# WGLab/NanoCaller

Hardware: AMD Instinct MI355X
Metric: candidate sites/sec (pileup+CNN) (higher is better)
Workload: dtype f32 (f16x3 split MFMA, f32 accumulate)

## Files before the change

### include/nanocaller_hip.h

```cpp
#ifndef NANOCALLER_HIP_H
#define NANOCALLER_HIP_H

#include <stddef.h>
#include <stdint.h>

#ifdef __cplusplus
extern "C" {
#endif

#define NC_ABI_VERSION 11

typedef struct nc_ctx nc_ctx;

enum nc_status {
    NC_OK = 0,
    NC_ERR_ARG = -1,
    NC_ERR_CAPACITY = -2,
    NC_ERR_NOMEM = -3,
    NC_ERR_HIP = -4,
    NC_ERR_STATE = -5,
    NC_ERR_SELFTEST = -6,
    NC_ERR_UNSUPPORTED = -7
};

enum nc_model_kind { NC_MODEL_SNP = 0, NC_MODEL_SNP_HAP = 1, NC_MODEL_INDEL = 2, NC_MODEL_INDEL_HAP = 3 };

enum nc_seq_mode { NC_SEQ_ONT = 0, NC_SEQ_SHORT_ONT = 1, NC_SEQ_UL_ONT = 2, NC_SEQ_UL_ONT_EXTREME = 3, NC_SEQ_PACBIO = 4 };

#define NC_CODE_ABSENT 7
#define NC_FLANK 50000
#define NC_SNP_TENSOR 1025

int nc_abi_version(void);
int nc_device_count(int *n);
int nc_ctx_create(int device_id, nc_ctx **out);
int nc_ctx_destroy(nc_ctx *ctx);
int nc_ctx_set_stream(nc_ctx *ctx, void *hip_stream);
int nc_ctx_sync(nc_ctx *ctx);
const char *nc_last_error(const nc_ctx *ctx);
int nc_malloc(nc_ctx *ctx, size_t bytes, void **dev);
int nc_free(nc_ctx *ctx, void *dev);
int nc_memcpy_h2d(nc_ctx *ctx, void *dev, const void *host, size_t bytes);
int nc_memcpy_d2h(nc_ctx *ctx, void *host, const void *dev, size_t bytes);
int nc_d2h_async(nc_ctx *ctx, void *stream, void *host, const void *dev, size_t bytes);
int nc_last_kernel_ms(nc_ctx *ctx, int which, float *ms);
int nc_enable_timing(nc_ctx *ctx, int on);
int nc_timing_sums(nc_ctx *ctx, double *sum_ms, int64_t *count);

typedef struct {
    int32_t start;
    int32_t end;
    int64_t base_flag;
} nc_tile_entry;

typedef struct {
    int64_t codes_len;
    const uint8_t *codes;
    int32_t tile_size;
    int32_t tile_pos0;
    int32_t n_tiles;
    const int32_t *tile_off;
    const nc_tile_entry *tile_ent;
    int64_t n_entries;
} nc_readpack;

int nc_pack_plan(int32_t n_reads, const int32_t *start, const int32_t *end, const uint8_t *keep,
                 int32_t tile_size, int32_t pos_lo, int32_t pos_hi,
                 int64_t *codes_len, int32_t *tile_pos0, int32_t *n_tiles, int64_t *n_entries);
int nc_pack_fill(int32_t n_reads, const int32_t *start, const int32_t *end, const int64_t *off,
                 const uint8_t *codes_in, const uint8_t *strand, const uint8_t *keep,
                 int32_t tile_size, int32_t tile_pos0, int32_t n_tiles,
                 uint8_t *codes_out, int64_t codes_len, int32_t *tile_off, nc_tile_entry *tile_ent,
                 int64_t n_entries);

typedef struct nc_wire nc_wire;
typedef struct {
    int32_t n_reads;
    const int32_t *rd_start;
    const int32_t *rd_end;
    const int64_t *slot_off;
    int64_t codes_len;
    int64_t n_blocks;
    const uint32_t *blk_off;
    const int32_t *blk_read;
    const uint16_t *events;
    int64_t n_events;
    const uint32_t *blk_ev;
    const uint8_t *ev_bytes;
    int64_t n_ev_bytes;
} nc_wire_arrays;
int nc_wire_build(int32_t n_reads, const int32_t *start, const int32_t *end, const int64_t *off, const uint8_t *codes_in,
                  const uint8_t *keep, const uint8_t *ref_wire, int32_t ref_pos0, int64_t ref_len, nc_wire **out);
int nc_wire_view(const nc_wire *w, nc_wire_arrays *view);
int nc_wire_free(nc_wire *w);
int nc_wire_ref_unpack(nc_ctx *ctx, const uint8_t *d_ref_nib, int64_t ref_len, uint8_t *d_ref_wire);
int nc_wire_ins_unpack(nc_ctx *ctx, const uint8_t *d_packed, int64_t n_bases, const int32_t *d_other_idx, int32_t n_other, uint8_t *d_ins_bases);
int nc_wire_build_del(int32_t n_reads, const int32_t *start, const int32_t *end, const int64_t *off, const uint8_t *codes_in,
                      const uint8_t *keep, const uint8_t *ref_wire, int32_t ref_pos0, int64_t ref_len, const int32_t *ev_off,
                      const int32_t *ev_pos, const int32_t *ev_len, nc_wire **out);
int nc_wire_apply_deletions(nc_ctx *ctx, int32_t n_reads, const int32_t *d_rd_start, const int32_t *d_rd_end, const int64_t *d_slot_off,
                            const int32_t *d_ev_off, const int32_t *d_ev_pos, const int32_t *d_ev_len, uint8_t *d_codes);
int nc_wire_expand(nc_ctx *ctx, int32_t n_reads, const int32_t *d_rd_start, const int32_t *d_rd_end, const int64_t *d_slot_off,
                   const uint8_t *d_ref_wire, int32_t ref_pos0, int64_t ref_len, const uint32_t *d_blk_off,
                   const int32_t *d_blk_read, const uint16_t *d_events, int64_t n_blocks, uint8_t *d_codes, int64_t codes_len,
                   uint8_t *d_ref_code);
int nc_wire_build2(int32_t n_reads, const int32_t *start, const int32_t *end, const int64_t *off, const uint8_t *codes_in,
                   const uint8_t *keep, const uint8_t *ref_wire, int32_t ref_pos0, int64_t ref_len, const int32_t *ev_off,
                   const int32_t *ev_pos, const int32_t *ev_len, int32_t flags, nc_wire **out);
int nc_wire_expand2(nc_ctx *ctx, int32_t n_reads, const int32_t *d_rd_start, const int32_t *d_rd_end, const int64_t *d_slot_off,
                    const uint8_t *d_ref_wire, int32_t ref_pos0, int64_t ref_len, const uint32_t *d_blk_off,
                    const int32_t *d_blk_read, const uint8_t *d_ev_bytes, int64_t n_blocks, uint8_t *d_codes, int64_t codes_len,
                    uint8_t *d_ref_code, const uint32_t *d_blk_ev, const int32_t *d_ev_off, const int32_t *d_ev_pos,
                    const int32_t *d_ev_len);
int nc_wire_expand_del(nc_ctx *ctx, int32_t n_reads, const int32_t *d_rd_start, const int32_t *d_rd_end, const int64_t *d_slot_off,
                       const uint8_t *d_ref_wire, int32_t ref_pos0, int64_t ref_len, const uint32_t *d_blk_off,
                       const int32_t *d_blk_read, const uint16_t *d_events, int64_t n_blocks, uint8_t *d_codes, int64_t codes_len,
                       uint8_t *d_ref_code, const uint32_t *d_blk_ev, const int32_t *d_ev_off, const int32_t *d_ev_pos,
                       const int32_t *d_ev_len);

int nc_indel_events_pack(int32_t n_reads, const int32_t *rd_start, const int32_t *ev_off, const int32_t *ev_pos, const int32_t *ev_len,
                         uint16_t *d16, int8_t *l8, int32_t *read_ins_off, int64_t big_cap, int32_t *big_idx, int32_t *big_pos,
                         int32_t *big_len, int64_t *n_big);
int nc_indel_events_expand(nc_ctx *ctx, int32_t n_reads, const int32_t *d_rd_start, const int32_t *d_ev_off, const uint16_t *d_d16,
                           const int8_t *d_l8, int32_t n_big, const int32_t *d_big_idx, const int32_t *d_big_pos, const int32_t *d_big_len,
                           const int32_t *d_read_ins_off, int32_t *d_ev_pos, int32_t *d_ev_len, int32_t *d_ins_off);
int nc_indel_events_pack8(int32_t n_reads, const int32_t *rd_start, const int32_t *ev_off, const int32_t *ev_pos, const int32_t *ev_len,
                          uint8_t *b8, uint16_t *d16x, int64_t esc_cap, int32_t *read_esc_off, int32_t *read_ins_off, int64_t big_cap,
                          int32_t *big_idx, int32_t *big_pos, int32_t *big_len, int64_t *n_esc, int64_t *n_big);
int nc_indel_events_expand8(nc_ctx *ctx, int32_t n_reads, const int32_t *d_rd_start, const int32_t *d_ev_off, const uint8_t *d_b8,
                            const uint16_t *d_d16x, const int32_t *d_read_esc_off, int32_t n_big, const int32_t *d_big_idx,
                            const int32_t *d_big_pos, const int32_t *d_big_len, const int32_t *d_read_ins_off, int32_t *d_ev_pos,
                            int32_t *d_ev_len, int32_t *d_ins_off);

int nc_inflate_device(nc_ctx *ctx, int32_t n_blocks, const uint8_t *d_comp, const int64_t *d_coff, const int32_t *d_clen, uint8_t *d_out,
                      const int64_t *d_ooff, const int32_t *d_isize, int32_t *d_status, uint32_t *d_tok, int32_t *d_ntok);
int nc_inflate_device_phase(nc_ctx *ctx, int32_t phase, int32_t n_blocks, const uint8_t *d_comp, const int64_t *d_coff, const int32_t *d_clen,
                            uint8_t *d_out, const int64_t *d_ooff, const int32_t *d_isize, int32_t *d_status, uint32_t *d_tok, int32_t *d_ntok);
int nc_bgzf_crc_device(nc_ctx *ctx, int32_t n_blocks, const uint8_t *d_comp, const int64_t *d_coff, const int32_t *d_clen, const uint8_t *d_out,
                       const int64_t *d_ooff, const int32_t *d_isize, int32_t *d_status);

int nc_bam_retag_sizes(nc_ctx *ctx, const uint8_t *d_raw, int32_t n_rec, const int64_t *d_rec_off, const uint64_t *d_hash, const int32_t *d_ps,
                       int32_t n_tags, int32_t *d_new_size, int32_t *d_tag_idx, int64_t *d_out_off, int32_t *d_status);
int nc_bam_retag(nc_ctx *ctx, const uint8_t *d_raw, int32_t n_rec, const int64_t *d_rec_off, const uint8_t *d_hp, const int32_t *d_ps,
                 const int32_t *d_tag_idx, const int64_t *d_out_off, uint8_t *d_out);
int nc_bgzf_deflate_device(nc_ctx *ctx, int32_t n, const uint8_t *d_in, const int64_t *d_ioff, const int32_t *d_ilen, uint8_t *d_out,
                           const int64_t *d_ooff, int32_t *d_clen, uint32_t *d_crc, int32_t *d_status);
int nc_bgzf_crc32_device(nc_ctx *ctx, int32_t n, const uint8_t *d_in, const int64_t *d_ioff, const int32_t *d_ilen, uint32_t *d_crc);
int nc_bgzf_assemble_device(nc_ctx *ctx, int32_t n, const uint8_t *d_pay, const int64_t *d_poff, const int32_t *d_clen, const uint32_t *d_crc,
                            const int32_t *d_isize, int64_t *d_foff, uint8_t *d_file);

#define NC_BAM_META_COLS 12
int nc_bgzf_members(const uint8_t *data, int64_t n, int64_t cap, int64_t *coff, int32_t *clen, int32_t *isize, int64_t *n_members);
int nc_bgzf_scan(const uint8_t *data, int64_t n, int64_t start, int64_t cap, int64_t *coff, int32_t *clen, int32_t *isize, int64_t *n_members,
                 int64_t *next);
int nc_bam_walk(nc_ctx *ctx, const uint8_t *d_raw, int64_t raw_len, int32_t n_seeds, const int64_t *d_seed, const int32_t *d_seed_tid,
                const int64_t *d_first, int64_t *d_out, int32_t *d_status);
int nc_bam_meta(nc_ctx *ctx, const uint8_t *d_raw, int64_t n_rec, const int64_t *d_rec_off, int32_t *d_meta, int32_t *d_status);
int nc_bam_codes(nc_ctx *ctx, const uint8_t *d_raw, int32_t n_reads, const int64_t *d_rec, const int64_t *d_slot, const int32_t *d_cigd,
                 const int32_t *d_ncig, const int32_t *d_start, uint8_t *d_codes);
int nc_bam_name_groups(nc_ctx *ctx, const uint8_t *d_raw, int64_t raw_len, int64_t n_cand, const int64_t *d_rec_off, const uint64_t *d_hash,
                       int32_t *d_gid, int32_t *d_status);
int nc_bam_indel_reads(nc_ctx *ctx, const uint8_t *d_raw, int32_t n_reads, const int64_t *d_rec, const int32_t *d_cigd, const int32_t *d_ncig,
                       int32_t tail_cap, int32_t *d_counts, const int32_t *d_ev_off, const int32_t *d_ins_base, const int32_t *d_tail_off,
                       int32_t *d_ev_pos, int32_t *d_ev_len, int32_t *d_ins_off, uint8_t *d_ins_bases, uint8_t *d_tail_bases);

typedef struct {
    int32_t mincov;
    double min_allele_freq;
    double nbr_t0, nbr_t1;
    int32_t haploid;
} nc_scan_params;

int nc_snp_scan(nc_ctx *ctx, const nc_readpack *pack,
                const uint8_t *ref_code_dev, int32_t ref_pos0, int32_t ref_len,
                int32_t scan_lo, int32_t scan_hi, const nc_scan_params *params,
                int32_t n_chunks, const int32_t *chunk_start_host, const int32_t *chunk_end_host,
                int32_t *n_nbr, int32_t *n_cand, int32_t *n_sites);

int nc_snp_scan_begin(nc_ctx *ctx, const nc_readpack *pack,
                      const uint8_t *ref_code_dev, int32_t ref_pos0, int32_t ref_len,
                      int32_t scan_lo, int32_t scan_hi, const nc_scan_params *params,
                      int32_t n_chunks, const int32_t *chunk_start_host, const int32_t *chunk_end_host);
int nc_snp_scan_end(nc_ctx *ctx, int32_t *n_nbr, int32_t *n_cand, int32_t *n_sites);

int nc_snp_scan_fetch(nc_ctx *ctx, int32_t *nbr_pos, int32_t *site_pos, int32_t *site_chunk,
                      int32_t *site_n, int32_t *site_alt);

int nc_snp_scan_fetch_async(nc_ctx *ctx, void *copy_stream, int32_t *nbr_pos, int32_t *site_pos, int32_t *site_chunk,
                            int32_t *site_n, int32_t *site_alt);

int nc_snp_featurize(nc_ctx *ctx, const nc_readpack *pack,
                     const uint8_t *ref_code_dev, int32_t ref_pos0, int32_t ref_len,
                     int32_t seq_mode, int32_t maxcov, int32_t min_nbr_sites,
                     float *x_dev, int32_t *ref_code_out_dev, int32_t *fwd_dp_dev, int32_t *rev_dp_dev,
                     int32_t *site_depth_dev, uint8_t *valid_dev);

int nc_snp_set_mates(nc_ctx *ctx, int32_t n_mates, const int64_t *d_mate_key, const int32_t *d_mate_rec);

int nc_indel_set_mates(nc_ctx *ctx, int32_t n_mates, const int64_t *d_mate_key, const int32_t *d_mate_rec);

int nc_snp_scale(nc_ctx *ctx, const int32_t *site_depth_dev, const uint8_t *valid_dev, double train_coverage,
                 int32_t mode, double *scale_dev, double *chunk_depth_host);
int nc_snp_chunk_depth_async(nc_ctx *ctx, void *copy_stream, double *chunk_depth_host_pinned);

int nc_load_weights(nc_ctx *ctx, int32_t model_kind, const float *blob_host, size_t n_floats);
int nc_set_cnn_precision(nc_ctx *ctx, int exact_fp32);
int nc_set_tensor_format(nc_ctx *ctx, int fmt);
int nc_snp_forward(nc_ctx *ctx, int32_t model_kind, int64_t n, const float *x_dev, const int32_t *ref_code_dev,
                   const double *scale_dev, int32_t scale_mode, float *probs_dev, float *gt_dev);

int nc_snp_forward_drain(nc_ctx *ctx, int32_t model_kind, int64_t n, const float *x_dev, const int32_t *ref_code_dev,
                         const double *scale_dev, int32_t scale_mode, float *probs_dev, float *gt_dev,
                         void *copy_stream, float *probs_host, float *gt_host);
int nc_cnn_x_limit(nc_ctx *ctx, int32_t model_kind, float *x_limit);
int nc_cnn_range_watch(nc_ctx *ctx, uint8_t *site_flags_dev);
int nc_snp_trunk_info(nc_ctx *ctx, int32_t *mfma_per_site, int32_t *kernel_id);
int nc_indel_forward(nc_ctx *ctx, int32_t model_kind, int64_t n, const float *x_dev, float *probs_dev);

int nc_indel_tensor(nc_ctx *ctx, int32_t n_sets, const uint8_t *rows_dev, const int64_t *row_off_dev,
                    const int32_t *n_rows_dev, const int32_t *n_cols_dev, const uint8_t *ref_rows_dev,
                    const int64_t *ref_off_dev, int32_t max_cols, float *x_dev, uint8_t *cns_dev);

typedef struct {
    int32_t n_reads;
    const int32_t *ev_off;
    const int32_t *ev_pos;
    const int32_t *ev_len;
    const uint8_t *read_hap;
} nc_indel_events;

typedef struct {
    int32_t mincov, win_size, small_win_size;
    double ins_t, del_t;
    int32_t haploid;
    int32_t impute;
} nc_indel_scan_params;

int nc_indel_scan(nc_ctx *ctx, const nc_readpack *pack, const nc_indel_events *events, const uint8_t *excl_dev,
                  int32_t start, int32_t end, const nc_indel_scan_params *params, int8_t *col_type_host);

int nc_indel_scan_batch(nc_ctx *ctx, const nc_readpack *pack, const nc_indel_events *events, const uint8_t *excl_dev,
                        int32_t n_chunks, const int32_t *starts, const int32_t *ends, const nc_indel_scan_params *params,
                        int8_t *col_type_host, const int64_t *col_off);

typedef struct nc_bam nc_bam;
typedef struct nc_decoded nc_decoded;
typedef struct {
    int32_t n_reads;
    const int32_t *start, *end, *flag;
    const int64_t *off;
    const uint8_t *codes;
    int64_t n_codes;
    const int32_t *ev_off;
    const int32_t *ev_pos, *ev_len;
    int64_t n_events;
    const uint8_t *hap;
    const int32_t *ps;
    const int64_t *seq_off;
    const uint8_t *seq;
    int64_t n_seq;
    const int32_t *name_off;
    const char *names;
    const int32_t *qstart;
} nc_decoded_arrays;

int nc_bam_open(const char *path, nc_bam **out);
int nc_bam_close(nc_bam *bam);
int nc_bam_n_refs(nc_bam *bam, int32_t *n_refs, int32_t *has_index);
int nc_bam_ref(nc_bam *bam, int32_t i, const char **name, int32_t *length);
const char *nc_bam_error(const nc_bam *bam);
int nc_bam_set_threads(nc_bam *bam, int32_t n);
int nc_bam_decode(nc_bam *bam, int32_t tid, int32_t beg1, int32_t end1, int32_t keep_seq, nc_decoded **out);
int nc_bam_decode_regions(const char *path, int32_t tid, int32_t beg1, int32_t end1, int32_t keep_seq, int32_t n_regions,
                          nc_decoded **out);
int nc_decoded_view(const nc_decoded *d, nc_decoded_arrays *view);
int nc_decoded_free(nc_decoded *d);
#define NC_FLAG_REFSKIP 0x10000
int nc_decoded_check(const nc_decoded *d, const uint8_t *keep, int64_t *n_refskip, int64_t *n_dup_overlap);
int nc_decoded_name_groups(const nc_decoded *d, const uint8_t *keep, int32_t *gid, int64_t *n_shared);

typedef struct nc_slices nc_slices;
typedef struct {
    int32_t n_anchor;
    const int32_t *anchor_off;
    const int32_t *read_idx;
    const int64_t *seq_off;
    const uint8_t *seq;
    int64_t n_slices;
} nc_slices_arrays;
int nc_indel_slices(const nc_decoded *d, int32_t n_anchor, const int32_t *anchor_pos, int32_t window_before, int32_t window_after,
                    const uint8_t *keep, nc_slices **out);
int nc_slices_view(const nc_slices *s, nc_slices_arrays *view);
int nc_slices_free(nc_slices *s);

typedef struct nc_pass2 nc_pass2;
typedef struct {
    int32_t n_kept;
    const int32_t *anchor_idx;
    const int32_t *first0;
    int32_t sets_per_anchor;
    int32_t n_sets;
    const int32_t *set_read0;
    int32_t n_alignments;
    const int32_t *read_off;
    const char *reads;
    const int32_t *ref_off;
    const char *refs;
    int32_t max_cols;
    const int32_t *al_dup;
} nc_pass2_arrays;
int nc_indel_pass2_sets(const nc_decoded *d, const uint8_t *keep, int32_t n_anchor, const int32_t *anchors, const char *contig,
                        int64_t chrom_len, int32_t ref_lo, int32_t ref_hi, int32_t window_after, int32_t mincov, int32_t maxcov,
                        int32_t haploid, const int32_t *imp_idx, const int32_t *imp_off, const int32_t *imp_reads, nc_pass2 **out);
int nc_pass2_view(const nc_pass2 *p, nc_pass2_arrays *view);
int nc_pass2_free(nc_pass2 *p);


typedef struct nc_indel_pack_h nc_indel_pack_h;
typedef struct {
    int32_t n_reads;
    const int32_t *ev_off;
    const int32_t *ev_pos, *ev_len;
    int64_t n_events;
    const int32_t *ins_off;
    const uint8_t *ins_bases;
    int64_t n_ins_bases;
    const int32_t *tail_off;
    const uint8_t *tail_bases;
    int64_t n_tail_bases;
    const int32_t *read_ps;
    const uint8_t *read_hap;
    const uint8_t *read_flag;
} nc_indel_pack_arrays;
int nc_indel_pack_build(const nc_decoded *d, const uint8_t *keep, int32_t tail_cap, nc_indel_pack_h **out);
int nc_indel_pack_view(const nc_indel_pack_h *p, nc_indel_pack_arrays *view);
int nc_indel_pack_free(nc_indel_pack_h *p);

typedef struct {
    int32_t n_reads;
    const int64_t *slot_off;
    const int32_t *rd_start;
    const int32_t *rd_end;
    const int32_t *ev_off, *ev_pos, *ev_len;
    const int32_t *ins_off;
    const uint8_t *ins_bases;
    const int32_t *tail_off;
    const uint8_t *tail_bases;
    const int32_t *read_ps;
    const uint8_t *read_hap, *read_flag;
} nc_indel_reads;

int nc_indel_sites_plan(nc_ctx *ctx, const nc_readpack *pack, const uint8_t *ref_code_dev, int32_t ref_pos0, int32_t ref_len,
                        int64_t chrom_len, const nc_indel_reads *reads, const uint8_t *excl_dev, int32_t n_chunks,
                        const int32_t *starts, const int32_t *ends, const nc_indel_scan_params *params, int32_t window_after,
                        int32_t maxcov, int32_t *n_sites, int64_t *n_alignments);
int nc_indel_sites_scoring(nc_ctx *ctx, int32_t open, int32_t extend, int32_t match, int32_t mismatch);
int nc_indel_sites_run(nc_ctx *ctx, float *x_dev);
int nc_indel_sites_fetch(nc_ctx *ctx, int32_t *pos, int32_t *chunk, int32_t *var_type, int32_t *phase, int32_t *ref_len,
                         int32_t *alt_len, int64_t *n_alt_bytes);
int nc_indel_sites_fetch_alt(nc_ctx *ctx, uint8_t *alt_bases, int64_t cap);
int nc_indel_sites_stage_ms(nc_ctx *ctx, float *ms6, int64_t *cells2 );
int nc_indel_sites_band_stats(nc_ctx *ctx, int64_t *stats6);
int nc_indel_sites_band(nc_ctx *ctx, int32_t mode, int32_t margin);

int nc_indel_vcf_format(const char *chrom, int64_t n, const int32_t *pos, const int32_t *chunk, int32_t n_chunks, const float *probs,
                        int32_t sets, const int32_t *ref_len, const int32_t *alt_len, const uint8_t *alt_bases, const int32_t *phase,
                        const char *contig, int64_t chrom_len, int32_t haploid, char *out, int64_t cap, int64_t *n_bytes,
                        int64_t *chunk_txt_off);

int nc_nw_cigar(const char *s1, int32_t n1, const char *s2, int32_t n2, int32_t open, int32_t extend, int32_t match, int32_t mismatch,
                int32_t *ops, int32_t *counts, int32_t cap, int32_t *n_ops);

int nc_allele_prediction(const char *alt, int32_t n_alt, const char *ref_seq, int32_t n_ref, int32_t max_range, int32_t *ref_len,
                         int32_t *alt_len);
int nc_allele_prediction_batch(int32_t n, const char *alts, const int32_t *alt_off, const char *refs, const int32_t *ref_off,
                               const int32_t *max_range, int32_t *ref_len, int32_t *alt_len);
int nc_allele_prediction_device(nc_ctx *ctx, int32_t n, const char *alts, const int32_t *alt_off, const char *refs, const int32_t *ref_off,
                                const int32_t *max_range, int32_t *ref_len, int32_t *alt_len);

int nc_star_msa(int32_t n_reads, const char *reads, const int32_t *read_off, const char *ref, int32_t n_ref, int32_t open,
                int32_t extend, int32_t match, int32_t mismatch, int32_t col_cap, uint8_t *rows, uint8_t *ref_row, int32_t *n_cols);

int nc_star_msa_tensor(nc_ctx *ctx, int32_t n_sets, const char *reads, const int32_t *read_off, const int32_t *set_read0,
                       const char *refs, const int32_t *ref_off, int32_t open, int32_t extend, int32_t match, int32_t mismatch,
                       int32_t max_cols, float *x_dev, uint8_t *cns_host, int32_t *n_cols_host, uint8_t *rows_host,
                       const int64_t *rows_host_off, uint8_t *ref_rows_host, const int64_t *ref_rows_host_off);
int nc_star_msa_tensor_dup(nc_ctx *ctx, int32_t n_sets, const char *reads, const int32_t *read_off, const int32_t *set_read0,
                           const char *refs, const int32_t *ref_off, int32_t open, int32_t extend, int32_t match, int32_t mismatch,
                           int32_t max_cols, float *x_dev, uint8_t *cns_host, int32_t *n_cols_host, uint8_t *rows_host,
                           const int64_t *rows_host_off, uint8_t *ref_rows_host, const int64_t *ref_rows_host_off, const int32_t *al_dup);

int nc_consensus_strings(const uint8_t *cns, int32_t n_sets, int32_t max_cols, const int32_t *n_cols, char *out, int64_t *off);

int nc_snp_vcf_format(const char *chrom, int64_t n, const int32_t *pos, const int32_t *ref, const float *probs,
                      const int32_t *order, const int32_t *dp, const double *freq, const int32_t *fwd, const int32_t *rev,
                      int32_t haploid, char *out, int64_t cap, int64_t *n_bytes);

int nc_argsort4(const float *probs, int64_t n, int32_t *order, int64_t *n_ties, int64_t *tie_idx, int64_t tie_cap);

int nc_bgzf_compress(const uint8_t *data, int64_t n, int32_t level, uint8_t *out, int64_t cap, int64_t *n_out,
                     int64_t *block_coff, int64_t blk_cap, int64_t *n_blocks);

int nc_bgzf_read_file(const char *path, uint8_t *out, int64_t cap, int64_t *n_out);

int nc_synth_indel_truth(nc_ctx *ctx, int64_t L, uint64_t seed, double het_snp, double hom_snp, double het_indel, double hom_indel,
                         int32_t max_len, uint8_t *ref_dev, uint8_t *hap_base_dev, int8_t *hap_indel_dev);
int nc_synth_indel_reads(nc_ctx *ctx, int64_t L, uint64_t seed, double p_sub, double p_del, double p_ins, double carry, int32_t n_reads,
                         const int32_t *start_dev, const int32_t *end_dev, const int64_t *slot_off_dev, const uint8_t *hap_dev,
                         const uint8_t *hap_base_dev, const int8_t *hap_indel_dev, int32_t fill, int32_t *ev_cnt_dev, int32_t *ins_cnt_dev,
                         const int32_t *ev_off_dev, const int32_t *ins_off_read_dev, uint8_t *codes_dev, int32_t *ev_pos_dev,
                         int32_t *ev_len_dev, int32_t *ins_off_dev, uint8_t *ins_bases_dev);

typedef struct nc_phase nc_phase;
typedef struct {
    int32_t n_reads, n_sites, n_blocks, n_groups;
    int64_t n_entries;
    const int64_t *entry_off;
    const int32_t *entry_site;
    const uint8_t *entry_allele;
    const int8_t *read_side;
    const int32_t *site_block;
    const uint8_t *site_h;
    const uint8_t *site_phased;
    const int32_t *site_ps;
    const int32_t *block_first, *block_last, *block_ps;
    const int64_t *block_cost;
    const uint8_t *group_hp;
    const int32_t *group_ps;
    float ms[4];
} nc_phase_arrays;
int nc_snp_phase_gather(nc_ctx *ctx, const uint8_t *codes, int64_t codes_len, int32_t n_reads, const int32_t *rd_start, const int32_t *rd_end,
                        const int64_t *slot_off, int32_t n_sites, const int32_t *site_pos, const uint8_t *site_alleles, nc_phase **out);
int nc_snp_phase_realign(nc_ctx *ctx, const uint8_t *codes, int64_t codes_len, const nc_indel_reads *reads, int64_t n_events, int64_t n_ins_bases,
                         const uint8_t *ref_code, int32_t ref_len, int32_t n_sites, const int32_t *site_pos, const uint8_t *site_alleles, nc_phase **out);
int nc_snp_phase_load(nc_ctx *ctx, int32_t n_reads, int32_t n_sites, const int32_t *site_pos, const int64_t *entry_off, const int32_t *entry_site,
                      const uint8_t *entry_allele, nc_phase **out);
int nc_snp_phase_solve(nc_ctx *ctx, nc_phase *ph, int32_t max_cov);
int nc_haplotag_run(nc_ctx *ctx, nc_phase *ph, int32_t n_groups, const int32_t *read_group);
int nc_snp_phase_view(const nc_phase *ph, nc_phase_arrays *out);
int nc_snp_phase_free(nc_phase *ph);
int nc_snp_phase_solve_gt(nc_ctx *ctx, nc_phase *ph, int32_t max_cov, const uint8_t *site_gt, int32_t gt_cost);
int nc_snp_phase_genotypes(const nc_phase *ph, const uint8_t **site_gt);
int nc_snp_phase_set_weights(nc_ctx *ctx, nc_phase *ph, const uint8_t *entry_weight, const uint8_t *read_ok);
int nc_snp_phase_weights_from_bam(nc_ctx *ctx, nc_phase *ph, const uint8_t *d_raw, int64_t raw_len, const int64_t *d_rec_off, int32_t mapq_min,
                                  int32_t default_weight, int32_t w_max);
int nc_snp_phase_weights(const nc_phase *ph, const uint8_t **entry_weight, const uint8_t **read_mapq, const uint8_t **read_ok);

int nc_fasta_decode(nc_ctx *ctx, const uint8_t *d_raw, int64_t raw_len, int64_t first, int64_t length, int64_t linebases, int64_t linewidth,
                    uint8_t *d_letters, uint8_t *d_scan, int64_t scan_pos0, int64_t scan_len, int64_t ga, int64_t gb, uint8_t *d_blind,
                    int32_t *d_status);

#define NC_BAMIDX_BAD_BLOCK_SIZE 2
#define NC_BAMIDX_BAD_FIELDS 4
#define NC_BAMIDX_TRUNCATED 8
#define NC_BAMIDX_BAD_REFID 16
#define NC_BAMIDX_UNSORTED 32
#define NC_BAMIDX_BAD_MEMBERS 64
int nc_bamidx_candidates(nc_ctx *ctx, const uint8_t *d_raw, int64_t len, int64_t readable, int32_t n_ref, const int32_t *d_ref_len, uint64_t *d_words,
                         int32_t *d_cnt);
int nc_bamidx_chain(nc_ctx *ctx, const uint8_t *d_raw, int64_t len, int64_t first, const uint64_t *d_words, const int32_t *d_rank, int32_t n_cand,
                    int64_t *d_pos, int32_t *d_jump, int32_t *d_mark);
int nc_bamidx_collect(nc_ctx *ctx, int32_t n_cand, const int64_t *d_pos, const int32_t *d_mark, const int32_t *d_mark_rank, int64_t *d_out);
int nc_bamidx_verify(nc_ctx *ctx, const uint8_t *d_raw, int64_t len, int64_t first, int64_t n_rec, const int64_t *d_out, int32_t last, int64_t *d_res);
int nc_bamidx_serial(nc_ctx *ctx, const uint8_t *d_raw, int64_t len, int64_t first, int32_t last, int64_t *d_out, int64_t *d_res);
int nc_bamidx_fields(nc_ctx *ctx, const uint8_t *d_raw, int64_t n_rec, const int64_t *d_rec_off, int64_t stream_base, const int32_t *d_meta, int32_t n_ref,
                     int32_t n_mem, const int64_t *d_mem_ooff, const int64_t *d_mem_foff, int32_t has_prev, int32_t prev_refid, int32_t prev_pos,
                     int32_t min_shift, int32_t depth, int64_t *d_voff, int32_t *d_fields, int32_t *d_status);

#ifdef __cplusplus
}
#endif
#endif
```

### nanocaller_amd/_lib.py

```python
from __future__ import annotations

import ctypes as C
import os

import numpy as np

_HERE = os.path.dirname(os.path.abspath(__file__))
LIB_PATH = os.environ.get("NANOCALLER_HIP_LIB") or os.path.join(_HERE, "libnanocaller_hip.so")

NC_OK = 0
NC_ERR_ARG = -1
NC_ERR_CAPACITY = -2
NC_ERR_NOMEM = -3
NC_ERR_UNSUPPORTED = -7
FLAG_REFSKIP = 0x10000
ABI_VERSION = 11
MODEL_SNP, MODEL_SNP_HAP, MODEL_INDEL, MODEL_INDEL_HAP = 0, 1, 2, 3
SEQ_MODES = {"ont": 0, "short_ont": 1, "ul_ont": 2, "ul_ont_extreme": 3, "pacbio": 4}
CODE_ABSENT = 7
FLANK = 50000
SNP_TENSOR = 1025
STAR_SCORING = (25, 1, 20, -10)

EXPORTS = [
    "nc_abi_version", "nc_device_count", "nc_ctx_create", "nc_ctx_destroy", "nc_ctx_set_stream", "nc_ctx_sync",
    "nc_last_error", "nc_malloc", "nc_free", "nc_memcpy_h2d", "nc_memcpy_d2h", "nc_last_kernel_ms",
    "nc_enable_timing", "nc_pack_plan", "nc_pack_fill", "nc_snp_scan", "nc_snp_scan_begin", "nc_snp_scan_end", "nc_snp_scan_fetch", "nc_snp_featurize",
    "nc_snp_scale", "nc_load_weights", "nc_snp_forward", "nc_indel_forward", "nc_indel_tensor", "nc_indel_scan",
    "nc_bam_open", "nc_bam_close", "nc_bam_n_refs", "nc_bam_ref", "nc_bam_error", "nc_bam_decode", "nc_decoded_view",
    "nc_decoded_free", "nc_snp_vcf_format", "nc_set_cnn_precision", "nc_snp_scan_fetch_async", "nc_snp_forward_drain", "nc_argsort4", "nc_indel_slices", "nc_slices_view", "nc_slices_free",
    "nc_nw_cigar", "nc_allele_prediction", "nc_bgzf_compress", "nc_bam_set_threads", "nc_indel_scan_batch", "nc_timing_sums", "nc_snp_chunk_depth_async", "nc_bam_decode_regions", "nc_star_msa", "nc_star_msa_tensor", "nc_star_msa_tensor_dup", "nc_set_tensor_format", "nc_allele_prediction_batch", "nc_allele_prediction_device", "nc_bgzf_read_file", "nc_consensus_strings",
    "nc_wire_build", "nc_wire_build_del", "nc_wire_apply_deletions", "nc_wire_ref_unpack", "nc_wire_view", "nc_wire_free", "nc_wire_expand", "nc_wire_expand_del", "nc_snp_set_mates", "nc_indel_set_mates", "nc_decoded_name_groups", "nc_wire_ins_unpack", "nc_indel_events_pack8", "nc_indel_events_expand8", "nc_wire_build2", "nc_wire_expand2", "nc_d2h_async",
    "nc_indel_pass2_sets", "nc_pass2_view", "nc_pass2_free",
    "nc_decoded_check", "nc_indel_pack_build", "nc_indel_pack_view", "nc_indel_pack_free", "nc_indel_sites_plan", "nc_indel_sites_run",
    "nc_indel_sites_fetch", "nc_indel_sites_fetch_alt", "nc_indel_sites_stage_ms", "nc_indel_sites_band_stats", "nc_indel_sites_band", "nc_indel_events_pack", "nc_indel_events_expand", "nc_inflate_device", "nc_inflate_device_phase", "nc_bgzf_crc_device", "nc_bgzf_members", "nc_bgzf_scan", "nc_bam_walk", "nc_bam_meta", "nc_bam_codes", "nc_bam_indel_reads", "nc_bam_name_groups", "nc_indel_sites_scoring", "nc_indel_vcf_format", "nc_synth_indel_truth", "nc_synth_indel_reads", "nc_cnn_x_limit", "nc_cnn_range_watch", "nc_snp_trunk_info",
    "nc_snp_phase_gather", "nc_snp_phase_load", "nc_snp_phase_solve", "nc_haplotag_run", "nc_snp_phase_view", "nc_snp_phase_free",
    "nc_snp_phase_realign", "nc_snp_phase_solve_gt", "nc_snp_phase_genotypes",
    "nc_snp_phase_set_weights", "nc_snp_phase_weights_from_bam", "nc_snp_phase_weights",
    "nc_bam_retag_sizes", "nc_bam_retag", "nc_bgzf_deflate_device", "nc_bgzf_crc32_device", "nc_bgzf_assemble_device",
    "nc_fasta_decode",
    "nc_bamidx_candidates", "nc_bamidx_chain", "nc_bamidx_collect", "nc_bamidx_verify", "nc_bamidx_serial", "nc_bamidx_fields",
]


class TileEntry(C.Structure):
    _fields_ = [("start", C.c_int32), ("end", C.c_int32), ("base_flag", C.c_int64)]


TILE_ENTRY_DTYPE = np.dtype([("start", "<i4"), ("end", "<i4"), ("base_flag", "<i8")])
assert TILE_ENTRY_DTYPE.itemsize == C.sizeof(TileEntry) == 16


class ReadPackC(C.Structure):
    _fields_ = [("codes_len", C.c_int64), ("codes", C.c_void_p), ("tile_size", C.c_int32), ("tile_pos0", C.c_int32),
                ("n_tiles", C.c_int32), ("tile_off", C.c_void_p), ("tile_ent", C.c_void_p), ("n_entries", C.c_int64)]


class ScanParamsC(C.Structure):
    _fields_ = [("mincov", C.c_int32), ("min_allele_freq", C.c_double), ("nbr_t0", C.c_double), ("nbr_t1", C.c_double),
                ("haploid", C.c_int32)]


class IndelEventsC(C.Structure):
    _fields_ = [("n_reads", C.c_int32), ("ev_off", C.c_void_p), ("ev_pos", C.c_void_p), ("ev_len", C.c_void_p),
                ("read_hap", C.c_void_p)]


class IndelScanParamsC(C.Structure):
    _fields_ = [("mincov", C.c_int32), ("win_size", C.c_int32), ("small_win_size", C.c_int32), ("ins_t", C.c_double),
                ("del_t", C.c_double), ("haploid", C.c_int32), ("impute", C.c_int32)]


class DecodedArraysC(C.Structure):
    _fields_ = [("n_reads", C.c_int32), ("start", C.c_void_p), ("end", C.c_void_p), ("flag", C.c_void_p), ("off", C.c_void_p),
                ("codes", C.c_void_p), ("n_codes", C.c_int64), ("ev_off", C.c_void_p), ("ev_pos", C.c_void_p),
                ("ev_len", C.c_void_p), ("n_events", C.c_int64), ("hap", C.c_void_p), ("ps", C.c_void_p),
                ("seq_off", C.c_void_p), ("seq", C.c_void_p), ("n_seq", C.c_int64), ("name_off", C.c_void_p),
                ("names", C.c_void_p), ("qstart", C.c_void_p)]


class SlicesArraysC(C.Structure):
    _fields_ = [("n_anchor", C.c_int32), ("anchor_off", C.c_void_p), ("read_idx", C.c_void_p), ("seq_off", C.c_void_p),
                ("seq", C.c_void_p), ("n_slices", C.c_int64)]


class Pass2ArraysC(C.Structure):
    _fields_ = [("n_kept", C.c_int32), ("anchor_idx", C.c_void_p), ("first0", C.c_void_p), ("sets_per_anchor", C.c_int32),
                ("n_sets", C.c_int32), ("set_read0", C.c_void_p), ("n_alignments", C.c_int32), ("read_off", C.c_void_p),
                ("reads", C.c_void_p), ("ref_off", C.c_void_p), ("refs", C.c_void_p), ("max_cols", C.c_int32), ("al_dup", C.c_void_p)]


class IndelPackArraysC(C.Structure):
    _fields_ = [("n_reads", C.c_int32), ("ev_off", C.c_void_p), ("ev_pos", C.c_void_p), ("ev_len", C.c_void_p), ("n_events", C.c_int64),
                ("ins_off", C.c_void_p), ("ins_bases", C.c_void_p), ("n_ins_bases", C.c_int64), ("tail_off", C.c_void_p),
                ("tail_bases", C.c_void_p), ("n_tail_bases", C.c_int64), ("read_ps", C.c_void_p), ("read_hap", C.c_void_p),
                ("read_flag", C.c_void_p)]


class IndelReadsC(C.Structure):
    _fields_ = [("n_reads", C.c_int32), ("slot_off", C.c_void_p), ("rd_start", C.c_void_p), ("rd_end", C.c_void_p), ("ev_off", C.c_void_p),
                ("ev_pos", C.c_void_p), ("ev_len", C.c_void_p), ("ins_off", C.c_void_p), ("ins_bases", C.c_void_p), ("tail_off", C.c_void_p),
                ("tail_bases", C.c_void_p), ("read_ps", C.c_void_p), ("read_hap", C.c_void_p), ("read_flag", C.c_void_p)]


class WireArraysC(C.Structure):
    _fields_ = [("n_reads", C.c_int32), ("rd_start", C.c_void_p), ("rd_end", C.c_void_p), ("slot_off", C.c_void_p),
                ("codes_len", C.c_int64), ("n_blocks", C.c_int64), ("blk_off", C.c_void_p), ("blk_read", C.c_void_p), ("events", C.c_void_p),
                ("n_events", C.c_int64), ("blk_ev", C.c_void_p), ("ev_bytes", C.c_void_p), ("n_ev_bytes", C.c_int64)]


class PhaseArraysC(C.Structure):
    _fields_ = [("n_reads", C.c_int32), ("n_sites", C.c_int32), ("n_blocks", C.c_int32), ("n_groups", C.c_int32), ("n_entries", C.c_int64),
                ("entry_off", C.c_void_p), ("entry_site", C.c_void_p), ("entry_allele", C.c_void_p), ("read_side", C.c_void_p),
                ("site_block", C.c_void_p), ("site_h", C.c_void_p), ("site_phased", C.c_void_p), ("site_ps", C.c_void_p),
                ("block_first", C.c_void_p), ("block_last", C.c_void_p), ("block_ps", C.c_void_p), ("block_cost", C.c_void_p),
                ("group_hp", C.c_void_p), ("group_ps", C.c_void_p), ("ms", C.c_float * 4)]


_lib = None


class NanoCallerHipError(RuntimeError):
    pass


def lib():
    global _lib
    if _lib is None:
        if not os.path.exists(LIB_PATH):
            raise NanoCallerHipError(
                "%s not found: build it with `python -c 'import __graft_entry__ as g; g.build()'` "
                "(hipcc --offload-arch=gfx950). There is no CPU fallback." % LIB_PATH)
        try:
            import torch
        except ImportError:
            pass
        L = C.CDLL(LIB_PATH)
        vp, i32, i64, dbl = C.c_void_p, C.c_int32, C.c_int64, C.c_double
        L.nc_abi_version.restype = C.c_int
        if L.nc_abi_version() != ABI_VERSION:
            raise NanoCallerHipError("%s has ABI version %d, this binding needs %d: rebuild it" % (LIB_PATH, L.nc_abi_version(), ABI_VERSION))
        L.nc_device_count.argtypes = [C.POINTER(C.c_int)]
        L.nc_ctx_create.argtypes = [C.c_int, C.POINTER(vp)]
        L.nc_ctx_destroy.argtypes = [vp]
        L.nc_ctx_set_stream.argtypes = [vp, vp]
        L.nc_ctx_sync.argtypes = [vp]
        L.nc_last_error.argtypes = [vp]
        L.nc_last_error.restype = C.c_char_p
        L.nc_malloc.argtypes = [vp, C.c_size_t, C.POINTER(vp)]
        L.nc_free.argtypes = [vp, vp]
        L.nc_memcpy_h2d.argtypes = [vp, vp, vp, C.c_size_t]
        L.nc_memcpy_d2h.argtypes = [vp, vp, vp, C.c_size_t]
        L.nc_last_kernel_ms.argtypes = [vp, C.c_int, C.POINTER(C.c_float)]
        L.nc_timing_sums.argtypes = [vp, vp, vp]
        L.nc_enable_timing.argtypes = [vp, C.c_int]
        L.nc_set_cnn_precision.argtypes = [vp, C.c_int]
        L.nc_pack_plan.argtypes = [i32, vp, vp, vp, i32, i32, i32, C.POINTER(i64), C.POINTER(i32), C.POINTER(i32),
                                   C.POINTER(i64)]
        L.nc_pack_fill.argtypes = [i32, vp, vp, vp, vp, vp, vp, i32, i32, i32, vp, i64, vp, vp, i64]
        L.nc_snp_scan.argtypes = [vp, C.POINTER(ReadPackC), vp, i32, i32, i32, i32, C.POINTER(ScanParamsC), i32, vp, vp,
                                  C.POINTER(i32), C.POINTER(i32), C.POINTER(i32)]
        L.nc_snp_scan_begin.argtypes = [vp, C.POINTER(ReadPackC), vp, i32, i32, i32, i32, C.POINTER(ScanParamsC), i32, vp, vp]
        L.nc_snp_scan_end.argtypes = [vp, C.POINTER(i32), C.POINTER(i32), C.POINTER(i32)]
        L.nc_snp_scan_fetch.argtypes = [vp, vp, vp, vp, vp, vp]
        L.nc_snp_scan_fetch_async.argtypes = [vp, vp, vp, vp, vp, vp, vp]
        L.nc_snp_featurize.argtypes = [vp, C.POINTER(ReadPackC), vp, i32, i32, i32, i32, i32, vp, vp, vp, vp, vp, vp]
        L.nc_snp_scale.argtypes = [vp, vp, vp, dbl, i32, vp, vp]
        L.nc_snp_chunk_depth_async.argtypes = [vp, vp, vp]
        L.nc_load_weights.argtypes = [vp, i32, vp, C.c_size_t]
        L.nc_snp_forward.argtypes = [vp, i32, i64, vp, vp, vp, i32, vp, vp]
        L.nc_snp_forward_drain.argtypes = [vp, i32, i64, vp, vp, vp, i32, vp, vp, vp, vp, vp]
        L.nc_indel_forward.argtypes = [vp, i32, i64, vp, vp]
        L.nc_indel_tensor.argtypes = [vp, i32, vp, vp, vp, vp, vp, vp, i32, vp, vp]
        L.nc_indel_scan.argtypes = [vp, C.POINTER(ReadPackC), C.POINTER(IndelEventsC), vp, i32, i32, C.POINTER(IndelScanParamsC), vp]
        L.nc_indel_scan_batch.argtypes = [vp, C.POINTER(ReadPackC), C.POINTER(IndelEventsC), vp, i32, vp, vp, C.POINTER(IndelScanParamsC), vp, vp]
        L.nc_bam_open.argtypes = [C.c_char_p, C.POINTER(vp)]
        L.nc_bam_close.argtypes = [vp]
        L.nc_bam_set_threads.argtypes = [vp, i32]
        L.nc_bam_n_refs.argtypes = [vp, C.POINTER(i32), C.POINTER(i32)]
        L.nc_bam_ref.argtypes = [vp, i32, C.POINTER(C.c_char_p), C.POINTER(i32)]
        L.nc_bam_error.argtypes = [vp]
        L.nc_bam_error.restype = C.c_char_p
        L.nc_bam_decode.argtypes = [vp, i32, i32, i32, i32, C.POINTER(vp)]
        L.nc_star_msa_tensor.argtypes = [vp, i32, vp, vp, vp, vp, vp, i32, i32, i32, i32, i32, vp, vp, vp, vp, vp, vp, vp]
        L.nc_star_msa_tensor_dup.argtypes = L.nc_star_msa_tensor.argtypes + [vp]
        L.nc_consensus_strings.argtypes = [vp, i32, i32, vp, vp, vp]
        L.nc_allele_prediction_batch.argtypes = [i32, C.c_char_p, vp, C.c_char_p, vp, vp, vp, vp]
        L.nc_allele_prediction_device.argtypes = [vp, i32, C.c_char_p, vp, C.c_char_p, vp, vp, vp, vp]
        L.nc_set_tensor_format.argtypes = [vp, C.c_int]
        L.nc_star_msa.argtypes = [i32, C.c_char_p, vp, C.c_char_p, i32, i32, i32, i32, i32, i32, vp, vp, C.POINTER(i32)]
        L.nc_bam_decode_regions.argtypes = [C.c_char_p, i32, i32, i32, i32, i32, C.POINTER(vp)]
        L.nc_decoded_view.argtypes = [vp, C.POINTER(DecodedArraysC)]
        L.nc_decoded_free.argtypes = [vp]
        L.nc_indel_slices.argtypes = [vp, i32, vp, i32, i32, vp, C.POINTER(vp)]
        L.nc_slices_view.argtypes = [vp, C.POINTER(SlicesArraysC)]
        L.nc_slices_free.argtypes = [vp]
        L.nc_nw_cigar.argtypes = [C.c_char_p, i32, C.c_char_p, i32, i32, i32, i32, i32, vp, vp, i32, C.POINTER(i32)]
        L.nc_allele_prediction.argtypes = [C.c_char_p, i32, C.c_char_p, i32, i32, C.POINTER(i32), C.POINTER(i32)]
        L.nc_bgzf_compress.argtypes = [vp, i64, i32, vp, i64, C.POINTER(i64), vp, i64, C.POINTER(i64)]
        L.nc_indel_pass2_sets.argtypes = [vp, vp, i32, vp, C.c_char_p, i64, i32, i32, i32, i32, i32, i32, vp, vp, vp, C.POINTER(vp)]
        L.nc_pass2_view.argtypes = [vp, C.POINTER(Pass2ArraysC)]
        L.nc_pass2_free.argtypes = [vp]
        L.nc_d2h_async.argtypes = [vp, vp, vp, vp, C.c_size_t]
        L.nc_wire_build.argtypes = [i32, vp, vp, vp, vp, vp, vp, i32, i64, C.POINTER(vp)]
        L.nc_wire_build_del.argtypes = [i32, vp, vp, vp, vp, vp, vp, i32, i64, vp, vp, vp, C.POINTER(vp)]
        L.nc_wire_build2.argtypes = [i32, vp, vp, vp, vp, vp, vp, i32, i64, vp, vp, vp, i32, C.POINTER(vp)]
        L.nc_wire_apply_deletions.argtypes = [vp, i32, vp, vp, vp, vp, vp, vp, vp]
        L.nc_wire_ref_unpack.argtypes = [vp, vp, i64, vp]
        L.nc_wire_view.argtypes = [vp, C.POINTER(WireArraysC)]
        L.nc_wire_free.argtypes = [vp]
        L.nc_wire_expand.argtypes = [vp, i32, vp, vp, vp, vp, i32, i64, vp, vp, vp, i64, vp, i64, vp]
        L.nc_wire_expand_del.argtypes = L.nc_wire_expand.argtypes + [vp, vp, vp, vp]
        L.nc_wire_expand2.argtypes = L.nc_wire_expand.argtypes + [vp, vp, vp, vp]
        L.nc_snp_set_mates.argtypes = [vp, i32, vp, vp]
        L.nc_indel_set_mates.argtypes = [vp, i32, vp, vp]
        L.nc_decoded_name_groups.argtypes = [vp, vp, vp, C.POINTER(i64)]
        L.nc_wire_ins_unpack.argtypes = [vp, vp, i64, vp, i32, vp]
        L.nc_indel_events_pack8.argtypes = [i32, vp, vp, vp, vp, vp, vp, i64, vp, vp, i64, vp, vp, vp, C.POINTER(i64), C.POINTER(i64)]
        L.nc_indel_events_expand8.argtypes = [vp, i32, vp, vp, vp, vp, vp, i32, vp, vp, vp, vp, vp, vp, vp]
        L.nc_decoded_check.argtypes = [vp, vp, C.POINTER(i64), C.POINTER(i64)]
        L.nc_indel_pack_build.argtypes = [vp, vp, i32, C.POINTER(vp)]
        L.nc_indel_pack_view.argtypes = [vp, C.POINTER(IndelPackArraysC)]
        L.nc_indel_pack_free.argtypes = [vp]
        L.nc_indel_sites_plan.argtypes = [vp, C.POINTER(ReadPackC), vp, i32, i32, i64, C.POINTER(IndelReadsC), vp, i32, vp, vp,
                                          C.POINTER(IndelScanParamsC), i32, i32, C.POINTER(i32), C.POINTER(i64)]
        L.nc_indel_sites_run.argtypes = [vp, vp]
        L.nc_indel_sites_scoring.argtypes = [vp, i32, i32, i32, i32]
        L.nc_indel_sites_fetch.argtypes = [vp, vp, vp, vp, vp, vp, vp, C.POINTER(i64)]
        L.nc_indel_sites_fetch_alt.argtypes = [vp, vp, i64]
        L.nc_indel_sites_stage_ms.argtypes = [vp, vp, vp]
        L.nc_indel_sites_band_stats.argtypes = [vp, vp]
        L.nc_indel_sites_band.argtypes = [vp, i32, i32]
        L.nc_indel_events_pack.argtypes = [i32, vp, vp, vp, vp, vp, vp, vp, i64, vp, vp, vp, C.POINTER(i64)]
        L.nc_indel_events_expand.argtypes = [vp, i32, vp, vp, vp, vp, i32, vp, vp, vp, vp, vp, vp, vp]
        L.nc_inflate_device.argtypes = [vp, i32, vp, vp, vp, vp, vp, vp, vp, vp, vp]
        L.nc_inflate_device_phase.argtypes = [vp, i32, i32, vp, vp, vp, vp, vp, vp, vp, vp, vp]
        L.nc_bgzf_crc_device.argtypes = [vp, i32, vp, vp, vp, vp, vp, vp, vp]
        L.nc_bgzf_members.argtypes = [vp, i64, i64, vp, vp, vp, C.POINTER(i64)]
        L.nc_bgzf_scan.argtypes = [vp, i64, i64, i64, vp, vp, vp, C.POINTER(i64), C.POINTER(i64)]
        L.nc_bam_walk.argtypes = [vp, vp, i64, i32, vp, vp, vp, vp, vp]
        L.nc_bam_meta.argtypes = [vp, vp, i64, vp, vp, vp]
        L.nc_bam_codes.argtypes = [vp, vp, i32, vp, vp, vp, vp, vp, vp]
        L.nc_bam_indel_reads.argtypes = [vp, vp, i32, vp, vp, vp, i32, vp, vp, vp, vp, vp, vp, vp, vp, vp]
        L.nc_bam_name_groups.argtypes = [vp, vp, i64, i64, vp, vp, vp, vp]
        L.nc_indel_vcf_format.argtypes = [C.c_char_p, i64, vp, vp, i32, vp, i32, vp, vp, vp, vp, C.c_char_p, i64, i32, vp, i64, C.POINTER(i64), vp]
        L.nc_synth_indel_truth.argtypes = [vp, i64, C.c_uint64, dbl, dbl, dbl, dbl, i32, vp, vp, vp]
        L.nc_synth_indel_reads.argtypes = [vp, i64, C.c_uint64, dbl, dbl, dbl, dbl, i32, vp, vp, vp, vp, vp, vp, i32, vp, vp, vp, vp, vp, vp, vp, vp, vp]
        L.nc_cnn_x_limit.argtypes = [vp, i32, C.POINTER(C.c_float)]
        L.nc_snp_trunk_info.argtypes = [vp, C.POINTER(C.c_int32), C.POINTER(C.c_int32)]
        L.nc_cnn_range_watch.argtypes = [vp, vp]
        L.nc_argsort4.argtypes = [vp, i64, vp, C.POINTER(i64), vp, i64]
        L.nc_snp_phase_gather.argtypes = [vp, vp, i64, i32, vp, vp, vp, i32, vp, vp, C.POINTER(vp)]
        L.nc_snp_phase_load.argtypes = [vp, i32, i32, vp, vp, vp, vp, C.POINTER(vp)]
        L.nc_snp_phase_solve.argtypes = [vp, vp, i32]
        L.nc_snp_phase_solve_gt.argtypes = [vp, vp, i32, vp, i32]
        L.nc_snp_phase_genotypes.argtypes = [vp, C.POINTER(vp)]
        L.nc_snp_phase_set_weights.argtypes = [vp, vp, vp, vp]
        L.nc_snp_phase_weights_from_bam.argtypes = [vp, vp, vp, i64, vp, i32, i32, i32]
        L.nc_snp_phase_weights.argtypes = [vp, C.POINTER(vp), C.POINTER(vp), C.POINTER(vp)]
        L.nc_snp_phase_realign.argtypes = [vp, vp, i64, C.POINTER(IndelReadsC), i64, i64, vp, i32, i32, vp, vp, C.POINTER(vp)]
        L.nc_haplotag_run.argtypes = [vp, vp, i32, vp]
        L.nc_snp_phase_view.argtypes = [vp, C.POINTER(PhaseArraysC)]
        L.nc_snp_phase_free.argtypes = [vp]
        L.nc_bam_retag_sizes.argtypes = [vp, vp, i32, vp, vp, vp, i32, vp, vp, vp, vp]
        L.nc_bam_retag.argtypes = [vp, vp, i32, vp, vp, vp, vp, vp, vp]
        L.nc_bgzf_deflate_device.argtypes = [vp, i32, vp, vp, vp, vp, vp, vp, vp, vp]
        L.nc_bgzf_crc32_device.argtypes = [vp, i32, vp, vp, vp, vp]
        L.nc_bgzf_assemble_device.argtypes = [vp, i32, vp, vp, vp, vp, vp, vp, vp]
        L.nc_fasta_decode.argtypes = [vp, vp, i64, i64, i64, i64, i64, vp, vp, i64, i64, i64, i64, vp, vp]
        L.nc_bamidx_candidates.argtypes = [vp, vp, i64, i64, i32, vp, vp, vp]
        L.nc_bamidx_chain.argtypes = [vp, vp, i64, i64, vp, vp, i32, vp, vp, vp]
        L.nc_bamidx_collect.argtypes = [vp, i32, vp, vp, vp, vp]
        L.nc_bamidx_verify.argtypes = [vp, vp, i64, i64, i64, vp, i32, vp]
        L.nc_bamidx_serial.argtypes = [vp, vp, i64, i64, i32, vp, vp]
        L.nc_bamidx_fields.argtypes = [vp, vp, i64, vp, i64, vp, i32, i32, vp, vp, i32, i32, i32, i32, i32, vp, vp, vp]
        L.nc_snp_vcf_format.argtypes = [C.c_char_p, i64, vp, vp, vp, vp, vp, vp, vp, vp, i32, vp, i64, C.POINTER(i64)]
        for name in EXPORTS:
            fn = getattr(L, name)
            if name not in ("nc_last_error", "nc_bam_error"):
                fn.restype = C.c_int
        _lib = L
    return _lib


def npp(a):
    if a is None:
        return None
    assert a.flags["C_CONTIGUOUS"]
    return a.ctypes.data_as(C.c_void_p)
```

### nanocaller_amd/csrc/nc_cnn.h

```cpp
#pragma once
#include <cmath>
#include <vector>

#include "nc_common.h"

constexpr float SELU_L = 1.0507009873554805f;
constexpr float SELU_LA = 1.0507009873554805f * 1.6732632423543772f;

__device__ __forceinline__ float selu(float x) { return x > 0.0f ? SELU_L * x : SELU_LA * (__expf(x) - 1.0f); }
__device__ __forceinline__ float selu_acc(float x) { return x > 0.0f ? SELU_L * x : SELU_LA * (expf(x) - 1.0f); }

typedef float f32x4v __attribute__((ext_vector_type(4)));
typedef _Float16 h8 __attribute__((ext_vector_type(8)));
typedef _Float16 h2 __attribute__((ext_vector_type(2)));
typedef float f32x2v __attribute__((ext_vector_type(2)));
__device__ __forceinline__ h8 as_h8(uint4 v) { union { uint4 u; h8 h; } c; c.u = v; return c.h; }
__device__ __forceinline__ h8 lds_h8(const _Float16 *p) { return *reinterpret_cast<const h8 *>(p); }
struct h_epi { float c1, c2, c3; };
__device__ __forceinline__ float exp2_clamp01(float x) { float r; asm("v_exp_f32_e64 %0, %1 clamp" : "=v"(r) : "v"(x)); return r; }
__device__ __forceinline__ float sub_h_lo(float v, uint32_t hpk) { float r; asm("v_fma_mix_f32 %0, %1, -1.0, %2 op_sel_hi:[1,0,0]" : "=v"(r) : "v"(hpk), "v"(v)); return r; }
__device__ __forceinline__ float sub_h_hi(float v, uint32_t hpk) { float r; asm("v_fma_mix_f32 %0, %1, -1.0, %2 op_sel:[1,0,0] op_sel_hi:[1,0,0]" : "=v"(r) : "v"(hpk), "v"(v)); return r; }
__device__ __forceinline__ f32x4v selu4_scaled(const f32x4v &acc, const h_epi &k)
{
    f32x4v s;
#pragma unroll
    for (int r = 0; r < 4; r++) {
        const float a = acc[r];
        const float e = exp2_clamp01(a * k.c1);
        const float pos = __builtin_amdgcn_fmed3f(a, 0.0f, k.c3);
        const float neg = fmaf(e, SELU_LA, -SELU_LA);
        s[r] = fmaf(pos, k.c2, neg);
    }
    return s;
}
__device__ __forceinline__ void split4_store(const f32x4v &v, _Float16 *hp, _Float16 *lp)
{
    const h2 h01 = __builtin_convertvector((f32x2v){v[0], v[1]}, h2), h23 = __builtin_convertvector((f32x2v){v[2], v[3]}, h2);
    const uint32_t u01 = __builtin_bit_cast(uint32_t, h01), u23 = __builtin_bit_cast(uint32_t, h23);
    const f32x2v d01 = {sub_h_lo(v[0], u01), sub_h_hi(v[1], u01)}, d23 = {sub_h_lo(v[2], u23), sub_h_hi(v[3], u23)};
    const h2 l01 = __builtin_convertvector(d01, h2), l23 = __builtin_convertvector(d23, h2);
    *reinterpret_cast<uint2 *>(hp) = make_uint2(u01, u23);
    *reinterpret_cast<uint2 *>(lp) = make_uint2(__builtin_bit_cast(uint32_t, l01), __builtin_bit_cast(uint32_t, l23));
}

struct H3Scale {
    float S;
    H3Scale(const float *w0, const float *w1, float s0) : S(s0)
    {
        float wmax = 0.0f;
        for (const float *q = w0; q < w1; q++) wmax = std::fmax(wmax, std::fabs(*q));
        while (S > 1.0f && wmax * S > 16384.0f) S *= 0.5f;
    }
    void split(float v, _Float16 &h, _Float16 &l) const
    {
        const float sv = v * S;
        h = (_Float16)sv;
        l = (_Float16)(sv - (float)h);
    }
};

inline unsigned blocks_for(int64_t n, int per = 256) { return (unsigned)((n + per - 1) / per); }

enum { NC_TRUNK_FP32 = 0, NC_TRUNK_P3 = 2, NC_TRUNK_LIN = 3 };
struct SnpTrunk { int kernel_id, mfma_per_site; };
SnpTrunk nc_cnn_snp_trunk_select(const nc_ctx *ctx);
struct SnpTrunkArgs {
    hipStream_t stream;
    hipEvent_t ev0, ev1;
    const float *x_f32;
    const int16_t *x_i16;
    float *a3;
    int64_t nb, site0;
    const double *scale;
    int scale_mode;
    float x_limit;
    uint8_t *range_sites;
};
void nc_cnn_launch_k4_conv12(const SnpTrunkArgs &a, const float *packed);
void nc_cnn_launch_k5_trunk(int kernel_id, const SnpTrunkArgs &a, const uint8_t *packed_h);
void nc_cnn_launch_fc1_h3(hipStream_t st, const float *a3, const uint8_t *packed_h, float *f1, int64_t nb);
std::vector<float> nc_cnn_pack_k4(const float *blob);
std::vector<uint8_t> nc_cnn_pack_snp_h3(const float *blob);

void nc_cnn_launch_fc1_fp32(hipStream_t st, int F, const float *a3, int K, const float *kf, const float *bf, float *f1, int64_t nb);

void nc_cnn_launch_indel_convs_fp32(hipStream_t st, int H, const float *x, const float *w, float *a1, float *a2, float *a3, int64_t nb);
int nc_cnn_launch_k10(nc_ctx *ctx, int H, const float *x, const uint8_t *packed_h, float *a3, int64_t nb);
std::vector<uint8_t> nc_cnn_pack_indel_h3(const float *blob);
```

### nanocaller_amd/csrc/nc_cnn.hip

```cpp
#include <algorithm>

#include "nc_cnn.h"

namespace {

__device__ __forceinline__ void dense_small(const float *in, int n_in, const float *k, const float *b, int n_out, float *out, bool act)
{
    for (int o = 0; o < n_out; o++) {
        float acc = b[o];
        for (int i = 0; i < n_in; i++) acc = fmaf(in[i], k[i * n_out + o], acc);
        out[o] = act ? selu_acc(acc) : acc;
    }
}

__device__ __forceinline__ void softmax_small(float *x, int n)
{
    float m = x[0];
    for (int i = 1; i < n; i++) m = fmaxf(m, x[i]);
    float sum = 0.0f;
    for (int i = 0; i < n; i++) { x[i] = expf(x[i] - m); sum += x[i]; }
    for (int i = 0; i < n; i++) x[i] = x[i] / sum;
}

__global__ __launch_bounds__(256) void k_snp_heads(const float *__restrict__ fc1, const float *__restrict__ w,
                                                   const int32_t *__restrict__ ref_code, int64_t n, float *__restrict__ probs,
                                                   float *__restrict__ gt)
{
    const int64_t s = (int64_t)blockIdx.x * 256 + threadIdx.x;
    if (s >= n) return;
    float f1[48], fa[16], in17[17], heads[4][2], fc2[16], in24[24], fc3[8], g[2];
    for (int i = 0; i < 48; i++) f1[i] = fc1[s * 48 + i];
    const float *p = w;
    dense_small(f1, 48, p, p + 768, 16, fa, true);
    p += 768 + 16;
    for (int i = 0; i < 16; i++) in17[i] = fa[i];
    const int rc = ref_code[s];
    for (int h = 0; h < 4; h++) {
        in17[16] = rc == h ? 1.0f : 0.0f;
        dense_small(in17, 17, p, p + 34, 2, heads[h], false);
        p += 34 + 2;
        softmax_small(heads[h], 2);
        probs[s * 4 + h] = heads[h][1];
    }
    dense_small(f1, 48, p, p + 768, 16, fc2, true);
    p += 768 + 16;
    for (int i = 0; i < 16; i++) in24[i] = fc2[i];
    for (int h = 0; h < 4; h++) { in24[16 + 2 * h] = heads[h][0]; in24[17 + 2 * h] = heads[h][1]; }
    dense_small(in24, 24, p, p + 192, 8, fc3, true);
    p += 192 + 8;
    dense_small(fc3, 8, p, p + 16, 2, g, false);
    softmax_small(g, 2);
    if (gt) { gt[s * 2] = g[0]; gt[s * 2 + 1] = g[1]; }
}

__global__ __launch_bounds__(256) void k_snp_hap_heads(const float *__restrict__ fc1, const float *__restrict__ w,
                                                       const int32_t *__restrict__ ref_code, int64_t n, float *__restrict__ probs)
{
    const int64_t s = (int64_t)blockIdx.x * 256 + threadIdx.x;
    if (s >= n) return;
    float f1[48], in20[20], out[4];
    for (int i = 0; i < 48; i++) f1[i] = fc1[s * 48 + i];
    const float *p = w;
    dense_small(f1, 48, p, p + 768, 16, in20, true);
    p += 768 + 16;
    const int rc = ref_code[s];
    for (int b = 0; b < 4; b++) in20[16 + b] = rc == b ? 1.0f : 0.0f;
    dense_small(in20, 20, p, p + 80, 4, out, true);
    softmax_small(out, 4);
    for (int b = 0; b < 4; b++) probs[s * 4 + b] = out[b];
}

__global__ __launch_bounds__(256) void k_indel_heads(const float *__restrict__ fc1, const float *__restrict__ w, int nout, int64_t n,
                                                     float *__restrict__ probs)
{
    const int64_t s = (int64_t)blockIdx.x * 256 + threadIdx.x;
    if (s >= n) return;
    float f1[32], f2[24], out[4];
    for (int i = 0; i < 32; i++) f1[i] = fc1[s * 32 + i];
    const float *p = w;
    dense_small(f1, 32, p, p + 768, 24, f2, true);
    p += 768 + 24;
    dense_small(f2, 24, p, p + 24 * nout, nout, out, false);
    if (nout == 4) {
        softmax_small(out, 4);
        for (int b = 0; b < 4; b++) probs[s * 4 + b] = out[b];
    } else {
        probs[s] = 1.0f / (1.0f + expf(-out[0]));
    }
}

const size_t NPARAM[4] = {109370, 108308, 634420, 158185};

int run_snp_trunk(nc_ctx *ctx, const nc_weights &w, int64_t s0, int64_t nb, const void *x_dev, const double *scale, int scale_mode, const float **f1_out, const float **tail)
{
    constexpr int64_t n3 = 3 * 9 * 64, F = 48;
    NC_TRY(nc_ensure(ctx, ctx->cnn_c, (size_t)(nb * (n3 + F)) * 4 + 64));
    float *a3 = (float *)ctx->cnn_c.p, *f1 = a3 + ((nb * n3 + 3) & ~int64_t(3));
    const float *kf = w.dev + (400 + 16) * 2 + 2000 + 16 + 6 * 48 * 32 + 32 + 6 * 32 * 64 + 64, *bf = kf + n3 * F;
    *tail = bf + F;
    *f1_out = f1;
    SnpTrunkArgs a = {ctx->stream, nullptr, nullptr, nullptr, nullptr, a3, nb, s0, scale, scale_mode, w.x_limit, ctx->range_sites};
    if (ctx->x_i16) a.x_i16 = (const int16_t *)x_dev + s0 * NC_SNP_TENSOR;
    else a.x_f32 = (const float *)x_dev + s0 * NC_SNP_TENSOR;
    if (ctx->timing && ctx->n_kev + 2 <= 128) {
        for (int e = 0; e < 2; e++)
            if (!ctx->kev[ctx->n_kev + e]) NC_HIP(ctx, hipEventCreate(&ctx->kev[ctx->n_kev + e]));
        a.ev0 = ctx->kev[ctx->n_kev];
        a.ev1 = ctx->kev[ctx->n_kev + 1];
        ctx->n_kev += 2;
    }
    const SnpTrunk t = nc_cnn_snp_trunk_select(ctx);
    if (t.kernel_id == NC_TRUNK_FP32) {
        nc_cnn_launch_k4_conv12(a, w.packed);
        nc_cnn_launch_fc1_fp32(ctx->stream, F, a3, (int)n3, kf, bf, f1, nb);
    } else {
        nc_cnn_launch_k5_trunk(t.kernel_id, a, (const uint8_t *)w.packed_h);
        nc_cnn_launch_fc1_h3(ctx->stream, a3, (const uint8_t *)w.packed_h, f1, nb);
    }
    NC_HIP(ctx, hipGetLastError());
    return NC_OK;
}

int run_indel_trunk(nc_ctx *ctx, const nc_weights &w, int H, int64_t nb, const float *x_batch, const float **f1_out, const float **tail)
{
    constexpr int W = 128, CI = 2, C1 = 8, C2 = 32, C3 = 48, F = 32, W2 = (W - 3) / 2 + 1, W3 = (W2 - 3) / 2 + 1;
    const int64_t n1 = (int64_t)H * W * 3 * C1, n2 = (int64_t)(H - 1) * W2 * C2, n3 = (int64_t)(H - 2) * W3 * C3;
    const bool h3 = !ctx->cnn_exact_fp32 && w.x_limit >= 1.0f;
    if (!h3) {
        NC_TRY(nc_ensure(ctx, ctx->cnn_a, (size_t)(nb * n1) * 4));
        NC_TRY(nc_ensure(ctx, ctx->cnn_b, (size_t)(nb * n2) * 4));
    }
    NC_TRY(nc_ensure(ctx, ctx->cnn_c, (size_t)(nb * (n3 + F)) * 4 + 64));
    float *a3 = (float *)ctx->cnn_c.p, *f1 = a3 + ((nb * n3 + 3) & ~int64_t(3));
    const float *kf = w.dev + (5 + 5 + 25) * CI * C1 + 3 * C1 + 6 * 3 * C1 * C2 + C2 + 6 * C2 * C3 + C3, *bf = kf + n3 * F;
    *tail = bf + F;
    *f1_out = f1;
    if (h3) NC_TRY(nc_cnn_launch_k10(ctx, H, x_batch, (const uint8_t *)w.packed_h, a3, nb));
    else nc_cnn_launch_indel_convs_fp32(ctx->stream, H, x_batch, w.dev, (float *)ctx->cnn_a.p, (float *)ctx->cnn_b.p, a3, nb);
    nc_cnn_launch_fc1_fp32(ctx->stream, F, a3, (int)n3, kf, bf, f1, nb);
    NC_HIP(ctx, hipGetLastError());
    return NC_OK;
}

float cnn_x_limit(int kind, const float *blob)
{
    const bool snp = kind == NC_MODEL_SNP || kind == NC_MODEL_SNP_HAP;
    const int CI = snp ? 5 : 2, C1 = snp ? 16 : 8, C2 = 32, C3 = snp ? 64 : 48;
    auto l1 = [](const float *k, int n_in, int cout) {
        double best = 0;
        for (int c = 0; c < cout; c++) {
            double acc = 0;
            for (int i = 0; i < n_in; i++) acc += std::fabs((double)k[(size_t)i * cout + c]);
            best = std::max(best, acc);
        }
        return best;
    };
    auto amax = [](const float *b, int n) { double m = 0; for (int i = 0; i < n; i++) m = std::max(m, std::fabs((double)b[i])); return m; };
    const float *k11 = blob, *b11 = k11 + 5 * CI * C1, *k12 = b11 + C1, *b12 = k12 + 5 * CI * C1, *k13 = b12 + C1, *b13 = k13 + 25 * CI * C1;
    const float *k2 = b13 + C1, *b2 = k2 + 6 * 3 * C1 * C2, *k3 = b2 + C2, *b3 = k3 + 6 * C2 * C3;
    const double L1 = std::max(l1(k11, 5 * CI, C1), std::max(l1(k12, 5 * CI, C1), l1(k13, 25 * CI, C1)));
    const double B1 = std::max(amax(b11, C1), std::max(amax(b12, C1), amax(b13, C1)));
    const double L2 = l1(k2, 6 * 3 * C1, C2), B2 = amax(b2, C2), L3 = l1(k3, 6 * C2, C3), B3 = amax(b3, C3);
    const double LAM = 1.0507009873554805, LA = LAM * 1.6732632423543772, CAP = 60000.0 * 0.999;
    auto worst = [&](double X) {
        const double a1 = std::max(LAM * (L1 * X + B1), LA), a2 = std::max(LAM * (L2 * a1 + B2), LA), a3 = std::max(LAM * (L3 * a2 + B3), LA);
        return snp ? std::max(a1, std::max(a2, a3)) : std::max(a1, a2);
    };
    double lo = 0.0, hi = 1e6;
    if (worst(0.0) >= CAP) hi = 0.0;
    for (int it = 0; it < 60 && hi > 0.0; it++) {
        const double mid = 0.5 * (lo + hi);
        if (worst(mid) < CAP) lo = mid; else hi = mid;
    }
    return (float)lo;
}

int upload_blob(nc_ctx *ctx, void **dev, const void *host, size_t bytes, const char *what)
{
    if (!*dev) {
        hipError_t e = hipMalloc(dev, bytes);
        if (e != hipSuccess) return nc_fail(ctx, NC_ERR_NOMEM, "hipMalloc %s: %s", what, hipGetErrorString(e));
    }
    NC_HIP(ctx, hipMemcpyAsync(*dev, host, bytes, hipMemcpyHostToDevice, ctx->stream));
    NC_HIP(ctx, hipStreamSynchronize(ctx->stream));
    return NC_OK;
}

}

extern "C" {

int nc_load_weights(nc_ctx *ctx, int32_t kind, const float *blob_host, size_t n_floats)
{
    if (!ctx) return NC_ERR_ARG;
    if (kind < 0 || kind > 3 || !blob_host) return nc_fail(ctx, NC_ERR_ARG, "nc_load_weights: bad argument");
    if (n_floats != NPARAM[kind])
        return nc_fail(ctx, NC_ERR_ARG, "nc_load_weights: kind %d expects %zu floats, got %zu", kind, NPARAM[kind], n_floats);
    NC_HIP(ctx, hipSetDevice(ctx->device));
    nc_weights &w = ctx->w[kind];
    NC_TRY(upload_blob(ctx, (void **)&w.dev, blob_host, n_floats * 4, "weights"));
    w.n = n_floats;
    w.x_limit = cnn_x_limit(kind, blob_host);
    if (kind == NC_MODEL_SNP || kind == NC_MODEL_SNP_HAP) {
        const std::vector<float> pk = nc_cnn_pack_k4(blob_host);
        NC_TRY(upload_blob(ctx, (void **)&w.packed, pk.data(), pk.size() * 4, "packed weights"));
        const std::vector<uint8_t> hp = nc_cnn_pack_snp_h3(blob_host);
        NC_TRY(upload_blob(ctx, &w.packed_h, hp.data(), hp.size(), "packed fp16 weights"));
    } else {
        const std::vector<uint8_t> hp = nc_cnn_pack_indel_h3(blob_host);
        NC_TRY(upload_blob(ctx, &w.packed_h, hp.data(), hp.size(), "packed fp16 weights"));
    }
    return NC_OK;
}


int nc_snp_forward(nc_ctx *ctx, int32_t kind, int64_t n, const float *x_dev, const int32_t *ref_code_dev, const double *scale_dev,
                   int32_t scale_mode, float *probs_dev, float *gt_dev)
{
    return nc_snp_forward_drain(ctx, kind, n, x_dev, ref_code_dev, scale_dev, scale_mode, probs_dev, gt_dev, nullptr, nullptr, nullptr);
}

int nc_snp_forward_drain(nc_ctx *ctx, int32_t kind, int64_t n, const float *x_dev, const int32_t *ref_code_dev, const double *scale_dev,
                         int32_t scale_mode, float *probs_dev, float *gt_dev, void *copy_stream, float *probs_host, float *gt_host)
{
    if (!ctx) return NC_ERR_ARG;
    if (probs_host && !copy_stream) return nc_fail(ctx, NC_ERR_ARG, "nc_snp_forward_drain: host drain needs a copy stream");
    if (kind != NC_MODEL_SNP && kind != NC_MODEL_SNP_HAP) return nc_fail(ctx, NC_ERR_ARG, "nc_snp_forward: not an SNP model kind");
    if (!ctx->w[kind].dev) return nc_fail(ctx, NC_ERR_STATE, "nc_snp_forward: weights of kind %d not loaded", kind);
    if (n < 0 || (n && (!x_dev || !ref_code_dev || !probs_dev))) return nc_fail(ctx, NC_ERR_ARG, "nc_snp_forward: null argument");
    if (scale_mode != 0 && scale_mode != 1) return nc_fail(ctx, NC_ERR_ARG, "nc_snp_forward: scale_mode");
    if (ctx->x_i16 && ctx->cnn_exact_fp32) return nc_fail(ctx, NC_ERR_STATE, "nc_snp_forward: int16 tensors are read by the split-precision trunk only");
    NC_HIP(ctx, hipSetDevice(ctx->device));
    NcTimer tm(ctx, 2);
    if (ctx->timing) nc_timing_resolve(ctx, 4);
    ctx->n_kev = 0;
    const int64_t BATCH = 262144;
    for (int64_t s0 = 0; s0 < n; s0 += BATCH) {
        const int64_t nb = n - s0 < BATCH ? n - s0 : BATCH;
        const float *tail = nullptr, *f1 = nullptr;
        NC_TRY(run_snp_trunk(ctx, ctx->w[kind], s0, nb, x_dev, scale_dev, scale_mode, &f1, &tail));
        if (kind == NC_MODEL_SNP)
            hipLaunchKernelGGL(k_snp_heads, dim3(blocks_for(nb)), dim3(256), 0, ctx->stream, f1, tail, ref_code_dev + s0, nb,
                               probs_dev + s0 * 4, gt_dev ? gt_dev + s0 * 2 : nullptr);
        else
            hipLaunchKernelGGL(k_snp_hap_heads, dim3(blocks_for(nb)), dim3(256), 0, ctx->stream, f1, tail, ref_code_dev + s0, nb,
                               probs_dev + s0 * 4);
        NC_HIP(ctx, hipGetLastError());
        if (probs_host) {
            const int slot = (int)((s0 / BATCH) & 3);
            if (!ctx->drain_ev[slot]) NC_HIP(ctx, hipEventCreateWithFlags(&ctx->drain_ev[slot], hipEventDisableTiming));
            NC_HIP(ctx, hipEventRecord(ctx->drain_ev[slot], ctx->stream));
            NC_HIP(ctx, hipStreamWaitEvent((hipStream_t)copy_stream, ctx->drain_ev[slot], 0));
            NC_TRY(nc_d2h(ctx, probs_host + s0 * 4, probs_dev + s0 * 4, (size_t)nb * 16, (hipStream_t)copy_stream));
            if (gt_host && gt_dev)
                NC_TRY(nc_d2h(ctx, gt_host + s0 * 2, gt_dev + s0 * 2, (size_t)nb * 8, (hipStream_t)copy_stream));
        }
    }
    tm.stop();
    if (ctx->timing) ctx->kev_pending = true;
    return NC_OK;
}

int nc_cnn_x_limit(nc_ctx *ctx, int32_t kind, float *x_limit)
{
    if (!ctx || kind < 0 || kind > 3 || !x_limit) return NC_ERR_ARG;
    if (!ctx->w[kind].dev) return nc_fail(ctx, NC_ERR_STATE, "nc_cnn_x_limit: weights of kind %d not loaded", kind);
    *x_limit = ctx->w[kind].x_limit;
    return NC_OK;
}

int nc_snp_trunk_info(nc_ctx *ctx, int32_t *mfma_per_site, int32_t *kernel_id)
{
    if (!ctx) return NC_ERR_ARG;
    const SnpTrunk t = nc_cnn_snp_trunk_select(ctx);
    if (mfma_per_site) *mfma_per_site = t.mfma_per_site;
    if (kernel_id) *kernel_id = t.kernel_id;
    return NC_OK;
}

int nc_cnn_range_watch(nc_ctx *ctx, uint8_t *site_flags_dev)
{
    if (!ctx) return NC_ERR_ARG;
    ctx->range_sites = site_flags_dev;
    return NC_OK;
}

int nc_indel_forward(nc_ctx *ctx, int32_t kind, int64_t n, const float *x_dev, float *probs_dev)
{
    if (!ctx) return NC_ERR_ARG;
    if (kind != NC_MODEL_INDEL && kind != NC_MODEL_INDEL_HAP) return nc_fail(ctx, NC_ERR_ARG, "nc_indel_forward: not an indel model kind");
    if (!ctx->w[kind].dev) return nc_fail(ctx, NC_ERR_STATE, "nc_indel_forward: weights of kind %d not loaded", kind);
    if (n < 0 || (n && (!x_dev || !probs_dev))) return nc_fail(ctx, NC_ERR_ARG, "nc_indel_forward: null argument");
    NC_HIP(ctx, hipSetDevice(ctx->device));
    const int nout = kind == NC_MODEL_INDEL ? 4 : 1;
    const int H = kind == NC_MODEL_INDEL ? 15 : 5;
    const int64_t xs = H * 128 * 2;
    NcTimer tm(ctx, 2);
    const int64_t BATCH = kind == NC_MODEL_INDEL ? 65536 : 262144;
    for (int64_t s0 = 0; s0 < n; s0 += BATCH) {
        const int64_t nb = n - s0 < BATCH ? n - s0 : BATCH;
        const float *tail = nullptr, *f1 = nullptr;
        NC_TRY(run_indel_trunk(ctx, ctx->w[kind], H, nb, x_dev + s0 * xs, &f1, &tail));
        hipLaunchKernelGGL(k_indel_heads, dim3(blocks_for(nb)), dim3(256), 0, ctx->stream, f1, tail, nout, nb, probs_dev + s0 * nout);
        NC_HIP(ctx, hipGetLastError());
    }
    tm.stop();
    return NC_OK;
}

}
```

### nanocaller_amd/csrc/nc_common.h

```cpp
#pragma once
#include <hip/hip_runtime.h>

#include <cstdarg>
#include <cstdint>
#include <cstdio>
#include <cstring>
#include <vector>

#include "../../include/nanocaller_hip.h"

__device__ __forceinline__ int32_t nc_wave_incl_scan(int32_t v)
{
    v += __builtin_amdgcn_update_dpp(0, v, 0x111, 0xf, 0xf, true);
    v += __builtin_amdgcn_update_dpp(0, v, 0x112, 0xf, 0xf, true);
    v += __builtin_amdgcn_update_dpp(0, v, 0x114, 0xf, 0xf, true);
    v += __builtin_amdgcn_update_dpp(0, v, 0x118, 0xf, 0xf, true);
    v += __builtin_amdgcn_update_dpp(0, v, 0x142, 0xa, 0xf, true);
    v += __builtin_amdgcn_update_dpp(0, v, 0x143, 0xc, 0xf, true);
    return v;
}

struct DevBuf {
    void *p = nullptr;
    size_t cap = 0;
    DevBuf() = default;
    DevBuf(const DevBuf &) = delete;
    DevBuf &operator=(const DevBuf &) = delete;
    ~DevBuf() { release(); }
    void release()
    {
        if (p) (void)hipFree(p);
        p = nullptr;
        cap = 0;
    }
};

struct nc_weights {
    float *dev = nullptr;
    size_t n = 0;
    float *packed = nullptr;
    void *packed_h = nullptr;
    float x_limit = 0.0f;
};

struct nc_ctx {
    int device = 0;
    hipStream_t own_stream = nullptr;
    hipStream_t stream = nullptr;
    char err[512] = {0};
    int timing = 0;
    bool x_i16 = false;
    bool cnn_exact_fp32 = false;
    bool k10_lds_set[2] = {false, false};
    bool huff_lds_set = false;
    bool deflate_lds_set = false;
    DevBuf deflate_tok;
    int32_t n_mates = 0;
    const int64_t *mate_key = nullptr;
    const int32_t *mate_rec = nullptr;
    int32_t n_imates = 0;
    const int64_t *imate_key = nullptr;
    const int32_t *imate_rec = nullptr;
    hipEvent_t ev0 = nullptr, ev1 = nullptr;
    float last_ms[6] = {0, 0, 0, 0, 0, 0};
    hipEvent_t kev[128] = {nullptr};
    int n_kev = 0;
    hipEvent_t tev[4][2] = {{nullptr, nullptr}, {nullptr, nullptr}, {nullptr, nullptr}, {nullptr, nullptr}};
    bool tev_pending[4] = {false, false, false, false};
    bool kev_pending = false;
    double sum_ms[6] = {0, 0, 0, 0, 0, 0};
    int64_t sum_n[6] = {0, 0, 0, 0, 0, 0};
    hipEvent_t drain_ev[4] = {nullptr};
    hipEvent_t scale_ev = nullptr;
    hipEvent_t scan_ev = nullptr;

    DevBuf stage_nbr, stage_cpos, stage_cn, stage_calt;
    DevBuf tile_cnt, tile_pre;
    DevBuf nbr_pos, cand_pos, cand_n, cand_alt;
    DevBuf chunk_start, chunk_end, chunk_lo, chunk_cnt, chunk_off;
    DevBuf site_pos, site_chunk, site_n, site_alt;
    DevBuf totals;
    DevBuf cnn_a, cnn_b, cnn_c;
    DevBuf chunk_depth;
    DevBuf nbr_idx;
    struct {
        size_t budget = 0;
        bool budget_shrunk = false;
        DevBuf ws;
        DevBuf ent_read;
        const void *ent_of = nullptr;
        int ent_spt = 0;
    } k7;
    DevBuf msa_reads, msa_read_off, msa_read_set, msa_refs, msa_ref_off;
    DevBuf msa_dup;
    DevBuf msa_rows_hf, msa_hcol, msa_tb, msa_trace, msa_cols, msa_out;
    int32_t n_nbr = 0, n_cand = 0, n_sites = 0, n_chunks = 0;
    bool have_scan = false;

    nc_weights w[4];
    struct nc_pipe_state *pipe = nullptr;
    uint8_t *range_sites = nullptr;

    int32_t *mbox = nullptr;
    bool scan_begun = false;
    int scan_tile = 0, scan_n_tiles = 0, scan_n_chunks = 0, scan_cap_nbr = 0, scan_cap_cand = 0;
    hipEvent_t scan_tot_ev = nullptr;
    uint8_t *stage_h = nullptr;
    int stage_turn = 0;
};

int nc_d2h(nc_ctx *ctx, void *host, const void *dev, size_t bytes, hipStream_t st);
int nc_h2d_small(nc_ctx *ctx, void *dev, const void *host, size_t bytes, hipStream_t st);
#define NC_D2H_KERNEL_MAX 65536
#define NC_STAGE_SLOT 16384
#define NC_STAGE_SLOTS 16

inline int nc_h2d_pieces(nc_ctx *ctx, void *dev, const void *host, size_t bytes, hipStream_t st)
{
    int in_flight = 0;
    for (size_t o = 0; o < bytes; o += NC_STAGE_SLOT) {
        if (++in_flight >= NC_STAGE_SLOTS - 2) {
            if (hipStreamSynchronize(st) != hipSuccess) return NC_ERR_HIP;
            in_flight = 1;
        }
        const size_t n = bytes - o < (size_t)NC_STAGE_SLOT ? bytes - o : (size_t)NC_STAGE_SLOT;
        const int rc = nc_h2d_small(ctx, (char *)dev + o, (const char *)host + o, n, st);
        if (rc != NC_OK) return rc;
    }
    return NC_OK;
}
inline int nc_d2h_pieces(nc_ctx *ctx, void *host_pinned, const void *dev, size_t bytes, hipStream_t st)
{
    for (size_t o = 0; o < bytes; o += NC_D2H_KERNEL_MAX) {
        const size_t n = bytes - o < (size_t)NC_D2H_KERNEL_MAX ? bytes - o : (size_t)NC_D2H_KERNEL_MAX;
        const int rc = nc_d2h(ctx, (char *)host_pinned + o, (const char *)dev + o, n, st);
        if (rc != NC_OK) return rc;
    }
    return NC_OK;
}

inline int nc_fail(nc_ctx *ctx, int code, const char *fmt, ...)
{
    if (ctx) {
        va_list ap;
        va_start(ap, fmt);
        vsnprintf(ctx->err, sizeof ctx->err, fmt, ap);
        va_end(ap);
    }
    return code;
}

#define NC_HIP(ctx, call)                                                                           \
    do {                                                                                            \
        hipError_t e_ = (call);                                                                     \
        if (e_ != hipSuccess)                                                                       \
            return nc_fail(ctx, NC_ERR_HIP, "%s failed: %s (%s:%d)", #call, hipGetErrorString(e_),  \
                           __FILE__, __LINE__);                                                     \
    } while (0)

inline int nc_ensure(nc_ctx *ctx, DevBuf &b, size_t bytes)
{
    if (bytes <= b.cap) return NC_OK;
    if (b.p) {
        NC_HIP(ctx, hipStreamSynchronize(ctx->stream));
        NC_HIP(ctx, hipFree(b.p));
        b.p = nullptr;
        b.cap = 0;
    }
    size_t want = bytes + bytes / 4 + 256;
    hipError_t e = hipMalloc(&b.p, want);
    if (e != hipSuccess) return nc_fail(ctx, NC_ERR_NOMEM, "hipMalloc(%zu) failed: %s", want, hipGetErrorString(e));
    b.cap = want;
    return NC_OK;
}

#define NC_TRY(x)                \
    do {                         \
        int rc_ = (x);           \
        if (rc_ != NC_OK) return rc_; \
    } while (0)

extern "C" __attribute__((visibility("hidden"))) void nc_timing_resolve(nc_ctx *ctx, int which);

struct NcTimer {
    nc_ctx *ctx;
    int which;
    NcTimer(nc_ctx *c, int w) : ctx(c), which(w)
    {
        if (ctx->timing == 1) {
            nc_timing_resolve(ctx, which);
            for (int e = 0; e < 2; e++)
                if (!ctx->tev[which][e]) (void)hipEventCreate(&ctx->tev[which][e]);
            (void)hipEventRecord(ctx->tev[which][0], ctx->stream);
        }
    }
    void stop()
    {
        if (ctx->timing == 1) {
            (void)hipEventRecord(ctx->tev[which][1], ctx->stream);
            ctx->tev_pending[which] = true;
        }
    }
};

int nc_selftest_device(nc_ctx *ctx);
void nc_pipe_destroy(nc_ctx *ctx);
```

### nanocaller_amd/csrc/nc_ctx.hip

```cpp
#include <algorithm>
#include <new>
#include <thread>
#include <vector>

#include "nc_common.h"
#include "nc_host.h"

extern "C" {

int nc_abi_version(void) { return NC_ABI_VERSION; }

int nc_device_count(int *n)
{
    if (!n) return NC_ERR_ARG;
    int c = 0;
    hipError_t e = hipGetDeviceCount(&c);
    if (e != hipSuccess) { *n = 0; return NC_ERR_HIP; }
    *n = c;
    return NC_OK;
}

}

namespace {
__global__ void k_copy16(uint4 *__restrict__ dst, const uint4 *__restrict__ src, size_t n16)
{
    for (size_t i = (size_t)blockIdx.x * blockDim.x + threadIdx.x; i < n16; i += (size_t)gridDim.x * blockDim.x) dst[i] = src[i];
    __threadfence_system();
}
__global__ void k_copy4(uint32_t *__restrict__ dst, const uint32_t *__restrict__ src, size_t n4)
{
    for (size_t i = (size_t)blockIdx.x * blockDim.x + threadIdx.x; i < n4; i += (size_t)gridDim.x * blockDim.x) dst[i] = src[i];
    __threadfence_system();
}
__global__ void k_copy1(uint8_t *__restrict__ dst, const uint8_t *__restrict__ src, size_t n)
{
    for (size_t i = (size_t)blockIdx.x * blockDim.x + threadIdx.x; i < n; i += (size_t)gridDim.x * blockDim.x) dst[i] = src[i];
    __threadfence_system();
}

void launch_copy(void *dst, const void *src, size_t bytes, hipStream_t st)
{
    const uintptr_t a = (uintptr_t)dst | (uintptr_t)src | (uintptr_t)bytes;
    if ((a & 15) == 0) {
        const size_t n = bytes / 16;
        hipLaunchKernelGGL(k_copy16, dim3((unsigned)std::min<size_t>((n + 255) / 256, 128)), dim3(256), 0, st, (uint4 *)dst, (const uint4 *)src, n);
    } else if ((a & 3) == 0) {
        const size_t n = bytes / 4;
        hipLaunchKernelGGL(k_copy4, dim3((unsigned)std::min<size_t>((n + 255) / 256, 128)), dim3(256), 0, st, (uint32_t *)dst, (const uint32_t *)src, n);
    } else {
        hipLaunchKernelGGL(k_copy1, dim3((unsigned)std::min<size_t>((bytes + 255) / 256, 128)), dim3(256), 0, st, (uint8_t *)dst, (const uint8_t *)src, bytes);
    }
}
}

int nc_d2h(nc_ctx *ctx, void *host, const void *dev, size_t bytes, hipStream_t st)
{
    if (!bytes) return NC_OK;
    hipPointerAttribute_t at;
    void *alias = nullptr;
    if (hipPointerGetAttributes(&at, host) == hipSuccess && at.type == hipMemoryTypeHost && at.devicePointer) alias = at.devicePointer;
    else (void)hipGetLastError();
    static const size_t kernel_max = [] { const char *e = getenv("NC_D2H_KERNEL_BYTES"); return e ? (size_t)atoll(e) : (size_t)NC_D2H_KERNEL_MAX; }();
    if (!alias || bytes > kernel_max) {
        NC_HIP(ctx, hipMemcpyAsync(host, dev, bytes, hipMemcpyDeviceToHost, st));
        return NC_OK;
    }
    launch_copy(alias, dev, bytes, st);
    NC_HIP(ctx, hipGetLastError());
    return NC_OK;
}

int nc_h2d_small(nc_ctx *ctx, void *dev, const void *host, size_t bytes, hipStream_t st)
{
    if (!bytes) return NC_OK;
    if (bytes > NC_STAGE_SLOT || !ctx->stage_h) {
        NC_HIP(ctx, hipMemcpyAsync(dev, host, bytes, hipMemcpyHostToDevice, st));
        return NC_OK;
    }
    uint8_t *slot = ctx->stage_h + (size_t)(ctx->stage_turn++ % NC_STAGE_SLOTS) * NC_STAGE_SLOT;
    memcpy(slot, host, bytes);
    const size_t padded = (bytes + 15) & ~(size_t)15;
    launch_copy(dev, slot, ((uintptr_t)dev & 15) ? bytes : padded, st);
    NC_HIP(ctx, hipGetLastError());
    return NC_OK;
}

extern "C" {

int nc_d2h_async(nc_ctx *ctx, void *stream, void *host, const void *dev, size_t bytes)
{
    if (!ctx || (bytes && (!host || !dev))) return NC_ERR_ARG;
    return nc_d2h(ctx, host, dev, bytes, stream ? (hipStream_t)stream : ctx->stream);
}

int nc_ctx_create(int device_id, nc_ctx **out)
{
    if (!out) return NC_ERR_ARG;
    *out = nullptr;
    int n = 0;
    if (hipGetDeviceCount(&n) != hipSuccess || n <= 0) return NC_ERR_HIP;
    if (device_id < 0 || device_id >= n) return NC_ERR_ARG;
    nc_ctx *ctx = new (std::nothrow) nc_ctx();
    if (!ctx) return NC_ERR_NOMEM;
    ctx->device = device_id;
    if (hipSetDevice(device_id) != hipSuccess || hipStreamCreate(&ctx->own_stream) != hipSuccess ||
        hipEventCreate(&ctx->ev0) != hipSuccess || hipEventCreate(&ctx->ev1) != hipSuccess) {
        delete ctx;
        return NC_ERR_HIP;
    }
    ctx->stream = ctx->own_stream;
    if (hipHostMalloc((void **)&ctx->mbox, 256, hipHostMallocDefault) != hipSuccess ||
        hipHostMalloc((void **)&ctx->stage_h, (size_t)NC_STAGE_SLOT * NC_STAGE_SLOTS, hipHostMallocDefault) != hipSuccess) {
        nc_ctx_destroy(ctx);
        return NC_ERR_NOMEM;
    }
    int rc = nc_selftest_device(ctx);
    if (rc != NC_OK) {
        fprintf(stderr, "nanocaller_hip: device self-test failed: %s\n", ctx->err);
        nc_ctx_destroy(ctx);
        return rc;
    }
    *out = ctx;
    return NC_OK;
}

int nc_ctx_destroy(nc_ctx *ctx)
{
    if (!ctx) return NC_OK;
    (void)hipSetDevice(ctx->device);
    (void)hipStreamSynchronize(ctx->stream);
    nc_pipe_destroy(ctx);
    for (auto &w : ctx->w) {
        if (w.dev) (void)hipFree(w.dev);
        if (w.packed) (void)hipFree(w.packed);
        if (w.packed_h) (void)hipFree(w.packed_h);
    }
    for (auto &e : ctx->kev) if (e) (void)hipEventDestroy(e);
    for (auto &e : ctx->drain_ev) if (e) (void)hipEventDestroy(e);
    if (ctx->scan_ev) (void)hipEventDestroy(ctx->scan_ev);
    if (ctx->scale_ev) (void)hipEventDestroy(ctx->scale_ev);
    for (auto &p : ctx->tev) for (auto &e : p) if (e) (void)hipEventDestroy(e);
    if (ctx->ev0) (void)hipEventDestroy(ctx->ev0);
    if (ctx->ev1) (void)hipEventDestroy(ctx->ev1);
    if (ctx->own_stream) (void)hipStreamDestroy(ctx->own_stream);
    if (ctx->mbox) (void)hipHostFree(ctx->mbox);
    if (ctx->stage_h) (void)hipHostFree(ctx->stage_h);
    delete ctx;
    return NC_OK;
}

int nc_ctx_set_stream(nc_ctx *ctx, void *hip_stream)
{
    if (!ctx) return NC_ERR_ARG;
    ctx->stream = hip_stream ? (hipStream_t)hip_stream : ctx->own_stream;
    return NC_OK;
}

int nc_ctx_sync(nc_ctx *ctx)
{
    if (!ctx) return NC_ERR_ARG;
    NC_HIP(ctx, hipStreamSynchronize(ctx->stream));
    return NC_OK;
}

const char *nc_last_error(const nc_ctx *ctx) { return ctx ? ctx->err : "null context"; }

int nc_malloc(nc_ctx *ctx, size_t bytes, void **dev)
{
    if (!ctx || !dev) return NC_ERR_ARG;
    NC_HIP(ctx, hipSetDevice(ctx->device));
    hipError_t e = hipMalloc(dev, bytes ? bytes : 16);
    if (e != hipSuccess) return nc_fail(ctx, NC_ERR_NOMEM, "hipMalloc(%zu): %s", bytes, hipGetErrorString(e));
    return NC_OK;
}

int nc_free(nc_ctx *ctx, void *dev)
{
    if (!ctx) return NC_ERR_ARG;
    if (dev) NC_HIP(ctx, hipFree(dev));
    return NC_OK;
}

int nc_memcpy_h2d(nc_ctx *ctx, void *dev, const void *host, size_t bytes)
{
    if (!ctx || (bytes && (!dev || !host))) return NC_ERR_ARG;
    if (bytes) NC_HIP(ctx, hipMemcpyAsync(dev, host, bytes, hipMemcpyHostToDevice, ctx->stream));
    NC_HIP(ctx, hipStreamSynchronize(ctx->stream));
    return NC_OK;
}

int nc_memcpy_d2h(nc_ctx *ctx, void *host, const void *dev, size_t bytes)
{
    if (!ctx || (bytes && (!dev || !host))) return NC_ERR_ARG;
    if (bytes) NC_HIP(ctx, hipMemcpyAsync(host, dev, bytes, hipMemcpyDeviceToHost, ctx->stream));
    NC_HIP(ctx, hipStreamSynchronize(ctx->stream));
    return NC_OK;
}

int nc_set_cnn_precision(nc_ctx *ctx, int exact_fp32)
{
    if (!ctx) return NC_ERR_ARG;
    ctx->cnn_exact_fp32 = exact_fp32 != 0;
    return NC_OK;
}

int nc_set_tensor_format(nc_ctx *ctx, int fmt)
{
    if (!ctx || (fmt != 0 && fmt != 1)) return NC_ERR_ARG;
    ctx->x_i16 = fmt == 1;
    return NC_OK;
}

int nc_enable_timing(nc_ctx *ctx, int on)
{
    if (!ctx) return NC_ERR_ARG;
    if (on && !ctx->timing)
        for (int w = 0; w < 6; w++) { ctx->sum_ms[w] = 0.0; ctx->sum_n[w] = 0; }
    ctx->timing = on == 2 ? 2 : on != 0;
    return NC_OK;
}

void nc_timing_resolve(nc_ctx *ctx, int which)
{
    if (which < 4) {
        if (!ctx->tev_pending[which]) return;
        if (hipEventSynchronize(ctx->tev[which][1]) == hipSuccess &&
            hipEventElapsedTime(&ctx->last_ms[which], ctx->tev[which][0], ctx->tev[which][1]) == hipSuccess) {
            ctx->sum_ms[which] += ctx->last_ms[which];
            ctx->sum_n[which]++;
        }
        ctx->tev_pending[which] = false;
        return;
    }
    if (!ctx->kev_pending) return;
    float tot = 0.0f;
    for (int e = 0; e + 1 < ctx->n_kev; e += 2) {
        float one = 0.0f;
        if (hipEventSynchronize(ctx->kev[e + 1]) == hipSuccess && hipEventElapsedTime(&one, ctx->kev[e], ctx->kev[e + 1]) == hipSuccess) tot += one;
    }
    ctx->last_ms[4] = tot;
    ctx->last_ms[5] = (float)(ctx->n_kev / 2);
    ctx->sum_ms[4] += tot;
    ctx->sum_ms[5] += ctx->n_kev / 2;
    ctx->sum_n[4]++;
    ctx->sum_n[5]++;
    ctx->kev_pending = false;
}

int nc_last_kernel_ms(nc_ctx *ctx, int which, float *ms)
{
    if (!ctx || !ms || which < 0 || which > 5) return NC_ERR_ARG;
    nc_timing_resolve(ctx, which < 4 ? which : 4);
    *ms = ctx->last_ms[which];
    return NC_OK;
}

int nc_timing_sums(nc_ctx *ctx, double *sum_ms, int64_t *count)
{
    if (!ctx || !sum_ms) return NC_ERR_ARG;
    for (int w = 0; w < 5; w++) nc_timing_resolve(ctx, w);
    for (int w = 0; w < 6; w++) {
        sum_ms[w] = ctx->sum_ms[w];
        if (count) count[w] = ctx->sum_n[w];
    }
    return NC_OK;
}

static inline int64_t floor16(int64_t x) { return x & ~int64_t(15); }
static inline int64_t ceil16(int64_t x) { return (x + 15) & ~int64_t(15); }

static bool tile_size_ok(int32_t t) { return t == 1024 || t == 2048 || t == 4096; }

int nc_pack_plan(int32_t n_reads, const int32_t *start, const int32_t *end, const uint8_t *keep,
                 int32_t tile_size, int32_t pos_lo, int32_t pos_hi,
                 int64_t *codes_len, int32_t *tile_pos0, int32_t *n_tiles, int64_t *n_entries)
{
    if (n_reads < 0 || (n_reads && (!start || !end)) || !tile_size_ok(tile_size) || pos_hi < pos_lo ||
        !codes_len || !tile_pos0 || !n_tiles || !n_entries)
        return NC_ERR_ARG;
    int64_t t0 = (int64_t)pos_lo - (((int64_t)pos_lo % tile_size) + tile_size) % tile_size;
    int64_t nt = ((int64_t)pos_hi - t0) / tile_size + 1;
    if (nt > INT32_MAX) return NC_ERR_ARG;
    int64_t bytes = 0, ents = 0;
    int32_t prev = INT32_MIN;
    for (int32_t r = 0; r < n_reads; r++) {
        if (keep && !keep[r]) continue;
        if (end[r] <= start[r]) return NC_ERR_ARG;
        if (start[r] < prev) return NC_ERR_ARG;
        prev = start[r];
        bytes += ceil16(end[r]) - floor16(start[r]);
        int64_t a = std::max<int64_t>(start[r], t0), b = std::min<int64_t>((int64_t)end[r] - 1, t0 + nt * tile_size - 1);
        if (a <= b) ents += (b - t0) / tile_size - (a - t0) / tile_size + 1;
    }
    *codes_len = bytes + 16;
    *tile_pos0 = (int32_t)t0;
    *n_tiles = (int32_t)nt;
    *n_entries = ents;
    return NC_OK;
}

int nc_pack_fill(int32_t n_reads, const int32_t *start, const int32_t *end, const int64_t *off,
                 const uint8_t *codes_in, const uint8_t *strand, const uint8_t *keep,
                 int32_t tile_size, int32_t tile_pos0, int32_t n_tiles,
                 uint8_t *codes_out, int64_t codes_len, int32_t *tile_off, nc_tile_entry *tile_ent,
                 int64_t n_entries)
{
    const bool index_only = !codes_in && !codes_out;
    if (n_reads < 0 || !tile_size_ok(tile_size) || n_tiles <= 0 || !tile_off || (n_entries && !tile_ent) ||
        (n_reads && (!start || !end)) || (!index_only && (!codes_out || (n_reads && (!off || !codes_in)))))
        return NC_ERR_ARG;
    const int64_t t0 = tile_pos0;
    std::vector<int64_t> cnt((size_t)n_tiles + 1, 0);
    for (int32_t r = 0; r < n_reads; r++) {
        if (keep && !keep[r]) continue;
        int64_t a = std::max<int64_t>(start[r], t0), b = std::min<int64_t>((int64_t)end[r] - 1, t0 + (int64_t)n_tiles * tile_size - 1);
        if (a > b) continue;
        for (int64_t t = (a - t0) / tile_size; t <= (b - t0) / tile_size; t++) cnt[(size_t)t + 1]++;
    }
    for (int32_t t = 0; t < n_tiles; t++) cnt[(size_t)t + 1] += cnt[(size_t)t];
    if (cnt[(size_t)n_tiles] != n_entries || n_entries > INT32_MAX) return NC_ERR_CAPACITY;
    for (int32_t t = 0; t <= n_tiles; t++) tile_off[t] = (int32_t)cnt[(size_t)t];
    std::vector<int64_t> cur(cnt.begin(), cnt.end() - 1);
    std::vector<int64_t> base((size_t)(n_reads > 0 ? n_reads : 1), 0);
    int64_t w = 0;
    for (int32_t r = 0; r < n_reads; r++) {
        if (keep && !keep[r]) { base[(size_t)r] = -1; continue; }
        const int64_t lo = floor16(start[r]), hi = ceil16(end[r]);
        if (w + (hi - lo) > codes_len) return NC_ERR_CAPACITY;
        base[(size_t)r] = w - lo;
        w += hi - lo;
        nc_tile_entry e;
        e.start = start[r];
        e.end = end[r];
        e.base_flag = base[(size_t)r] | (strand ? (strand[r] & 15) : 0);
        int64_t a = std::max<int64_t>(start[r], t0), b = std::min<int64_t>((int64_t)end[r] - 1, t0 + (int64_t)n_tiles * tile_size - 1);
        if (a > b) continue;
        for (int64_t t = (a - t0) / tile_size; t <= (b - t0) / tile_size; t++) tile_ent[cur[(size_t)t]++] = e;
    }
    if (!index_only) {
        const int hw = nc_host_cpus();
        int T = hw > 32 ? 32 : hw;
        if (n_reads < 4096) T = 1;
        auto fill = [&](int32_t r0, int32_t r1, int64_t out0, int64_t out1) {
            memset(codes_out + out0, NC_CODE_ABSENT, (size_t)(out1 - out0));
            for (int32_t r = r0; r < r1; r++)
                if (!(keep && !keep[r]))
                    memcpy(codes_out + base[(size_t)r] + start[r], codes_in + off[r], (size_t)(end[r] - start[r]));
        };
        auto slot0 = [&](int32_t r) { return base[(size_t)r] + floor16(start[r]); };
        std::vector<int32_t> cut((size_t)T + 1, n_reads);
        cut[0] = 0;
        for (int t = 1; t < T; t++) {
            int32_t r = (int32_t)((int64_t)n_reads * t / T);
            while (r < n_reads && keep && !keep[r]) r++;
            cut[(size_t)t] = r;
        }
        std::vector<std::thread> th;
        for (int t = 0; t < T; t++) {
            const int32_t r0 = cut[(size_t)t], r1 = cut[(size_t)t + 1];
            const int64_t out0 = t == 0 ? 0 : (r0 < n_reads ? slot0(r0) : w);
            const int64_t out1 = t + 1 == T ? codes_len : (r1 < n_reads ? slot0(r1) : w);
            if (out1 <= out0 && r1 <= r0) continue;
            if (T == 1) fill(r0, r1, out0, out1);
            else th.emplace_back(fill, r0, r1, out0, out1);
        }
        for (auto &x : th) x.join();
    }
    return NC_OK;
}

}
```

### nanocaller_amd/engine.py

```python
from __future__ import annotations

import ctypes as C
import os
import weakref
from dataclasses import dataclass

import numpy as np
import torch

from . import _lib
from .pack import HostPack
from .weights import Weights


def _ptr(t):
    return C.c_void_p(t.data_ptr()) if t is not None else None


@dataclass
class DevicePack:
    codes: torch.Tensor
    tile_off: torch.Tensor
    tile_ent: torch.Tensor
    ref_code: torch.Tensor
    tile_size: int
    tile_pos0: int
    n_tiles: int
    n_entries: int
    pos_lo: int
    pos_hi: int
    events: dict | None = None
    reads: dict | None = None
    indel: dict | None = None
    mates: tuple | None = None
    records: tuple | None = None

    def c_struct(self) -> _lib.ReadPackC:
        return _lib.ReadPackC(codes_len=self.codes.numel(), codes=self.codes.data_ptr(), tile_size=self.tile_size,
                              tile_pos0=self.tile_pos0, n_tiles=self.n_tiles, tile_off=self.tile_off.data_ptr(),
                              tile_ent=self.tile_ent.data_ptr(), n_entries=self.n_entries)

    @property
    def nbytes(self):
        return self.codes.numel() + self.tile_off.numel() * 4 + self.tile_ent.numel() + self.ref_code.numel()


@dataclass
class SnpSites:
    n_sites: int
    n_nbr: int
    pos: np.ndarray
    chunk: np.ndarray
    dp: np.ndarray
    alt: np.ndarray
    x: torch.Tensor | None = None
    ref_code: torch.Tensor | None = None
    fwd_dp: torch.Tensor | None = None
    rev_dp: torch.Tensor | None = None
    depth: torch.Tensor | None = None
    valid: torch.Tensor | None = None


class _PinnedPool:

    def __init__(self):
        self.blocks = []

    def get(self, shape, dtype):
        shape = tuple(int(v) for v in (shape if isinstance(shape, (tuple, list, torch.Size)) else (shape,)))
        nbytes = int(np.prod(shape, dtype=np.int64)) * torch.empty(0, dtype=dtype).element_size()
        best = None
        for b in self.blocks:
            if (b[1] is None or b[1]() is None) and b[0].numel() >= nbytes and (best is None or b[0].numel() < best[0].numel()):
                best = b
        if best is None:
            cap = max(4096, nbytes + nbytes // 4)
            best = [torch.empty(cap, dtype=torch.uint8, pin_memory=True), None]
            self.blocks.append(best)
        t = best[0][:nbytes].view(dtype).view(shape)
        arr = t.numpy()
        best[1] = weakref.ref(arr)
        return t, arr


class Engine:

    def __init__(self, device: int = 0):
        if not torch.cuda.is_available():
            raise _lib.NanoCallerHipError("no ROCm device visible: the NanoCaller HIP path has no CPU fallback")
        self.L = _lib.lib()
        self.device = torch.device("cuda", device)
        torch.cuda.set_device(self.device)
        ctx = C.c_void_p()
        rc = self.L.nc_ctx_create(device, C.byref(ctx))
        if rc != _lib.NC_OK:
            raise _lib.NanoCallerHipError("nc_ctx_create(device=%d) failed with status %d" % (device, rc))
        self.ctx = ctx
        self._loaded = {}
        self._pinned = _PinnedPool()
        self.use_torch_stream()

    def close(self):
        if getattr(self, "ctx", None):
            self.L.nc_ctx_destroy(self.ctx)
            self.ctx = None

    def __del__(self):
        try:
            self.close()
        except Exception:
            pass

    def _check(self, rc, what):
        if rc != _lib.NC_OK:
            msg = self.L.nc_last_error(self.ctx)
            raise _lib.NanoCallerHipError("%s failed (%d): %s" % (what, rc, msg.decode() if msg else ""))

    def use_torch_stream(self):
        import os
        s = torch.cuda.current_stream(self.device)
        if s.cuda_stream == 0 and os.environ.get("NC_ONE_QUEUE", "1") != "0":
            if getattr(self, "_tstream", None) is None:
                self._tstream = torch.cuda.Stream(device=self.device)
            self._tstream.wait_stream(s)
            torch.cuda.set_stream(self._tstream)
            s = self._tstream
        self._check(self.L.nc_ctx_set_stream(self.ctx, C.c_void_p(s.cuda_stream)), "nc_ctx_set_stream")

    def _adopt_thread(self):
        import os
        s = torch.cuda.current_stream(self.device)
        if s.cuda_stream == 0 and os.environ.get("NC_ONE_QUEUE", "1") != "0" and getattr(self, "_tstream", None) is not None:
            self._tstream.wait_stream(s)
            torch.cuda.set_stream(self._tstream)

    def set_cnn_precision(self, exact_fp32: bool):
        self._check(self.L.nc_set_cnn_precision(self.ctx, 1 if exact_fp32 else 0), "nc_set_cnn_precision")
        self.exact_fp32 = bool(exact_fp32)

    def set_tensor_format(self, int16: bool):
        self._check(self.L.nc_set_tensor_format(self.ctx, 1 if int16 else 0), "nc_set_tensor_format")
        self.x_int16 = bool(int16)

    TRUNK_KERNELS = {0: "k4_conv12", 2: "k5_trunk_p3", 3: "k5_trunk_lin"}

    def trunk_info(self):
        n, k = C.c_int32(), C.c_int32()
        self._check(self.L.nc_snp_trunk_info(self.ctx, C.byref(n), C.byref(k)), "nc_snp_trunk_info")
        return int(n.value), self.TRUNK_KERNELS[int(k.value)]

    def trunk_mfma_per_site(self) -> int:
        return self.trunk_info()[0]

    def enable_timing(self, on=True, trunk_only=False):
        self._check(self.L.nc_enable_timing(self.ctx, (2 if trunk_only else 1) if on else 0), "nc_enable_timing")

    def last_ms(self, which):
        ms = C.c_float()
        self._check(self.L.nc_last_kernel_ms(self.ctx, which, C.byref(ms)), "nc_last_kernel_ms")
        return float(ms.value)

    def timing_sums(self):
        sums, cnt = np.zeros(6, np.float64), np.zeros(6, np.int64)
        self._check(self.L.nc_timing_sums(self.ctx, _lib.npp(sums), _lib.npp(cnt)), "nc_timing_sums")
        return sums, cnt

    def upload(self, hp: HostPack) -> DevicePack:
        dev = self.device
        ent_bytes = np.frombuffer(hp.tile_ent.tobytes(), np.uint8) if hp.tile_ent.size else np.zeros(16, np.uint8)
        dp = DevicePack(codes=torch.from_numpy(hp.codes).to(dev), tile_off=torch.from_numpy(hp.tile_off).to(dev),
                        tile_ent=torch.from_numpy(ent_bytes.copy()).to(dev), ref_code=torch.from_numpy(hp.ref_code).to(dev),
                        tile_size=hp.tile_size, tile_pos0=hp.tile_pos0, n_tiles=hp.n_tiles,
                        n_entries=int(hp.tile_ent.shape[0]), pos_lo=hp.pos_lo, pos_hi=hp.pos_hi)
        if hp.mates is not None:
            dp.mates = (torch.from_numpy(hp.mates[0]).to(dev), torch.from_numpy(hp.mates[1]).to(dev))
        if hp.ev_off is not None:
            z = lambda a, dt: torch.from_numpy(np.ascontiguousarray(a, dt) if a.size else np.zeros(1, dt)).to(dev)
            dp.events = dict(n_reads=int(hp.read_hap.shape[0]), ev_off=z(hp.ev_off, np.int32), ev_pos=z(hp.ev_pos, np.int32),
                             ev_len=z(hp.ev_len, np.int32), read_hap=z(hp.read_hap, np.uint8))
        return dp

    def load_weights(self, kind: int, w: Weights):
        if self._loaded.get(kind) == w.path:
            return
        if w.kind != kind:
            raise ValueError("weights %s are of kind %d, expected %d" % (w.path, w.kind, kind))
        flat = np.ascontiguousarray(w.flat, np.float32)
        self._check(self.L.nc_load_weights(self.ctx, kind, _lib.npp(flat), flat.size), "nc_load_weights")
        self._loaded[kind] = w.path

    def snp_scan(self, dp: DevicePack, chunks, *, mincov, min_allele_freq, threshold, haploid=False, async_fetch=False, between=None) -> SnpSites:
        cs = np.ascontiguousarray([c[0] for c in chunks], np.int32)
        ce = np.ascontiguousarray([c[1] for c in chunks], np.int32)
        scan_lo = max(1, int(cs.min()) - _lib.FLANK)
        scan_hi = int(ce.max()) + _lib.FLANK
        if scan_lo < dp.pos_lo or min(scan_hi, dp.pos_hi) < scan_lo:
            pass
        params = _lib.ScanParamsC(mincov=int(mincov), min_allele_freq=float(min_allele_freq), nbr_t0=float(threshold[0]),
                                  nbr_t1=float(threshold[1]), haploid=1 if haploid else 0)
        pc = dp.c_struct()
        self._check(self.L.nc_snp_scan_begin(self.ctx, C.byref(pc), _ptr(dp.ref_code), dp.tile_pos0, dp.ref_code.numel(), scan_lo,
                                             scan_hi, C.byref(params), len(chunks), _lib.npp(cs), _lib.npp(ce)), "nc_snp_scan_begin")
        if between is not None:
            between()
        n_nbr, n_cand, n_sites = C.c_int32(), C.c_int32(), C.c_int32()
        self._check(self.L.nc_snp_scan_end(self.ctx, C.byref(n_nbr), C.byref(n_cand), C.byref(n_sites)), "nc_snp_scan_end")
        N = n_sites.value
        hb, h = self._pinned.get((4, max(N, 1)), torch.int32)
        ptr = [C.c_void_p(hb[i].data_ptr()) for i in range(4)]
        if async_fetch:
            self._check(self.L.nc_snp_scan_fetch_async(self.ctx, self._copy_stream_ptr(), None, ptr[0], ptr[1], ptr[2], ptr[3]),
                        "nc_snp_scan_fetch_async")
        else:
            self._check(self.L.nc_snp_scan_fetch(self.ctx, None, ptr[0], ptr[1], ptr[2], ptr[3]), "nc_snp_scan_fetch")
        return SnpSites(n_sites=N, n_nbr=n_nbr.value, pos=h[0, :N], chunk=h[1, :N], dp=h[2, :N], alt=h[3, :N])

    def fetch_nbr_sites(self, n_nbr) -> np.ndarray:
        out = np.empty(n_nbr, np.int32)
        self._check(self.L.nc_snp_scan_fetch(self.ctx, _lib.npp(out), None, None, None, None), "nc_snp_scan_fetch")
        return out

    def snp_featurize(self, dp: DevicePack, sites: SnpSites, *, seq, maxcov, min_nbr_sites=1) -> SnpSites:
        N = sites.n_sites
        dev = self.device
        if dp.mates is not None and not getattr(self, "x_int16", False):
            self.set_tensor_format(int16=True)
            try:
                self.snp_featurize(dp, sites, seq=seq, maxcov=maxcov, min_nbr_sites=min_nbr_sites)
            finally:
                self.set_tensor_format(int16=False)
            sites.x = sites.x.to(torch.float32)
            return sites
        i16 = getattr(self, "x_int16", False)
        xb = N * 1025 * (2 if i16 else 4)
        a16 = lambda v: (v + 15) & ~15
        o_ref = a16(xb); o_fwd = a16(o_ref + 4 * N); o_rev = a16(o_fwd + 16 * N); o_dep = a16(o_rev + 16 * N); o_val = a16(o_dep + 4 * N)
        buf = torch.empty(o_val + N + 16, dtype=torch.uint8, device=dev)
        sites.x = buf[:xb].view(torch.int16 if i16 else torch.float32).view(N, 5, 41, 5)
        sites.ref_code = buf[o_ref:o_ref + 4 * N].view(torch.int32)
        sites.fwd_dp = buf[o_fwd:o_fwd + 16 * N].view(torch.int32).view(N, 4)
        sites.rev_dp = buf[o_rev:o_rev + 16 * N].view(torch.int32).view(N, 4)
        sites.depth = buf[o_dep:o_dep + 4 * N].view(torch.int32)
        sites.valid = buf[o_val:o_val + N]
        pc = dp.c_struct()
        if dp.mates is not None:
            self._check(self.L.nc_snp_set_mates(self.ctx, int(dp.mates[0].numel()), _ptr(dp.mates[0]), _ptr(dp.mates[1])), "nc_snp_set_mates")
        try:
            self._check(self.L.nc_snp_featurize(self.ctx, C.byref(pc), _ptr(dp.ref_code), dp.tile_pos0, dp.ref_code.numel(),
                                                _lib.SEQ_MODES[seq], int(maxcov), int(min_nbr_sites), _ptr(sites.x),
                                                _ptr(sites.ref_code), _ptr(sites.fwd_dp), _ptr(sites.rev_dp), _ptr(sites.depth),
                                                _ptr(sites.valid)), "nc_snp_featurize")
        finally:
            if dp.mates is not None:
                self.L.nc_snp_set_mates(self.ctx, 0, None, None)
        return sites

    def snp_scale(self, sites: SnpSites, n_chunks, train_coverage, per_site=False, async_fetch=False):
        scale = torch.empty(sites.n_sites, dtype=torch.float64, device=self.device)
        if not async_fetch:
            cd = np.zeros(n_chunks, np.float64)
            self._check(self.L.nc_snp_scale(self.ctx, _ptr(sites.depth), _ptr(sites.valid), float(train_coverage),
                                            1 if per_site else 0, _ptr(scale), _lib.npp(cd)), "nc_snp_scale")
            return scale, cd
        hb, cd = self._pinned.get((max(int(n_chunks), 1),), torch.float64)
        self._check(self.L.nc_snp_scale(self.ctx, _ptr(sites.depth), _ptr(sites.valid), float(train_coverage),
                                        1 if per_site else 0, _ptr(scale), None), "nc_snp_scale")
        self._check(self.L.nc_snp_chunk_depth_async(self.ctx, self._copy_stream_ptr(), C.c_void_p(hb.data_ptr())), "nc_snp_chunk_depth_async")
        return scale, cd[:int(n_chunks)]

    def x_limit(self, kind) -> float:
        v = C.c_float()
        self._check(self.L.nc_cnn_x_limit(self.ctx, kind, C.byref(v)), "nc_cnn_x_limit")
        return float(v.value)

    def snp_forward_guarded(self, kind, x, ref_code, scale, scale_mode=0):
        n = int(x.shape[0])
        flags = torch.zeros(max(n, 1), dtype=torch.uint8, device=self.device)
        probs, gt = self.snp_forward(kind, x, ref_code, scale, scale_mode, range_flags=flags)
        idx = torch.nonzero(flags[:n]).squeeze(1)
        if idx.numel():
            self.range_rerun(kind, x, ref_code, scale, scale_mode, idx, probs, gt)
        return probs, gt, int(idx.numel())

    def range_rerun(self, kind, x, ref_code, scale, scale_mode, idx, probs, gt):
        was_exact, was_i16 = getattr(self, "exact_fp32", False), getattr(self, "x_int16", False)
        xs = x[idx].to(torch.float32).contiguous()
        self.set_tensor_format(int16=False)
        self.set_cnn_precision(exact_fp32=True)
        try:
            p2, g2 = self.snp_forward(kind, xs, ref_code[idx].contiguous(), scale[idx].contiguous() if scale is not None else None, scale_mode,
                                      want_gt=gt is not None)
        finally:
            self.set_cnn_precision(exact_fp32=was_exact)
            self.set_tensor_format(int16=was_i16)
        probs[idx] = p2
        if gt is not None and g2 is not None:
            gt[idx] = g2

    def snp_forward(self, kind, x, ref_code, scale, scale_mode=0, want_gt=True, drain=False, range_flags=None):
        n = int(x.shape[0])
        if range_flags is not None:
            self._check(self.L.nc_cnn_range_watch(self.ctx, C.c_void_p(range_flags.data_ptr())), "nc_cnn_range_watch")
        try:
            return self._snp_forward(kind, x, ref_code, scale, scale_mode, want_gt, drain, n)
        finally:
            if range_flags is not None:
                self.L.nc_cnn_range_watch(self.ctx, None)

    def _snp_forward(self, kind, x, ref_code, scale, scale_mode, want_gt, drain, n):
        probs = torch.empty((n, 4), dtype=torch.float32, device=self.device)
        gt = torch.empty((n, 2), dtype=torch.float32, device=self.device) if (want_gt and kind == _lib.MODEL_SNP) else None
        if not drain:
            self._check(self.L.nc_snp_forward(self.ctx, kind, n, _ptr(x), _ptr(ref_code), _ptr(scale), int(scale_mode),
                                              _ptr(probs), _ptr(gt)), "nc_snp_forward")
            return probs, gt
        hp, hp_np = self._pinned.get((n, 4), torch.float32)
        hg, hg_np = self._pinned.get((n, 2), torch.float32) if gt is not None else (None, None)
        self._check(self.L.nc_snp_forward_drain(self.ctx, kind, n, _ptr(x), _ptr(ref_code), _ptr(scale), int(scale_mode),
                                                _ptr(probs), _ptr(gt), self._copy_stream_ptr(), C.c_void_p(hp.data_ptr()),
                                                C.c_void_p(hg.data_ptr()) if hg is not None else None), "nc_snp_forward_drain")
        return probs, gt, hp_np, hg_np

    def indel_forward(self, kind, x):
        n = int(x.shape[0])
        nout = 4 if kind == _lib.MODEL_INDEL else 1
        probs = torch.empty((n, nout), dtype=torch.float32, device=self.device)
        self._check(self.L.nc_indel_forward(self.ctx, kind, n, _ptr(x), _ptr(probs)), "nc_indel_forward")
        return probs

    def snp_phase(self, site_pos, site_alleles, read_group, n_groups, *, max_cov=15, reads=None, csr=None, realign=None, site_gt=None,
                  distrust_cost=1, weights=None, bam_quals=None) -> dict:
        L = self.L
        pos = np.ascontiguousarray(site_pos, np.int32)
        h = C.c_void_p()
        if realign is not None:
            codes, reads_c, n_events, n_ins, ref_code = realign
            al = np.ascontiguousarray(site_alleles, np.uint8).reshape(-1, 2)
            torch.cuda.current_stream(self.device).synchronize()
            rc = L.nc_snp_phase_realign(self.ctx, _ptr(codes), codes.numel(), C.byref(reads_c), int(n_events), int(n_ins), _ptr(ref_code),
                                        int(ref_code.numel()), pos.size, _lib.npp(pos), _lib.npp(al), C.byref(h))
            self._check(rc, "nc_snp_phase_realign")
        elif reads is not None:
            codes, rs, re_, so = reads
            al = np.ascontiguousarray(site_alleles, np.uint8).reshape(-1, 2)
            torch.cuda.current_stream(self.device).synchronize()
            rc = L.nc_snp_phase_gather(self.ctx, _ptr(codes), codes.numel(), int(rs.numel()), _ptr(rs), _ptr(re_), _ptr(so), pos.size, _lib.npp(pos),
                                       _lib.npp(al), C.byref(h))
            self._check(rc, "nc_snp_phase_gather")
        else:
            off, site, allele = (np.ascontiguousarray(a, t) for a, t in zip(csr, (np.int64, np.int32, np.uint8)))
            self._check(L.nc_snp_phase_load(self.ctx, off.size - 1, pos.size, _lib.npp(pos), _lib.npp(off), _lib.npp(site), _lib.npp(allele),
                                            C.byref(h)), "nc_snp_phase_load")
        try:
            if weights is not None and bam_quals is not None:
                raise ValueError("snp_phase: weights= and bam_quals= are two sources of the same weights")
            if weights is not None:
                ew, ok = (None if a is None else np.ascontiguousarray(a, np.uint8) for a in weights)
                v = _lib.PhaseArraysC()
                L.nc_snp_phase_view(h, C.byref(v))
                if (ew is not None and ew.size != v.n_entries) or (ok is not None and ok.size != v.n_reads):
                    raise ValueError("snp_phase: weights= holds %s weights / %s flags for %d entries / %d reads"
                                     % (None if ew is None else ew.size, None if ok is None else ok.size, v.n_entries, v.n_reads))
                self._check(L.nc_snp_phase_set_weights(self.ctx, h, None if ew is None else _lib.npp(ew), None if ok is None else _lib.npp(ok)),
                            "nc_snp_phase_set_weights")
            if bam_quals is not None:
                raw, rec_off, mapq_min, default_weight, w_max = bam_quals
                v = _lib.PhaseArraysC()
                L.nc_snp_phase_view(h, C.byref(v))
                if rec_off.dtype != torch.int64 or rec_off.numel() != v.n_reads or raw.dtype != torch.uint8:
                    raise ValueError("snp_phase: bam_quals= needs a uint8 record stream and %d int64 record offsets, one per read" % v.n_reads)
                torch.cuda.current_stream(self.device).synchronize()
                self._check(L.nc_snp_phase_weights_from_bam(self.ctx, h, _ptr(raw), int(raw.numel()), _ptr(rec_off), int(mapq_min), int(default_weight),
                                                            int(w_max)), "nc_snp_phase_weights_from_bam")
            if site_gt is None:
                self._check(L.nc_snp_phase_solve(self.ctx, h, int(max_cov)), "nc_snp_phase_solve")
            else:
                gt = np.ascontiguousarray(site_gt, np.uint8)
                if gt.shape != pos.shape:
                    raise ValueError("snp_phase: site_gt holds %d classes for %d sites" % (gt.size, pos.size))
                self._check(L.nc_snp_phase_solve_gt(self.ctx, h, int(max_cov), _lib.npp(gt), int(distrust_cost)), "nc_snp_phase_solve_gt")
            grp = np.ascontiguousarray(read_group, np.int32)
            self._check(L.nc_haplotag_run(self.ctx, h, int(n_groups), _lib.npp(grp)), "nc_haplotag_run")
            v = _lib.PhaseArraysC()
            L.nc_snp_phase_view(h, C.byref(v))

            def a(ptr, n, dt):
                return np.ctypeslib.as_array(C.cast(ptr, C.POINTER(np.ctypeslib.as_ctypes_type(dt))), (n,)).copy() if n and ptr else np.zeros(0, dt)
            R, S, nb, ng = v.n_reads, v.n_sites, v.n_blocks, v.n_groups
            extra = {}
            if site_gt is not None:
                g = C.c_void_p()
                L.nc_snp_phase_genotypes(h, C.byref(g))
                extra = dict(site_gt=a(g, S, np.uint8))
            if weights is not None or bam_quals is not None:
                pw, pm, po = C.c_void_p(), C.c_void_p(), C.c_void_p()
                L.nc_snp_phase_weights(h, C.byref(pw), C.byref(pm), C.byref(po))
                extra.update(entry_weight=a(pw, v.n_entries, np.uint8), read_mapq=a(pm, R, np.uint8), read_ok=a(po, R, np.uint8))
            return dict(entry_off=a(v.entry_off, R + 1, np.int64), entry_site=a(v.entry_site, v.n_entries, np.int32),
                        entry_allele=a(v.entry_allele, v.n_entries, np.uint8), side=a(v.read_side, R, np.int8),
                        site_block=a(v.site_block, S, np.int32), site_h=a(v.site_h, S, np.uint8), site_phased=a(v.site_phased, S, np.uint8).astype(bool),
                        site_ps=a(v.site_ps, S, np.int32), block_first=a(v.block_first, nb, np.int32), block_last=a(v.block_last, nb, np.int32),
                        block_ps=a(v.block_ps, nb, np.int32), block_cost=a(v.block_cost, nb, np.int64), group_hp=a(v.group_hp, ng, np.uint8),
                        group_ps=a(v.group_ps, ng, np.int32), ms=dict(zip(("gather", "select", "dp", "haplotag"), list(v.ms))), **extra)
        finally:
            L.nc_snp_phase_free(h)

    def bam_retag_sizes(self, raw, rec_off, thash, tps, new_size, tag_idx, out_off, status, raw_byte_off=0):
        self._check(self.L.nc_bam_retag_sizes(self.ctx, C.c_void_p(raw.data_ptr() + raw_byte_off), int(rec_off.numel()), _ptr(rec_off),
                                              _ptr(thash) if thash.numel() else None, _ptr(tps) if tps.numel() else None, int(thash.numel()),
                                              _ptr(new_size), _ptr(tag_idx), _ptr(out_off), _ptr(status)), "nc_bam_retag_sizes")

    def bam_retag(self, raw, rec_off, thp, tps, tag_idx, out_off, out, out_byte_off=0, raw_byte_off=0):
        self._check(self.L.nc_bam_retag(self.ctx, C.c_void_p(raw.data_ptr() + raw_byte_off), int(rec_off.numel()), _ptr(rec_off),
                                        _ptr(thp) if thp.numel() else None, _ptr(tps) if tps.numel() else None, _ptr(tag_idx), _ptr(out_off),
                                        C.c_void_p(out.data_ptr() + out_byte_off)), "nc_bam_retag")

    def bgzf_deflate(self, data, ioff, ilen, out, ooff, clen, status, crc=None):
        self._check(self.L.nc_bgzf_deflate_device(self.ctx, int(ioff.numel()), _ptr(data), _ptr(ioff), _ptr(ilen), _ptr(out), _ptr(ooff), _ptr(clen),
                                                  _ptr(crc), _ptr(status)), "nc_bgzf_deflate_device")

    def bgzf_crc32(self, data, ioff, ilen, crc):
        self._check(self.L.nc_bgzf_crc32_device(self.ctx, int(ioff.numel()), _ptr(data), _ptr(ioff), _ptr(ilen), _ptr(crc)), "nc_bgzf_crc32_device")

    def bgzf_assemble(self, pay, poff, clen, crc, isize, foff, file=None):
        self._check(self.L.nc_bgzf_assemble_device(self.ctx, int(clen.numel()), _ptr(pay), _ptr(poff), _ptr(clen), _ptr(crc), _ptr(isize), _ptr(foff),
                                                   _ptr(file)), "nc_bgzf_assemble_device")

    def fasta_decode(self, raw, first, length, linebases, linewidth, *, letters=None, scan=None, scan_pos0=1, ga=1, gb=None, blind=None, status=None,
                     raw_len=None):
        if status is None:
            status = torch.empty(1, dtype=torch.int32, device=self.device)
        rc = self.L.nc_fasta_decode(self.ctx, _ptr(raw), int(raw.numel() if raw_len is None else raw_len), int(first), int(length), int(linebases),
                                    int(linewidth), _ptr(letters), _ptr(scan), int(scan_pos0), 0 if scan is None else int(scan.numel()), int(ga),
                                    int(length if gb is None else gb), _ptr(blind), _ptr(status))
        self._check(rc, "nc_fasta_decode")

    def indel_scan(self, dp: DevicePack, start, end, *, mincov, win_size, small_win_size, ins_t, del_t, excl=None, haploid=False, impute=False):
        if dp.events is None:
            raise ValueError("this read pack carries no indel events / haplotype tags")
        ev = dp.events
        evc = _lib.IndelEventsC(n_reads=ev["n_reads"], ev_off=ev["ev_off"].data_ptr(), ev_pos=ev["ev_pos"].data_ptr(),
                                ev_len=ev["ev_len"].data_ptr(), read_hap=ev["read_hap"].data_ptr())
        prm = _lib.IndelScanParamsC(mincov=int(mincov), win_size=int(win_size), small_win_size=int(small_win_size),
                                    ins_t=float(ins_t), del_t=float(del_t), haploid=1 if haploid else 0, impute=1 if impute else 0)
        lo = max(1, int(start))
        out = np.empty(int(end) - lo + 1, np.int8)
        pc = dp.c_struct()
        self._check(self.L.nc_indel_scan(self.ctx, C.byref(pc), C.byref(evc), _ptr(excl), lo, int(end), C.byref(prm),
                                         _lib.npp(out)), "nc_indel_scan")
        return out

    def indel_scan_batch(self, dp: DevicePack, chunks, *, mincov, win_size, small_win_size, ins_t, del_t, excl=None, haploid=False, impute=False):
        if dp.events is None:
            raise ValueError("this read pack carries no indel events / haplotype tags")
        ev = dp.events
        evc = _lib.IndelEventsC(n_reads=ev["n_reads"], ev_off=ev["ev_off"].data_ptr(), ev_pos=ev["ev_pos"].data_ptr(),
                                ev_len=ev["ev_len"].data_ptr(), read_hap=ev["read_hap"].data_ptr())
        prm = _lib.IndelScanParamsC(mincov=int(mincov), win_size=int(win_size), small_win_size=int(small_win_size),
                                    ins_t=float(ins_t), del_t=float(del_t), haploid=1 if haploid else 0, impute=1 if impute else 0)
        starts = np.ascontiguousarray([c[0] for c in chunks], np.int32)
        ends = np.ascontiguousarray([c[1] for c in chunks], np.int32)
        ncol = ends.astype(np.int64) - np.maximum(starts, 1) + 1
        off = np.zeros(len(chunks) + 1, np.int64)
        np.cumsum(ncol, out=off[1:])
        out = np.empty(int(off[-1]), np.int8)
        pc = dp.c_struct()
        self._check(self.L.nc_indel_scan_batch(self.ctx, C.byref(pc), C.byref(evc), _ptr(excl), len(chunks), _lib.npp(starts),
                                               _lib.npp(ends), C.byref(prm), _lib.npp(out), _lib.npp(off)), "nc_indel_scan_batch")
        return [out[off[k]:off[k + 1]] for k in range(len(chunks))]

    def star_msa_tensor(self, read_sets, refs, *, open_=None, extend=None, match=None, mismatch=None, max_cols=None, want_rows=False, cns_as_str=False):
        S = len(read_sets)
        if S == 0:
            x = torch.empty((0, 5, 128, 2), dtype=torch.float32, device=self.device)
            return (x, [], np.zeros(0, np.int32)) + (([], []) if want_rows else ())
        n_reads = np.fromiter(map(len, read_sets), np.int64, S)
        set0 = np.zeros(S + 1, np.int32)
        np.cumsum(n_reads, out=set0[1:])
        flat = [q for rs in read_sets for q in rs]
        rlen = np.fromiter(map(len, flat), np.int64, len(flat))
        read_off = np.zeros(len(flat) + 1, np.int32)
        np.cumsum(rlen, out=read_off[1:])
        reflen = np.fromiter(map(len, refs), np.int64, S)
        ref_off = np.zeros(S + 1, np.int32)
        np.cumsum(reflen, out=ref_off[1:])
        raw_reads, raw_refs = "".join(flat).encode(), "".join(refs).encode()
        per_set = np.zeros(S, np.int64)
        nz = n_reads > 0
        if len(flat):
            per_set[nz] = np.add.reduceat(rlen, set0[:-1][nz])
        cap = reflen + per_set
        mc = int(max_cols) if max_cols else int(cap.max())
        return self.star_msa_tensor_flat(S, raw_reads, read_off, set0, raw_refs, ref_off, mc, open_=open_, extend=extend, match=match,
                                         mismatch=mismatch, want_rows=want_rows, cns_as_str=cns_as_str, _n_reads=n_reads, _cap=cap)

    def star_msa_tensor_flat(self, S, reads, read_off, set_read0, refs, ref_off, max_cols, *, open_=None, extend=None, match=None, mismatch=None,
                             want_rows=False, cns_as_str=False, _n_reads=None, _cap=None, al_dup=None):
        open_, extend, match, mismatch = [d if v is None else v for v, d in zip((open_, extend, match, mismatch), _lib.STAR_SCORING)]
        x = torch.empty((S, 5, 128, 2), dtype=torch.float32, device=self.device)
        mc = int(max_cols)
        cns = np.empty((S, mc), np.uint8)
        ncols = np.empty(S, np.int32)
        ptr = lambda a: _lib.npp(a) if isinstance(a, np.ndarray) else a
        rows = rr = roff = rroff = None
        if want_rows:
            roff = np.zeros(S + 1, np.int64)
            np.cumsum(_n_reads * _cap, out=roff[1:])
            rroff = np.zeros(S + 1, np.int64)
            np.cumsum(_cap, out=rroff[1:])
            rows, rr = np.empty(max(int(roff[-1]), 1), np.uint8), np.empty(max(int(rroff[-1]), 1), np.uint8)
        self._check(self.L.nc_star_msa_tensor_dup(self.ctx, S, reads, ptr(read_off), ptr(set_read0), refs, ptr(ref_off),
                                                  int(open_), int(extend), int(match), int(mismatch), mc, _ptr(x), _lib.npp(cns), _lib.npp(ncols),
                                                  _lib.npp(rows), _lib.npp(roff), _lib.npp(rr), _lib.npp(rroff), ptr(al_dup)), "nc_star_msa_tensor")
        if int(ncols.max()) > mc and not want_rows:
            return self.star_msa_tensor_flat(S, reads, read_off, set_read0, refs, ref_off, int(ncols.max()), open_=open_, extend=extend,
                                             match=match, mismatch=mismatch, cns_as_str=cns_as_str, al_dup=al_dup)
        if cns_as_str:
            cut = np.empty(S + 1, np.int64)
            flat = np.empty(max(S * mc, 1), np.uint8)
            self._check(self.L.nc_consensus_strings(_lib.npp(cns), S, mc, _lib.npp(ncols), _lib.npp(flat), _lib.npp(cut)), "nc_consensus_strings")
            cl = cut.tolist()
            big = flat[:cl[-1]].tobytes().decode("ascii")
            out_cns = [big[a:b] for a, b in zip(cl, cl[1:])]
        else:
            keep = (np.arange(mc, dtype=np.int32)[None, :] < np.minimum(ncols, mc)[:, None]) & (cns != 4)
            cnt = keep.sum(1)
            cut = np.zeros(S + 1, np.int64)
            np.cumsum(cnt, out=cut[1:])
            flat_cns = cns[keep]
            out_cns = [flat_cns[cut[k]:cut[k + 1]] for k in range(S)]
        if not want_rows:
            return x, out_cns, ncols
        out_rows = [rows[roff[s]:roff[s] + int(_n_reads[s]) * int(ncols[s])].reshape(int(_n_reads[s]), int(ncols[s])) for s in range(S)]
        out_rr = [rr[rroff[s]:rroff[s] + int(ncols[s])] for s in range(S)]
        return x, out_cns, ncols, out_rows, out_rr

    def indel_tensor(self, rows_list, ref_rows_list):
        S = len(rows_list)
        dev = self.device
        n_rows = np.array([r.shape[0] for r in rows_list], np.int32)
        n_cols = np.array([r.shape[1] for r in rows_list], np.int32)
        row_off = np.zeros(S, np.int64)
        ref_off = np.zeros(S, np.int64)
        if S:
            np.cumsum((n_rows.astype(np.int64) * n_cols)[:-1], out=row_off[1:])
            np.cumsum(n_cols.astype(np.int64)[:-1], out=ref_off[1:])
        max_cols = max(128, int(n_cols.max()) if S else 128)
        rows = np.concatenate([np.ascontiguousarray(r, np.uint8).ravel() for r in rows_list]) if S else np.zeros(1, np.uint8)
        refs = np.concatenate([np.ascontiguousarray(r, np.uint8).ravel() for r in ref_rows_list]) if S else np.zeros(1, np.uint8)
        t = lambda a: torch.from_numpy(a).to(dev)
        d_rows, d_refs, d_ro, d_fo, d_nr, d_nc = t(rows), t(refs), t(row_off), t(ref_off), t(n_rows), t(n_cols)
        x = torch.empty((S, 5, 128, 2), dtype=torch.float32, device=dev)
        cns = torch.empty((S, max_cols), dtype=torch.uint8, device=dev)
        self._check(self.L.nc_indel_tensor(self.ctx, S, _ptr(d_rows), _ptr(d_ro), _ptr(d_nr), _ptr(d_nc), _ptr(d_refs),
                                           _ptr(d_fo), max_cols, _ptr(x), _ptr(cns)), "nc_indel_tensor")
        cns_h = cns.cpu().numpy()
        out = []
        for s in range(S):
            row = cns_h[s, :n_cols[s]]
            out.append(row[row != 4])
        return x, out

    def to_host(self, tensors):
        outs = []
        for t in tensors:
            if t is None:
                outs.append(None)
                continue
            h, h_np = self._pinned.get(t.shape, t.dtype)
            h.copy_(t, non_blocking=True)
            outs.append(h_np)
        torch.cuda.current_stream(self.device).synchronize()
        return outs

    def _copy_stream(self):
        if getattr(self, "_cstream", None) is None:
            self._cstream = torch.cuda.Stream(device=self.device)
        return self._cstream

    def _copy_stream_ptr(self):
        return C.c_void_p(self._copy_stream().cuda_stream)

    def to_host_async(self, tensors):
        cs = self._copy_stream()
        ev = torch.cuda.Event()
        ev.record(torch.cuda.current_stream(self.device))
        cs.wait_event(ev)
        outs = []
        with torch.cuda.stream(cs):
            for t in tensors:
                if t is None:
                    outs.append(None)
                    continue
                h, h_np = self._pinned.get(t.shape, t.dtype)
                t = t.contiguous()
                self._check(self.L.nc_d2h_async(self.ctx, C.c_void_p(cs.cuda_stream), C.c_void_p(h.data_ptr()), C.c_void_p(t.data_ptr()),
                                                t.numel() * t.element_size()), "nc_d2h_async")
                t.record_stream(cs)
                outs.append(h_np)
        return outs

    def copy_event(self):
        ev = torch.cuda.Event()
        ev.record(self._copy_stream())
        return ev

    def wait_copies(self):
        self._copy_stream().synchronize()

    def sync(self):
        torch.cuda.synchronize(self.device)


_engines = {}


def get_engine(device: int = 0) -> Engine:
    if device not in _engines:
        _engines[device] = Engine(device)
    else:
        _engines[device]._adopt_thread()
    return _engines[device]


def local_device(devices=None, rank=0) -> int:
    import os
    local = int(os.environ.get("LOCAL_RANK", rank))
    if devices:
        return int(devices[local % len(devices)])
    n = torch.cuda.device_count() if torch.cuda.is_available() else 0
    return local % n if n > 0 else 0
```

### nanocaller_amd/snpCaller.py

```python
from __future__ import annotations

import datetime
import os
import queue
import shutil
import struct
import sys
import zlib

import numpy as np
import torch

from . import _lib
from .engine import get_engine
from .generate_SNP_pileups import device_pack_for, release_contig
from .weights import Weights, get_SNP_model

num_to_base_map = {0: 'A', 1: 'G', 2: 'T', 3: 'C'}
_B = "AGTC"


def _qual(p, cap=99.0, mult=-10.0):
    return min(cap, mult * np.log10(1e-10 + 1 - float(p)))


def snp_vcf_lines(chrom, pos, ref_idx, probs, dp, freq, fwd_dp, rev_dp):
    probs = np.asarray(probs, np.float32)
    order = np.argsort(probs, axis=1)
    k = np.sum(probs >= 0.5, axis=1)
    out = []
    for j in range(len(pos)):
        pr = probs[j]
        info = 'PR=' + ','.join("{:.4f}".format(x) for x in pr[[0, 3, 1, 2]]) + ";FQ={:.4f}".format(freq[j])
        r = int(ref_idx[j])
        d = int(dp[j])
        ref_dp = (fwd_dp[j][r], rev_dp[j][r])
        p1, p2 = int(order[j, -1]), int(order[j, -2])
        head = '%s\t%d\t.\t%s\t' % (chrom, pos[j], _B[r])
        fmt = 'GT:DP:VF:AD:ADF:ADR'
        if k[j] >= 2:
            if p1 == r:
                a = (fwd_dp[j][p2], rev_dp[j][p2])
                out.append(head + '%s\t%.3f\t%s\t%s\t%s\t%s:%d:%.4f:%d,%d:%d,%d:%d,%d\n' % (
                    _B[p2], _qual(pr[p2]), 'PASS', info, fmt, '0/1', d, sum(a) / d, sum(ref_dp), sum(a), ref_dp[0], a[0],
                    ref_dp[1], a[1]))
            elif p2 == r and pr[p2] >= 0.5:
                a = (fwd_dp[j][p1], rev_dp[j][p1])
                out.append(head + '%s\t%.3f\t%s\t%s\t%s\t%s:%d:%.4f:%d,%d:%d,%d:%d,%d\n' % (
                    _B[p1], _qual(pr[p2]), 'PASS', info, fmt, '0/1', d, sum(a) / d, sum(ref_dp), sum(a), ref_dp[0], a[0],
                    ref_dp[1], a[1]))
            elif p2 != r and p1 != r and pr[p2] >= 0.5:
                a1 = (fwd_dp[j][p1], rev_dp[j][p1])
                a2 = (fwd_dp[j][p2], rev_dp[j][p2])
                out.append(head + '%s,%s\t%.3f\t%s\t%s\t%s\t%s:%d:%.4f,%.4f:%d,%d,%d:%d,%d,%d:%d,%d,%d\n' % (
                    _B[p1], _B[p2], _qual(pr[p2]), 'PASS', info, fmt, '1/2', d, sum(a1) / d, sum(a2) / d, sum(ref_dp),
                    sum(a1), sum(a2), ref_dp[0], a1[0], a2[0], ref_dp[1], a1[1], a2[1]))
        elif k[j] == 1 and r != p1 and pr[p1] >= 0.5:
            a = (fwd_dp[j][p1], rev_dp[j][p1])
            out.append(head + '%s\t%.3f\t%s\t%s\t%s\t%s:%d:%.4f:%d,%d:%d,%d:%d,%d\n' % (
                _B[p1], _qual(pr[p1]), 'PASS', info, fmt, '1/1', d, sum(a) / d, sum(ref_dp), sum(a), ref_dp[0], a[0],
                ref_dp[1], a[1]))
        elif k[j] == 1 and r == p1:
            out.append(head + '%s\t%.3f\t%s\t%s\t%s\t%s:%d:.:.:.:.\n' % ('.', _qual(pr[p1]), 'REF', info, fmt, './.', d))
        else:
            out.append(head + '%s\t%.3f\t%s\t%s\t%s\t%s:%d:.:.:.:.\n' % ('.', 0, 'LOW', info, fmt, './.', d))
    return out


def snp_vcf_lines_haploid(chrom, pos, ref_idx, probs, dp, freq):
    probs = np.asarray(probs, np.float32)
    pred = np.argmax(probs, 1)
    out = []
    for j in range(len(pos)):
        pr = probs[j]
        p = int(pred[j])
        r = int(ref_idx[j])
        info = 'PR=' + ','.join("{:.4f}".format(x) for x in pr[[0, 3, 1, 2]]) + ";FQ={:.4f}".format(freq[j])
        out.append('%s\t%d\t.\t%s\t%s\t%.3f\t%s\t%s\tGT:DP:VF:AD:ADF:ADR\t%s:%d:%.4f:.:.:.\n' % (
            chrom, pos[j], _B[r], _B[p], _qual(pr[p], 999.0, -100.0), 'PASS' if p != r else 'REF', info, '1/1', int(dp[j]),
            freq[j]))
    return out


def argsort4(probs):
    import ctypes as C
    L = _lib.lib()
    probs = np.ascontiguousarray(probs, np.float32)
    n = probs.shape[0]
    order = np.empty((n, 4), np.int32)
    ties = np.empty(max(n, 1), np.int64)
    nt = C.c_int64()
    rc = L.nc_argsort4(_lib.npp(probs), n, _lib.npp(order), C.byref(nt), _lib.npp(ties), ties.size)
    if rc != _lib.NC_OK:
        raise _lib.NanoCallerHipError("nc_argsort4 failed (%d)" % rc)
    if nt.value:
        t = ties[:nt.value]
        order[t] = np.argsort(probs[t], axis=1)
    return order


def snp_vcf_text(chrom, pos, ref_idx, probs, dp, freq, fwd_dp=None, rev_dp=None, haploid=False, as_array=False, out=None):
    import ctypes as C
    L = _lib.lib()
    n = len(pos)
    i32 = lambda a: np.ascontiguousarray(a, np.int32)
    probs = np.ascontiguousarray(probs, np.float32)
    order = None if haploid else argsort4(probs)
    pos_, ref_, dp_ = i32(pos), i32(ref_idx), i32(dp)
    freq_ = np.ascontiguousarray(freq, np.float64)
    fwd_ = None if haploid else i32(fwd_dp)
    rev_ = None if haploid else i32(rev_dp)
    cap = (400 + len(chrom)) * max(n, 1) + 1024
    if out is None or out.size < cap:
        out = np.empty(cap, np.uint8)
    cap = out.size
    nb = C.c_int64()
    rc = L.nc_snp_vcf_format(chrom.encode(), n, _lib.npp(pos_), _lib.npp(ref_), _lib.npp(probs), _lib.npp(order),
                             _lib.npp(dp_), _lib.npp(freq_), _lib.npp(fwd_), _lib.npp(rev_), 1 if haploid else 0,
                             _lib.npp(out), cap, C.byref(nb))
    if rc != _lib.NC_OK:
        raise _lib.NanoCallerHipError("nc_snp_vcf_format failed (%d)" % rc)
    return out[:nb.value] if as_array else out[:nb.value].tobytes()


VCF_HEADER = (
    '##fileformat=VCFv4.2\n'
    '##FILTER=<ID=PASS,Description="All filters passed">\n'
    '##FILTER=<ID=LOW,Description="All alleles have probability less than 50%.">\n'
    '##FILTER=<ID=REF,Description="Homozygous Reference. Only reference allele has greater than 50% probability. '
    'All alternative alleles having probability less than 50%.">\n'
    '{contigs}'
    '##FORMAT=<ID=GT,Number=1,Type=String,Description="Genotype">\n'
    '##FORMAT=<ID=DP,Number=1,Type=Integer,Description="Depth">\n'
    '##FORMAT=<ID=AD,Number=R,Type=Integer,Description="Allelic depths for the ref and alt alleles in the order listed">\n'
    '##FORMAT=<ID=ADF,Number=R,Type=Integer,Description="Allelic depths on forward strand for the ref and alt alleles in the order listed">\n'
    '##FORMAT=<ID=ADR,Number=R,Type=Integer,Description="Allelic depths on reverse strand for the ref and alt alleles in the order listed">\n'
    '##FORMAT=<ID=VF,Number=A,Type=Float,Description="Alternative allele frequency in the order listed">\n'
    '##INFO=<ID=PR,Number=4,Type=Float,Description="Probability of presence of alleles A, C, G and T, in the given order. '
    'Probability of each base is out of 1, independent of each other.">\n'
    '##INFO=<ID=FQ,Number=1,Type=Float,Description="Maximum frequency of non-reference base.">\n'
    '#CHROM\tPOS\tID\tREF\tALT\tQUAL\tFILTER\tINFO\tFORMAT\t{sample}\n')


PARAM_KEYS = frozenset(['chunks_list', 'regions_list', 'sam_path', 'fasta_path', 'mincov', 'maxcov', 'min_allele_freq', 'min_nbr_sites',
                        'threshold', 'snp_model', 'vcf_path', 'prefix', 'sample', 'seq', 'supplementary', 'exclude_bed',
                        'suppress_progress', 'disable_coverage_normalization'])

_WEIGHTS = {}


def _weights(path):
    if path not in _WEIGHTS:
        _WEIGHTS[path] = Weights(path)
    return _WEIGHTS[path]


class PendingCall:

    def __init__(self, finish):
        self._finish, self._res = finish, None

    def result(self):
        if self._finish is not None:
            self._res, self._finish = self._finish(), None
        return self._res


_PENDING_CNN = {}


def flush_pending_cnn(device=0):
    f = _PENDING_CNN.pop(device, None)
    if f is not None:
        f()


def call_chunks(params, chunks, device=0, dpk=None, defer=False, pipeline=None):
    if pipeline is None:
        pipeline = bool(defer) and os.environ.get('NC_PIPE_CNN', '0') == '1'
    if not pipeline:
        flush_pending_cnn(device)
    chrom = chunks[0]['chrom']
    ploidy = chunks[0]['ploidy']
    assert all(c['chrom'] == chrom and c['ploidy'] == ploidy for c in chunks)
    eng = get_engine(device)
    eng.use_torch_stream()
    if ploidy == 'diploid':
        path, train_cov = get_SNP_model(params['snp_model'])
        if path is None:
            print('Invalid SNP model name or path', flush=True)
            sys.exit(1)
        kind = _lib.MODEL_SNP
    else:
        path, _ = get_SNP_model('haploid')
        train_cov = 30
        kind = _lib.MODEL_SNP_HAP
    eng.load_weights(kind, _weights(path))
    if dpk is None:
        from .generate_SNP_pileups import contig_span
        dpk = device_pack_for(params, chrom, device, span=contig_span(params['sam_path'], chrom, chunks))
    sites = eng.snp_scan(dpk, [(c['start'], c['end']) for c in chunks], mincov=params['mincov'],
                         min_allele_freq=params['min_allele_freq'], threshold=params['threshold'],
                         haploid=(ploidy == 'haploid'), async_fetch=True, between=(lambda: flush_pending_cnn(device)) if pipeline else None)
    res = dict(chrom=chrom, ploidy=ploidy, n=0)
    if sites.n_sites == 0:
        eng.wait_copies()
        return PendingCall(lambda: res) if defer else res
    eng.set_tensor_format(int16=not getattr(eng, "exact_fp32", False))
    eng.snp_featurize(dpk, sites, seq=params['seq'], maxcov=params['maxcov'], min_nbr_sites=params['min_nbr_sites'])
    all_valid = bool(sites.valid.all().item()) if params['min_nbr_sites'] > 1 else True
    per_site = bool(params.get('disable_coverage_normalization'))
    scale, chunk_depth = eng.snp_scale(sites, len(chunks), train_cov, per_site=per_site, async_fetch=True)
    scan_copied = eng.copy_event()
    h_ref, h_fwd, h_rev, h_valid = eng.to_host_async([sites.ref_code, sites.fwd_dp, sites.rev_dp, None if all_valid else sites.valid])
    guard = not getattr(eng, "exact_fp32", False)
    i16 = not getattr(eng, "exact_fp32", False)
    eng.set_tensor_format(int16=False)
    cnn = {}

    def enqueue_cnn():
        eng.use_torch_stream()
        eng.set_tensor_format(int16=i16)
        try:
            flags_ = torch.zeros(sites.n_sites, dtype=torch.uint8, device=eng.device) if guard else None
            cnn['d_probs'], cnn['d_gt'], cnn['h_probs'], cnn['h_gt'] = eng.snp_forward(kind, sites.x, sites.ref_code, scale, scale_mode=1 if per_site else 0,
                                                                                   drain=True, range_flags=flags_)
            cnn['flags'] = flags_
            cnn['h_nflag'] = eng.to_host_async([flags_.sum(dtype=torch.int32).reshape(1)])[0] if guard else None
        finally:
            eng.set_tensor_format(int16=False)
        cnn['drained'] = eng.copy_event()
    if pipeline:
        _PENDING_CNN[device] = enqueue_cnn
    else:
        enqueue_cnn()
    scan_copied.synchronize()
    freq = sites.alt.astype(np.float64) / sites.dp.astype(np.float64)
    keep_alive = (sites, scale, cnn)

    def finish():
        nonlocal keep_alive
        if 'drained' not in cnn:
            if _PENDING_CNN.get(device) is enqueue_cnn:
                flush_pending_cnn(device)
            else:
                enqueue_cnn()
        drained, h_nflag, flags, d_probs, d_gt, h_probs, h_gt = (cnn[k] for k in ('drained', 'h_nflag', 'flags', 'd_probs', 'd_gt', 'h_probs', 'h_gt'))
        drained.synchronize()
        n_rerun = int(h_nflag[0]) if h_nflag is not None else 0
        if n_rerun:
            idx = torch.nonzero(flags).squeeze(1)
            eng.use_torch_stream()
            eng.range_rerun(kind, sites.x, sites.ref_code, scale, 1 if per_site else 0, idx, d_probs, d_gt)
            ih = idx.cpu().numpy()
            h_probs[ih] = d_probs[idx].cpu().numpy()
            if h_gt is not None and d_gt is not None:
                h_gt[ih] = d_gt[idx].cpu().numpy()
        res['range_reruns'] = n_rerun
        keep_alive = None
        out = dict(pos=sites.pos, chunk=sites.chunk, ref=h_ref, probs=h_probs, gt=h_gt, dp=sites.dp, alt=sites.alt,
                   fwd_dp=h_fwd, rev_dp=h_rev, freq=freq)
        if not all_valid:
            m = h_valid.astype(bool)
            out = {k: (v[m] if v is not None else None) for k, v in out.items()}
        res.update(out, n=int(out['pos'].shape[0]), chunk_depth=chunk_depth)
        return res
    return PendingCall(finish) if defer else finish()


def _prepare_wire(params, chrom, grp):
    from .generate_SNP_pileups import _check_supported, _exclude_rows, _resolve, contig_span
    from .wire import build_wire_from_world
    span = contig_span(params['sam_path'], chrom, grp)
    world = _resolve(params['sam_path'], chrom, params.get('fasta_path'), span)
    _check_supported(world, params['sam_path'], chrom, bool(params.get('supplementary')), by_name=True)
    kw = dict(pos_lo=span[0], pos_hi=span[1]) if span else {}
    return build_wire_from_world(world, supplementary=bool(params.get('supplementary')), exclude=_exclude_rows(params, chrom), **kw)


def _prepare_device(dbam, params, chrom, grp, ref=None):
    from .device_fasta import reference_for
    from .generate_SNP_pileups import _exclude_rows
    length = dbam.ref_lengths[dbam.ref_names.index(chrom)] if chrom in dbam.ref_names else 0
    lo = max(1, min(c['start'] for c in grp) - _lib.FLANK)
    hi = min(length, max(c['end'] for c in grp) + _lib.FLANK)
    span = None if (hi - lo + 1) >= 0.9 * length else (lo, hi)
    ref = ref.result() if ref is not None else reference_for(params['fasta_path'], chrom, dbam.device, params)
    return dbam.prepare(chrom, ref, supplementary=bool(params.get('supplementary')), exclude=_exclude_rows(params, chrom), span=span, by_name=True)


def caller(params, chunks_Q, counter_Q, snp_files, device=0, worker_id=1):
    curr_vcf_path = os.path.join(params['intermediate_snp_files_dir'], '%s.%d.snps.vcf' % (params['prefix'], worker_id))
    snp_files.append(curr_vcf_path)
    chunks = []
    while True:
        try:
            chunks.append(chunks_Q.get(block=False))
        except queue.Empty:
            break
        except Exception:
            if chunks_Q.empty():
                break
            raise
    groups = {}
    for c in chunks:
        groups.setdefault((c['chrom'], c['ploidy']), []).append(c)
    from concurrent.futures import ThreadPoolExecutor

    scratch = [None]

    def emit(f, chrom, ploidy, r, grp):
        if r['n']:
            need = (400 + len(chrom)) * r['n'] + 1024
            if scratch[0] is None or scratch[0].size < need:
                scratch[0] = np.empty(need + need // 4, np.uint8)
            f.write(snp_vcf_text(chrom, r['pos'], r['ref'], r['probs'], r['dp'], r['freq'], r['fwd_dp'], r['rev_dp'],
                                 haploid=(ploidy != 'diploid'), as_array=True, out=scratch[0]))
        f.flush()
        os.fsync(f.fileno())
        for _ in grp:
            counter_Q.put(1)

    with open(curr_vcf_path, 'wb') as f, ThreadPoolExecutor(max_workers=1) as pool:
        pending, in_flight = None, []

        def collect():
            nonlocal pending
            chrom, ploidy, call, grp, gi = in_flight.pop(0)
            r = call.result()
            if pending is not None:
                pending.result()
            pending = pool.submit(emit, f, chrom, ploidy, r, grp)
            if last_use[chrom] == gi:
                if piped:
                    prep_pool.submit(release_contig, chrom)
                else:
                    release_contig(chrom)
        keys = list(groups)
        last_use = {chrom: i for i, (chrom, _) in enumerate(keys)}
        for k in keys:
            groups[k].sort(key=lambda c: c['start'])
        piped = isinstance(params['sam_path'], str) and os.path.exists(params['sam_path']) and not os.environ.get('NC_SERIAL_INGEST')
        uploader = None
        preps = []
        dev_codes, refs = [None], {}
        run_end, run_dev = [len(keys)] * len(keys), [None] * len(keys)
        if piped and keys and params.get('device_ingest', os.environ.get('NC_DEVICE_INGEST', '1') != '0') and params.get('fasta_path'):
            from .device_bam import DeviceIngestUnavailable, ensure_index, open_device_bam, plan_shares
            from .device_fasta import reference_for
            ensure_index(params['sam_path'], params, device)
            try:
                lim = os.environ.get('NC_DEVICE_INGEST_SHARE_GB')
                order = list(dict.fromkeys(k[0] for k in keys))
                share_of = {}
                for n_sh, (cs, fits) in enumerate(plan_shares(params['sam_path'], order, None if lim is None else int(float(lim) * (1 << 30)), device=device)):
                    for c in cs:
                        share_of[c] = (n_sh, tuple(cs) if fits else None)
                a0 = 0
                for j in range(1, len(keys) + 1):
                    if j == len(keys) or share_of[keys[j][0]][0] != share_of[keys[a0][0]][0]:
                        for q in range(a0, j):
                            run_end[q], run_dev[q] = j, share_of[keys[a0][0]][1]
                        a0 = j
            except DeviceIngestUnavailable:
                pass
        dbam, prepare, nxt = None, None, 0
        depth = max(1, int(os.environ.get('NC_CALLER_DEPTH', 2 if piped else 1)))
        if piped and keys:
            ahead = int(os.environ.get('NC_INGEST_AHEAD', 2))
            prep_pool = ThreadPoolExecutor(max_workers=max(1, ahead))

        def enter_run(i):
            nonlocal dbam, prepare, uploader, nxt
            dbam = None
            prepare = None
            if i > 0 and run_dev[i - 1] is not None:
                from .device_bam import release as _release_device_bam
                get_engine(device).sync()
                _release_device_bam(params['sam_path'])
            if run_dev[i] is not None:
                ref_pool = ThreadPoolExecutor(max_workers=2)
                for k in keys[i:min(run_end[i], i + 3)]:
                    refs.setdefault(k[0], ref_pool.submit(reference_for, params['fasta_path'], k[0], device, params))
                try:
                    dbam = open_device_bam(params['sam_path'], device, contigs=list(run_dev[i]))
                except DeviceIngestUnavailable:
                    dbam = None
                ref_pool.shutdown(wait=False)
            if dbam is not None:
                db = dbam
                prepare = lambda chrom, grp: _prepare_device(db, params, chrom, grp, refs.pop(chrom, None))
            else:
                prepare = lambda chrom, grp: _prepare_wire(params, chrom, grp)
                if uploader is None:
                    from .wire import WireUploader
                    uploader = WireUploader(get_engine(device))
            nxt = i
            while nxt < run_end[i] and len(preps) < max(1, ahead):
                preps.append(prep_pool.submit(prepare, keys[nxt][0], groups[keys[nxt]]))
                nxt += 1
        for i, (chrom, ploidy) in enumerate(keys):
            grp = groups[(chrom, ploidy)]
            if piped:
                if i == 0 or run_end[i - 1] == i:
                    enter_run(i)
                wp = preps.pop(0).result()
                if nxt < run_end[i]:
                    preps.append(prep_pool.submit(prepare, keys[nxt][0], groups[keys[nxt]]))
                    nxt += 1
                if dbam is not None:
                    if dev_codes[0] is None or dev_codes[0].numel() < wp['codes_len']:
                        dev_codes[0] = torch.empty(wp['codes_len'] + wp['codes_len'] // 8, dtype=torch.uint8, device=get_engine(device).device)
                    call = call_chunks(params, grp, device, dpk=dbam.pack(wp, codes=dev_codes[0]), defer=True)
                else:
                    tk = uploader.submit(wp)
                    call = call_chunks(params, grp, device, dpk=uploader.expand(tk), defer=True)
                    uploader.release(tk)
            else:
                call = call_chunks(params, grp, device, defer=True)
            in_flight.append((chrom, ploidy, call, grp, i))
            while len(in_flight) > depth:
                collect()
        while in_flight:
            collect()
        if pending is not None:
            pending.result()
        if piped and keys:
            prep_pool.shutdown(wait=True)
        if dbam is not None:
            from .device_bam import release as release_device_bam
            dbam = None
            release_device_bam(params['sam_path'])
            from .device_fasta import release as release_device_fasta
            release_device_fasta(params['fasta_path'])


def bgzf_write(path, data: bytes):
    from . import vcfio
    vcfio.bgzf_write(path, data)


def _sort_key(line, order):
    f = line.split('\t', 2)
    return (order.get(f[0], 1 << 30), int(f[1]))


def call_manager(params, devices=None):
    from . import shard
    from .engine import local_device
    import torch.distributed as dist
    rank, world = (dist.get_rank(), dist.get_world_size()) if (dist.is_available() and dist.is_initialized()) else (0, 1)
    if world > 1:
        from .numa import bind_rank
        bind_rank(local_device(devices, rank))
    chunks_Q = queue.Queue()
    counter_Q = queue.Queue()
    snp_files = []
    from .device_bam import ensure_index
    ensure_index(params.get('sam_path'), params, local_device(devices, rank), collective=True)
    wts = shard.depth_weights(params.get('sam_path'), params['chunks_list']) if world > 1 else None
    for chunk in shard.shard_chunks(params['chunks_list'], rank, world, wts):
        chunks_Q.put(chunk)
    params['intermediate_snp_files_dir'] = os.path.join(params['vcf_path'], 'intermediate_snp_files')
    if rank == 0:
        if os.path.exists(params['intermediate_snp_files_dir']):
            shutil.rmtree(params['intermediate_snp_files_dir'])
        os.makedirs(params['intermediate_snp_files_dir'])
    shard.barrier()
    caller(params, chunks_Q, counter_Q, snp_files, device=local_device(devices, rank), worker_id=rank + 1)
    shard.barrier()
    all_path_ = os.path.join(params['vcf_path'], '%s.snps.vcf.gz' % params['prefix'])
    if rank != 0:
        shard.barrier()
        return all_path_
    snp_files = [os.path.join(params['intermediate_snp_files_dir'], '%s.%d.snps.vcf' % (params['prefix'], r + 1))
                 for r in range(world)]
    all_path = os.path.join(params['vcf_path'], '%s.unfiltered.snps.vcf.gz' % params['prefix'])
    pass_path = os.path.join(params['vcf_path'], '%s.snps.vcf.gz' % params['prefix'])
    if not params.get('suppress_progress'):
        print('\n%s: Combining SNP calls.' % str(datetime.datetime.now()))
    contigs = []
    for x in params['regions_list']:
        if x[0] not in contigs:
            contigs.append(x[0])
    header = VCF_HEADER.format(contigs=''.join('##contig=<ID=%s>\n' % c for c in contigs), sample=params['sample'])
    lines = []
    for fn in snp_files:
        with open(fn) as fd:
            lines.extend(fd.readlines())
    order = {c: i for i, c in enumerate(contigs)}
    keyed = []
    for ln in lines:
        f = ln.split('\t', 7)
        keyed.append((order.get(f[0], 1 << 30), int(f[1]), len(f[3]), f[6] == 'PASS', ln))
    keyed.sort(key=lambda k: (k[0], k[1]))
    from . import vcfio
    for path, recs in ((all_path, keyed), (pass_path, [k for k in keyed if k[3]])):
        body = ''.join(k[4] for k in recs).encode()
        vcfio.write_vcf_gz_with_csi(path, header, body, contigs, np.array([k[0] for k in recs], np.int64),
                                    np.array([k[1] for k in recs], np.int64), np.array([k[2] for k in recs], np.int64),
                                    np.array([len(k[4].encode()) for k in recs], np.int64))
    shard.barrier()
    return pass_path
```

Measured before the change: 61.21 million.

## Split SNP CNN into trunk and deferred tail overlapped on a side stream

```diff
diff --git a/include/nanocaller_hip.h b/include/nanocaller_hip.h
--- a/include/nanocaller_hip.h
+++ b/include/nanocaller_hip.h
@@ -212,6 +212,11 @@
 int nc_snp_forward_drain(nc_ctx *ctx, int32_t model_kind, int64_t n, const float *x_dev, const int32_t *ref_code_dev,
                          const double *scale_dev, int32_t scale_mode, float *probs_dev, float *gt_dev,
                          void *copy_stream, float *probs_host, float *gt_host);
+typedef struct nc_snp_tail nc_snp_tail;
+int nc_snp_trunk_phase(nc_ctx *ctx, int32_t model_kind, int64_t n, const float *x_dev, const int32_t *ref_code_dev,
+                       const double *scale_dev, int32_t scale_mode, float *probs_dev, float *gt_dev,
+                       void *side_stream, float *probs_host, float *gt_host, nc_snp_tail **tail);
+int nc_snp_tail_enqueue(nc_ctx *ctx, nc_snp_tail *tail, void *side_stream, void *start_event);
 int nc_cnn_x_limit(nc_ctx *ctx, int32_t model_kind, float *x_limit);
 int nc_cnn_range_watch(nc_ctx *ctx, uint8_t *site_flags_dev);
 int nc_snp_trunk_info(nc_ctx *ctx, int32_t *mfma_per_site, int32_t *kernel_id);
diff --git a/nanocaller_amd/_lib.py b/nanocaller_amd/_lib.py
--- a/nanocaller_amd/_lib.py
+++ b/nanocaller_amd/_lib.py
@@ -28,7 +28,7 @@
     "nc_enable_timing", "nc_pack_plan", "nc_pack_fill", "nc_snp_scan", "nc_snp_scan_begin", "nc_snp_scan_end", "nc_snp_scan_fetch", "nc_snp_featurize",
     "nc_snp_scale", "nc_load_weights", "nc_snp_forward", "nc_indel_forward", "nc_indel_tensor", "nc_indel_scan",
     "nc_bam_open", "nc_bam_close", "nc_bam_n_refs", "nc_bam_ref", "nc_bam_error", "nc_bam_decode", "nc_decoded_view",
-    "nc_decoded_free", "nc_snp_vcf_format", "nc_set_cnn_precision", "nc_snp_scan_fetch_async", "nc_snp_forward_drain", "nc_argsort4", "nc_indel_slices", "nc_slices_view", "nc_slices_free",
+    "nc_decoded_free", "nc_snp_vcf_format", "nc_set_cnn_precision", "nc_snp_scan_fetch_async", "nc_snp_forward_drain", "nc_snp_trunk_phase", "nc_snp_tail_enqueue", "nc_argsort4", "nc_indel_slices", "nc_slices_view", "nc_slices_free",
     "nc_nw_cigar", "nc_allele_prediction", "nc_bgzf_compress", "nc_bam_set_threads", "nc_indel_scan_batch", "nc_timing_sums", "nc_snp_chunk_depth_async", "nc_bam_decode_regions", "nc_star_msa", "nc_star_msa_tensor", "nc_star_msa_tensor_dup", "nc_set_tensor_format", "nc_allele_prediction_batch", "nc_allele_prediction_device", "nc_bgzf_read_file", "nc_consensus_strings",
     "nc_wire_build", "nc_wire_build_del", "nc_wire_apply_deletions", "nc_wire_ref_unpack", "nc_wire_view", "nc_wire_free", "nc_wire_expand", "nc_wire_expand_del", "nc_snp_set_mates", "nc_indel_set_mates", "nc_decoded_name_groups", "nc_wire_ins_unpack", "nc_indel_events_pack8", "nc_indel_events_expand8", "nc_wire_build2", "nc_wire_expand2", "nc_d2h_async",
     "nc_indel_pass2_sets", "nc_pass2_view", "nc_pass2_free",
@@ -170,6 +170,8 @@
         L.nc_load_weights.argtypes = [vp, i32, vp, C.c_size_t]
         L.nc_snp_forward.argtypes = [vp, i32, i64, vp, vp, vp, i32, vp, vp]
         L.nc_snp_forward_drain.argtypes = [vp, i32, i64, vp, vp, vp, i32, vp, vp, vp, vp, vp]
+        L.nc_snp_trunk_phase.argtypes = [vp, i32, i64, vp, vp, vp, i32, vp, vp, vp, vp, vp, C.POINTER(vp)]
+        L.nc_snp_tail_enqueue.argtypes = [vp, vp, vp, vp]
         L.nc_indel_forward.argtypes = [vp, i32, i64, vp, vp]
         L.nc_indel_tensor.argtypes = [vp, i32, vp, vp, vp, vp, vp, vp, i32, vp, vp]
         L.nc_indel_scan.argtypes = [vp, C.POINTER(ReadPackC), C.POINTER(IndelEventsC), vp, i32, i32, C.POINTER(IndelScanParamsC), vp]
diff --git a/nanocaller_amd/csrc/nc_cnn.h b/nanocaller_amd/csrc/nc_cnn.h
--- a/nanocaller_amd/csrc/nc_cnn.h
+++ b/nanocaller_amd/csrc/nc_cnn.h
@@ -82,6 +82,19 @@
 std::vector<float> nc_cnn_pack_k4(const float *blob);
 std::vector<uint8_t> nc_cnn_pack_snp_h3(const float *blob);
 
+struct SnpBatch {
+    const float *a3 = nullptr;
+    float *f1 = nullptr;
+    bool fp32 = false;
+};
+struct nc_snp_tail {
+    int32_t kind = 0;
+    int64_t n = 0;
+    const int32_t *ref_code = nullptr;
+    float *probs = nullptr, *gt = nullptr, *probs_host = nullptr, *gt_host = nullptr;
+    SnpBatch batch[NC_SNP_SLOTS];
+};
+
 void nc_cnn_launch_fc1_fp32(hipStream_t st, int F, const float *a3, int K, const float *kf, const float *bf, float *f1, int64_t nb);
 
 void nc_cnn_launch_indel_convs_fp32(hipStream_t st, int H, const float *x, const float *w, float *a1, float *a2, float *a3, int64_t nb);
diff --git a/nanocaller_amd/csrc/nc_cnn.hip b/nanocaller_amd/csrc/nc_cnn.hip
--- a/nanocaller_amd/csrc/nc_cnn.hip
+++ b/nanocaller_amd/csrc/nc_cnn.hip
@@ -1,4 +1,5 @@
 #include <algorithm>
+#include <new>
 
 #include "nc_cnn.h"
 
@@ -91,14 +92,15 @@
 
 const size_t NPARAM[4] = {109370, 108308, 634420, 158185};
 
-int run_snp_trunk(nc_ctx *ctx, const nc_weights &w, int64_t s0, int64_t nb, const void *x_dev, const double *scale, int scale_mode, const float **f1_out, const float **tail)
-{
-    constexpr int64_t n3 = 3 * 9 * 64, F = 48;
-    NC_TRY(nc_ensure(ctx, ctx->cnn_c, (size_t)(nb * (n3 + F)) * 4 + 64));
-    float *a3 = (float *)ctx->cnn_c.p, *f1 = a3 + ((nb * n3 + 3) & ~int64_t(3));
-    const float *kf = w.dev + (400 + 16) * 2 + 2000 + 16 + 6 * 48 * 32 + 32 + 6 * 32 * 64 + 64, *bf = kf + n3 * F;
-    *tail = bf + F;
-    *f1_out = f1;
+constexpr int64_t SNP_BATCH = 262144, SNP_N3 = 3 * 9 * 64, SNP_F = 48;
+inline const float *snp_fc1_weights(const nc_weights &w) { return w.dev + (400 + 16) * 2 + 2000 + 16 + 6 * 48 * 32 + 32 + 6 * 32 * 64 + 64; }
+
+int launch_snp_trunk(nc_ctx *ctx, const nc_weights &w, DevBuf &buf, int64_t s0, int64_t nb, const void *x_dev, const double *scale, int scale_mode, SnpBatch *out)
+{
+    NC_TRY(nc_ensure(ctx, buf, (size_t)(nb * (SNP_N3 + SNP_F)) * 4 + 64));
+    float *a3 = (float *)buf.p;
+    out->a3 = a3;
+    out->f1 = a3 + ((nb * SNP_N3 + 3) & ~int64_t(3));
     SnpTrunkArgs a = {ctx->stream, nullptr, nullptr, nullptr, nullptr, a3, nb, s0, scale, scale_mode, w.x_limit, ctx->range_sites};
     if (ctx->x_i16) a.x_i16 = (const int16_t *)x_dev + s0 * NC_SNP_TENSOR;
     else a.x_f32 = (const float *)x_dev + s0 * NC_SNP_TENSOR;
@@ -110,14 +112,52 @@
         ctx->n_kev += 2;
     }
     const SnpTrunk t = nc_cnn_snp_trunk_select(ctx);
-    if (t.kernel_id == NC_TRUNK_FP32) {
-        nc_cnn_launch_k4_conv12(a, w.packed);
-        nc_cnn_launch_fc1_fp32(ctx->stream, F, a3, (int)n3, kf, bf, f1, nb);
-    } else {
-        nc_cnn_launch_k5_trunk(t.kernel_id, a, (const uint8_t *)w.packed_h);
-        nc_cnn_launch_fc1_h3(ctx->stream, a3, (const uint8_t *)w.packed_h, f1, nb);
-    }
+    out->fp32 = t.kernel_id == NC_TRUNK_FP32;
+    if (out->fp32) nc_cnn_launch_k4_conv12(a, w.packed);
+    else nc_cnn_launch_k5_trunk(t.kernel_id, a, (const uint8_t *)w.packed_h);
     NC_HIP(ctx, hipGetLastError());
+    return NC_OK;
+}
+
+int launch_snp_tail(nc_ctx *ctx, hipStream_t st, int kind, const nc_weights &w, const SnpBatch &b, int64_t s0, int64_t nb, const int32_t *ref_code_dev,
+                    float *probs_dev, float *gt_dev)
+{
+    const float *kf = snp_fc1_weights(w), *bf = kf + SNP_N3 * SNP_F, *heads = bf + SNP_F;
+    if (b.fp32) nc_cnn_launch_fc1_fp32(st, (int)SNP_F, b.a3, (int)SNP_N3, kf, bf, b.f1, nb);
+    else nc_cnn_launch_fc1_h3(st, b.a3, (const uint8_t *)w.packed_h, b.f1, nb);
+    if (kind == NC_MODEL_SNP)
+        hipLaunchKernelGGL(k_snp_heads, dim3(blocks_for(nb)), dim3(256), 0, st, b.f1, heads, ref_code_dev + s0, nb, probs_dev + s0 * 4,
+                           gt_dev ? gt_dev + s0 * 2 : nullptr);
+    else
+        hipLaunchKernelGGL(k_snp_hap_heads, dim3(blocks_for(nb)), dim3(256), 0, st, b.f1, heads, ref_code_dev + s0, nb, probs_dev + s0 * 4);
+    NC_HIP(ctx, hipGetLastError());
+    return NC_OK;
+}
+
+int drain_snp_batch(nc_ctx *ctx, hipStream_t st, int64_t s0, int64_t nb, const float *probs_dev, const float *gt_dev, float *probs_host, float *gt_host)
+{
+    NC_TRY(nc_d2h(ctx, probs_host + s0 * 4, probs_dev + s0 * 4, (size_t)nb * 16, st));
+    if (gt_host && gt_dev) NC_TRY(nc_d2h(ctx, gt_host + s0 * 2, gt_dev + s0 * 2, (size_t)nb * 8, st));
+    return NC_OK;
+}
+
+int check_snp_forward(nc_ctx *ctx, int32_t kind, int64_t n, const void *x_dev, const int32_t *ref_code_dev, int32_t scale_mode, const float *probs_dev)
+{
+    if (kind != NC_MODEL_SNP && kind != NC_MODEL_SNP_HAP) return nc_fail(ctx, NC_ERR_ARG, "nc_snp_forward: not an SNP model kind");
+    if (!ctx->w[kind].dev) return nc_fail(ctx, NC_ERR_STATE, "nc_snp_forward: weights of kind %d not loaded", kind);
+    if (n < 0 || (n && (!x_dev || !ref_code_dev || !probs_dev))) return nc_fail(ctx, NC_ERR_ARG, "nc_snp_forward: null argument");
+    if (scale_mode != 0 && scale_mode != 1) return nc_fail(ctx, NC_ERR_ARG, "nc_snp_forward: scale_mode");
+    if (ctx->x_i16 && ctx->cnn_exact_fp32) return nc_fail(ctx, NC_ERR_STATE, "nc_snp_forward: int16 tensors are read by the split-precision trunk only");
+    return NC_OK;
+}
+
+int wait_snp_tails(nc_ctx *ctx)
+{
+    for (int b = 0; b < NC_SNP_SLOTS; b++)
+        if (ctx->snp_act_busy[b]) {
+            NC_HIP(ctx, hipEventSynchronize(ctx->snp_act_ev[b]));
+            ctx->snp_act_busy[b] = false;
+        }
     return NC_OK;
 }
 
@@ -188,6 +228,8 @@
 
 }
 
+void nc_snp_tail_free(nc_snp_tail *t) { delete t; }
+
 extern "C" {
 
 int nc_load_weights(nc_ctx *ctx, int32_t kind, const float *blob_host, size_t n_floats)
@@ -197,6 +239,8 @@
     if (n_floats != NPARAM[kind])
         return nc_fail(ctx, NC_ERR_ARG, "nc_load_weights: kind %d expects %zu floats, got %zu", kind, NPARAM[kind], n_floats);
     NC_HIP(ctx, hipSetDevice(ctx->device));
+    if (ctx->snp_tail) return nc_fail(ctx, NC_ERR_STATE, "nc_load_weights: a deferred SNP tail is pending (nc_snp_tail_enqueue)");
+    NC_TRY(wait_snp_tails(ctx));
     nc_weights &w = ctx->w[kind];
     NC_TRY(upload_blob(ctx, (void **)&w.dev, blob_host, n_floats * 4, "weights"));
     w.n = n_floats;
@@ -225,40 +269,101 @@
 {
     if (!ctx) return NC_ERR_ARG;
     if (probs_host && !copy_stream) return nc_fail(ctx, NC_ERR_ARG, "nc_snp_forward_drain: host drain needs a copy stream");
-    if (kind != NC_MODEL_SNP && kind != NC_MODEL_SNP_HAP) return nc_fail(ctx, NC_ERR_ARG, "nc_snp_forward: not an SNP model kind");
-    if (!ctx->w[kind].dev) return nc_fail(ctx, NC_ERR_STATE, "nc_snp_forward: weights of kind %d not loaded", kind);
-    if (n < 0 || (n && (!x_dev || !ref_code_dev || !probs_dev))) return nc_fail(ctx, NC_ERR_ARG, "nc_snp_forward: null argument");
-    if (scale_mode != 0 && scale_mode != 1) return nc_fail(ctx, NC_ERR_ARG, "nc_snp_forward: scale_mode");
-    if (ctx->x_i16 && ctx->cnn_exact_fp32) return nc_fail(ctx, NC_ERR_STATE, "nc_snp_forward: int16 tensors are read by the split-precision trunk only");
+    NC_TRY(check_snp_forward(ctx, kind, n, x_dev, ref_code_dev, scale_mode, probs_dev));
     NC_HIP(ctx, hipSetDevice(ctx->device));
     NcTimer tm(ctx, 2);
     if (ctx->timing) nc_timing_resolve(ctx, 4);
     ctx->n_kev = 0;
-    const int64_t BATCH = 262144;
-    for (int64_t s0 = 0; s0 < n; s0 += BATCH) {
-        const int64_t nb = n - s0 < BATCH ? n - s0 : BATCH;
-        const float *tail = nullptr, *f1 = nullptr;
-        NC_TRY(run_snp_trunk(ctx, ctx->w[kind], s0, nb, x_dev, scale_dev, scale_mode, &f1, &tail));
-        if (kind == NC_MODEL_SNP)
-            hipLaunchKernelGGL(k_snp_heads, dim3(blocks_for(nb)), dim3(256), 0, ctx->stream, f1, tail, ref_code_dev + s0, nb,
-                               probs_dev + s0 * 4, gt_dev ? gt_dev + s0 * 2 : nullptr);
-        else
-            hipLaunchKernelGGL(k_snp_hap_heads, dim3(blocks_for(nb)), dim3(256), 0, ctx->stream, f1, tail, ref_code_dev + s0, nb,
-                               probs_dev + s0 * 4);
-        NC_HIP(ctx, hipGetLastError());
+    for (int64_t s0 = 0; s0 < n; s0 += SNP_BATCH) {
+        const int64_t nb = n - s0 < SNP_BATCH ? n - s0 : SNP_BATCH;
+        SnpBatch b;
+        NC_TRY(launch_snp_trunk(ctx, ctx->w[kind], ctx->cnn_c, s0, nb, x_dev, scale_dev, scale_mode, &b));
+        NC_TRY(launch_snp_tail(ctx, ctx->stream, kind, ctx->w[kind], b, s0, nb, ref_code_dev, probs_dev, gt_dev));
         if (probs_host) {
-            const int slot = (int)((s0 / BATCH) & 3);
+            const int slot = (int)((s0 / SNP_BATCH) & 3);
             if (!ctx->drain_ev[slot]) NC_HIP(ctx, hipEventCreateWithFlags(&ctx->drain_ev[slot], hipEventDisableTiming));
             NC_HIP(ctx, hipEventRecord(ctx->drain_ev[slot], ctx->stream));
             NC_HIP(ctx, hipStreamWaitEvent((hipStream_t)copy_stream, ctx->drain_ev[slot], 0));
-            NC_TRY(nc_d2h(ctx, probs_host + s0 * 4, probs_dev + s0 * 4, (size_t)nb * 16, (hipStream_t)copy_stream));
-            if (gt_host && gt_dev)
-                NC_TRY(nc_d2h(ctx, gt_host + s0 * 2, gt_dev + s0 * 2, (size_t)nb * 8, (hipStream_t)copy_stream));
+            NC_TRY(drain_snp_batch(ctx, (hipStream_t)copy_stream, s0, nb, probs_dev, gt_dev, probs_host, gt_host));
         }
     }
     tm.stop();
     if (ctx->timing) ctx->kev_pending = true;
     return NC_OK;
+}
+
+int nc_snp_trunk_phase(nc_ctx *ctx, int32_t kind, int64_t n, const float *x_dev, const int32_t *ref_code_dev, const double *scale_dev,
+                       int32_t scale_mode, float *probs_dev, float *gt_dev, void *side_stream, float *probs_host, float *gt_host, nc_snp_tail **tail_out)
+{
+    if (!ctx) return NC_ERR_ARG;
+    if (!tail_out || !side_stream) return nc_fail(ctx, NC_ERR_ARG, "nc_snp_trunk_phase: null argument");
+    *tail_out = nullptr;
+    const int64_t nbatch = n > 0 ? (n + SNP_BATCH - 1) / SNP_BATCH : 0;
+    if (ctx->timing == 1 || nbatch > NC_SNP_SLOTS)
+        return nc_snp_forward_drain(ctx, kind, n, x_dev, ref_code_dev, scale_dev, scale_mode, probs_dev, gt_dev, side_stream, probs_host, gt_host);
+    NC_TRY(check_snp_forward(ctx, kind, n, x_dev, ref_code_dev, scale_mode, probs_dev));
+    if (ctx->snp_tail) return nc_fail(ctx, NC_ERR_STATE, "nc_snp_trunk_phase: the previous call's tail has not been enqueued (nc_snp_tail_enqueue)");
+    NC_HIP(ctx, hipSetDevice(ctx->device));
+    if (ctx->timing) nc_timing_resolve(ctx, 4);
+    ctx->n_kev = 0;
+    nc_snp_tail *t = new (std::nothrow) nc_snp_tail();
+    if (!t) return nc_fail(ctx, NC_ERR_NOMEM, "nc_snp_trunk_phase: out of host memory");
+    t->kind = kind;
+    t->n = n;
+    t->ref_code = ref_code_dev;
+    t->probs = probs_dev;
+    t->gt = gt_dev;
+    t->probs_host = probs_host;
+    t->gt_host = gt_host;
+    auto trunks = [&]() -> int {
+        for (int b = 0; b < (int)nbatch; b++) {
+            const int64_t s0 = b * SNP_BATCH, nb = n - s0 < SNP_BATCH ? n - s0 : SNP_BATCH;
+            if (ctx->snp_act_busy[b]) {
+                if ((size_t)(nb * (SNP_N3 + SNP_F)) * 4 + 64 > ctx->snp_act[b].cap) NC_HIP(ctx, hipEventSynchronize(ctx->snp_act_ev[b]));
+                else NC_HIP(ctx, hipStreamWaitEvent(ctx->stream, ctx->snp_act_ev[b], 0));
+                ctx->snp_act_busy[b] = false;
+            }
+            NC_TRY(launch_snp_trunk(ctx, ctx->w[kind], ctx->snp_act[b], s0, nb, x_dev, scale_dev, scale_mode, &t->batch[b]));
+            if (!ctx->snp_trunk_ev[b]) NC_HIP(ctx, hipEventCreateWithFlags(&ctx->snp_trunk_ev[b], hipEventDisableTiming));
+            NC_HIP(ctx, hipEventRecord(ctx->snp_trunk_ev[b], ctx->stream));
+        }
+        return NC_OK;
+    };
+    const int rc = trunks();
+    if (rc != NC_OK) {
+        delete t;
+        return rc;
+    }
+    if (ctx->timing) ctx->kev_pending = true;
+    ctx->snp_tail = t;
+    *tail_out = t;
+    return NC_OK;
+}
+
+int nc_snp_tail_enqueue(nc_ctx *ctx, nc_snp_tail *tail, void *side_stream, void *start_event)
+{
+    if (!ctx) return NC_ERR_ARG;
+    if (!tail || !side_stream) return nc_fail(ctx, NC_ERR_ARG, "nc_snp_tail_enqueue: null argument");
+    if (tail != ctx->snp_tail) return nc_fail(ctx, NC_ERR_STATE, "nc_snp_tail_enqueue: not the pending tail of this context");
+    NC_HIP(ctx, hipSetDevice(ctx->device));
+    const hipStream_t st = (hipStream_t)side_stream;
+    auto tails = [&]() -> int {
+        if (start_event) NC_HIP(ctx, hipStreamWaitEvent(st, (hipEvent_t)start_event, 0));
+        for (int b = 0; (int64_t)b * SNP_BATCH < tail->n; b++) {
+            const int64_t s0 = b * SNP_BATCH, nb = tail->n - s0 < SNP_BATCH ? tail->n - s0 : SNP_BATCH;
+            NC_HIP(ctx, hipStreamWaitEvent(st, ctx->snp_trunk_ev[b], 0));
+            NC_TRY(launch_snp_tail(ctx, st, tail->kind, ctx->w[tail->kind], tail->batch[b], s0, nb, tail->ref_code, tail->probs, tail->gt));
+            if (!ctx->snp_act_ev[b]) NC_HIP(ctx, hipEventCreateWithFlags(&ctx->snp_act_ev[b], hipEventDisableTiming));
+            NC_HIP(ctx, hipEventRecord(ctx->snp_act_ev[b], st));
+            ctx->snp_act_busy[b] = true;
+            if (tail->probs_host) NC_TRY(drain_snp_batch(ctx, st, s0, nb, tail->probs, tail->gt, tail->probs_host, tail->gt_host));
+        }
+        return NC_OK;
+    };
+    const int rc = tails();
+    ctx->snp_tail = nullptr;
+    delete tail;
+    return rc;
 }
 
 int nc_cnn_x_limit(nc_ctx *ctx, int32_t kind, float *x_limit)
diff --git a/nanocaller_amd/csrc/nc_common.h b/nanocaller_amd/csrc/nc_common.h
--- a/nanocaller_amd/csrc/nc_common.h
+++ b/nanocaller_amd/csrc/nc_common.h
@@ -42,6 +42,8 @@
     void *packed_h = nullptr;
     float x_limit = 0.0f;
 };
+
+#define NC_SNP_SLOTS 8
 
 struct nc_ctx {
     int device = 0;
@@ -81,6 +83,11 @@
     DevBuf site_pos, site_chunk, site_n, site_alt;
     DevBuf totals;
     DevBuf cnn_a, cnn_b, cnn_c;
+    DevBuf snp_act[NC_SNP_SLOTS];
+    hipEvent_t snp_trunk_ev[NC_SNP_SLOTS] = {nullptr};
+    hipEvent_t snp_act_ev[NC_SNP_SLOTS] = {nullptr};
+    bool snp_act_busy[NC_SNP_SLOTS] = {false};
+    nc_snp_tail *snp_tail = nullptr;
     DevBuf chunk_depth;
     DevBuf nbr_idx;
     struct {
@@ -203,5 +210,6 @@
     }
 };
 
+void nc_snp_tail_free(nc_snp_tail *t);
 int nc_selftest_device(nc_ctx *ctx);
 void nc_pipe_destroy(nc_ctx *ctx);
diff --git a/nanocaller_amd/csrc/nc_ctx.hip b/nanocaller_amd/csrc/nc_ctx.hip
--- a/nanocaller_amd/csrc/nc_ctx.hip
+++ b/nanocaller_amd/csrc/nc_ctx.hip
@@ -138,6 +138,12 @@
     }
     for (auto &e : ctx->kev) if (e) (void)hipEventDestroy(e);
     for (auto &e : ctx->drain_ev) if (e) (void)hipEventDestroy(e);
+    for (int b = 0; b < NC_SNP_SLOTS; b++) {
+        if (ctx->snp_act_busy[b]) (void)hipEventSynchronize(ctx->snp_act_ev[b]);
+        if (ctx->snp_act_ev[b]) (void)hipEventDestroy(ctx->snp_act_ev[b]);
+        if (ctx->snp_trunk_ev[b]) (void)hipEventDestroy(ctx->snp_trunk_ev[b]);
+    }
+    nc_snp_tail_free(ctx->snp_tail);
     if (ctx->scan_ev) (void)hipEventDestroy(ctx->scan_ev);
     if (ctx->scale_ev) (void)hipEventDestroy(ctx->scale_ev);
     for (auto &p : ctx->tev) for (auto &e : p) if (e) (void)hipEventDestroy(e);
diff --git a/nanocaller_amd/engine.py b/nanocaller_amd/engine.py
--- a/nanocaller_amd/engine.py
+++ b/nanocaller_amd/engine.py
@@ -59,6 +59,17 @@
     rev_dp: torch.Tensor | None = None
     depth: torch.Tensor | None = None
     valid: torch.Tensor | None = None
+
+
+@dataclass
+class PendingTail:
+    handle: object
+    probs: torch.Tensor
+    gt: torch.Tensor | None
+    h_probs: np.ndarray
+    h_gt: np.ndarray | None
+    keep: tuple = ()
+    done: torch.cuda.Event | None = None
 
 
 class _PinnedPool:
@@ -320,6 +331,54 @@
                                                 _ptr(probs), _ptr(gt), self._copy_stream_ptr(), C.c_void_p(hp.data_ptr()),
                                                 C.c_void_p(hg.data_ptr()) if hg is not None else None), "nc_snp_forward_drain")
         return probs, gt, hp_np, hg_np
+
+    def snp_forward_deferred(self, kind, x, ref_code, scale, scale_mode=0, want_gt=True, range_flags=None) -> "PendingTail":
+        self.flush_tail()
+        n = int(x.shape[0])
+        probs = torch.empty((n, 4), dtype=torch.float32, device=self.device)
+        gt = torch.empty((n, 2), dtype=torch.float32, device=self.device) if (want_gt and kind == _lib.MODEL_SNP) else None
+        hp, hp_np = self._pinned.get((n, 4), torch.float32)
+        hg, hg_np = self._pinned.get((n, 2), torch.float32) if gt is not None else (None, None)
+        handle = C.c_void_p()
+        if range_flags is not None:
+            self._check(self.L.nc_cnn_range_watch(self.ctx, C.c_void_p(range_flags.data_ptr())), "nc_cnn_range_watch")
+        try:
+            self._check(self.L.nc_snp_trunk_phase(self.ctx, kind, n, _ptr(x), _ptr(ref_code), _ptr(scale), int(scale_mode), _ptr(probs), _ptr(gt),
+                                                  self._tail_stream_ptr(), C.c_void_p(hp.data_ptr()), C.c_void_p(hg.data_ptr()) if hg is not None else None,
+                                                  C.byref(handle)), "nc_snp_trunk_phase")
+        finally:
+            if range_flags is not None:
+                self.L.nc_cnn_range_watch(self.ctx, None)
+        pt = PendingTail(handle=handle if handle.value else None, probs=probs, gt=gt, h_probs=hp_np, h_gt=hg_np,
+                         keep=(x, ref_code, scale, probs, gt, hp, hg))
+        if pt.handle is None:
+            self._tail_enqueued(pt)
+        else:
+            self._pending_tail = pt
+        return pt
+
+    def enqueue_tail(self, pt: "PendingTail", start=None):
+        if pt.done is not None:
+            return
+        assert pt is getattr(self, "_pending_tail", None)
+        self._pending_tail = None
+        handle, pt.handle = pt.handle, None
+        self._check(self.L.nc_snp_tail_enqueue(self.ctx, handle, self._tail_stream_ptr(), C.c_void_p(start.cuda_event) if start is not None else None),
+                    "nc_snp_tail_enqueue")
+        self._tail_enqueued(pt)
+
+    def _tail_enqueued(self, pt):
+        ts = self._tail_stream()
+        for t in pt.keep[:5]:
+            if t is not None:
+                t.record_stream(ts)
+        pt.done = torch.cuda.Event()
+        pt.done.record(ts)
+
+    def flush_tail(self):
+        pt = getattr(self, "_pending_tail", None)
+        if pt is not None:
+            self.enqueue_tail(pt)
 
     def indel_forward(self, kind, x):
         n = int(x.shape[0])
@@ -581,6 +640,14 @@
     def _copy_stream_ptr(self):
         return C.c_void_p(self._copy_stream().cuda_stream)
 
+    def _tail_stream(self):
+        if getattr(self, "_sstream", None) is None:
+            self._sstream = torch.cuda.Stream(device=self.device)
+        return self._sstream
+
+    def _tail_stream_ptr(self):
+        return C.c_void_p(self._tail_stream().cuda_stream)
+
     def to_host_async(self, tensors):
         cs = self._copy_stream()
         ev = torch.cuda.Event()
diff --git a/nanocaller_amd/snpCaller.py b/nanocaller_amd/snpCaller.py
--- a/nanocaller_amd/snpCaller.py
+++ b/nanocaller_amd/snpCaller.py
@@ -169,15 +169,15 @@
 _PENDING_CNN = {}
 
 
-def flush_pending_cnn(device=0):
+def flush_pending_cnn(device=0, overlap=False):
     f = _PENDING_CNN.pop(device, None)
     if f is not None:
-        f()
+        f(overlap)
 
 
 def call_chunks(params, chunks, device=0, dpk=None, defer=False, pipeline=None):
     if pipeline is None:
-        pipeline = bool(defer) and os.environ.get('NC_PIPE_CNN', '0') == '1'
+        pipeline = bool(defer) and os.environ.get('NC_TAIL_OVERLAP', '1') != '0'
     if not pipeline:
         flush_pending_cnn(device)
     chrom = chunks[0]['chrom']
@@ -201,7 +201,7 @@
         dpk = device_pack_for(params, chrom, device, span=contig_span(params['sam_path'], chrom, chunks))
     sites = eng.snp_scan(dpk, [(c['start'], c['end']) for c in chunks], mincov=params['mincov'],
                          min_allele_freq=params['min_allele_freq'], threshold=params['threshold'],
-                         haploid=(ploidy == 'haploid'), async_fetch=True, between=(lambda: flush_pending_cnn(device)) if pipeline else None)
+                         haploid=(ploidy == 'haploid'), async_fetch=True, between=(lambda: flush_pending_cnn(device, overlap=True)) if pipeline else None)
     res = dict(chrom=chrom, ploidy=ploidy, n=0)
     if sites.n_sites == 0:
         eng.wait_copies()
@@ -217,41 +217,52 @@
     i16 = not getattr(eng, "exact_fp32", False)
     eng.set_tensor_format(int16=False)
     cnn = {}
-
-    def enqueue_cnn():
-        eng.use_torch_stream()
-        eng.set_tensor_format(int16=i16)
-        try:
-            flags_ = torch.zeros(sites.n_sites, dtype=torch.uint8, device=eng.device) if guard else None
-            cnn['d_probs'], cnn['d_gt'], cnn['h_probs'], cnn['h_gt'] = eng.snp_forward(kind, sites.x, sites.ref_code, scale, scale_mode=1 if per_site else 0,
-                                                                                   drain=True, range_flags=flags_)
-            cnn['flags'] = flags_
-            cnn['h_nflag'] = eng.to_host_async([flags_.sum(dtype=torch.int32).reshape(1)])[0] if guard else None
-        finally:
-            eng.set_tensor_format(int16=False)
-        cnn['drained'] = eng.copy_event()
+    scale_mode = 1 if per_site else 0
+    eng.set_tensor_format(int16=i16)
+    try:
+        flags = torch.zeros(sites.n_sites, dtype=torch.uint8, device=eng.device) if guard else None
+        if pipeline:
+            tail = eng.snp_forward_deferred(kind, sites.x, sites.ref_code, scale, scale_mode=scale_mode, range_flags=flags)
+            cnn['d_probs'], cnn['d_gt'], cnn['h_probs'], cnn['h_gt'] = tail.probs, tail.gt, tail.h_probs, tail.h_gt
+        else:
+            tail = None
+            cnn['d_probs'], cnn['d_gt'], cnn['h_probs'], cnn['h_gt'] = eng.snp_forward(kind, sites.x, sites.ref_code, scale, scale_mode=scale_mode,
+                                                                                   drain=True, range_flags=flags)
+    finally:
+        eng.set_tensor_format(int16=False)
+
+    def enqueue_tail(overlap=False):
+        if tail is not None:
+            start = None
+            if overlap:
+                start = torch.cuda.Event()
+                start.record(torch.cuda.current_stream(eng.device))
+            eng.enqueue_tail(tail, start)
+        cnn['h_nflag'] = eng.to_host_async([flags.sum(dtype=torch.int32).reshape(1)])[0] if guard else None
+        cnn['drained'] = [eng.copy_event()] + ([tail.done] if tail is not None else [])
     if pipeline:
-        _PENDING_CNN[device] = enqueue_cnn
+        _PENDING_CNN[device] = enqueue_tail
     else:
-        enqueue_cnn()
+        enqueue_tail()
     scan_copied.synchronize()
     freq = sites.alt.astype(np.float64) / sites.dp.astype(np.float64)
-    keep_alive = (sites, scale, cnn)
+    keep_alive = (sites, scale, cnn, tail)
 
     def finish():
         nonlocal keep_alive
         if 'drained' not in cnn:
-            if _PENDING_CNN.get(device) is enqueue_cnn:
+            if _PENDING_CNN.get(device) is enqueue_tail:
                 flush_pending_cnn(device)
             else:
-                enqueue_cnn()
-        drained, h_nflag, flags, d_probs, d_gt, h_probs, h_gt = (cnn[k] for k in ('drained', 'h_nflag', 'flags', 'd_probs', 'd_gt', 'h_probs', 'h_gt'))
-        drained.synchronize()
+                enqueue_tail()
+        drained, h_nflag, d_probs, d_gt, h_probs, h_gt = (cnn[k] for k in ('drained', 'h_nflag', 'd_probs', 'd_gt', 'h_probs', 'h_gt'))
+        for ev in drained:
+            ev.synchronize()
         n_rerun = int(h_nflag[0]) if h_nflag is not None else 0
         if n_rerun:
             idx = torch.nonzero(flags).squeeze(1)
             eng.use_torch_stream()
-            eng.range_rerun(kind, sites.x, sites.ref_code, scale, 1 if per_site else 0, idx, d_probs, d_gt)
+            eng.range_rerun(kind, sites.x, sites.ref_code, scale, scale_mode, idx, d_probs, d_gt)
             ih = idx.cpu().numpy()
             h_probs[ih] = d_probs[idx].cpu().numpy()
             if h_gt is not None and d_gt is not None:
```

Result: slower. 59.19 million (-3.3%).
